# Fedomn/sqlrs

Hardware: AMD Instinct MI355X
Metric: Mrows/sec for filter->hash-join->group-by pipeline; achieved HBM GB/s vs peak (higher is better)
Workload: dtype int64 keys / f64 sum; 1 GPU; C5 filter(val>0.5) -> hash-join(fact x dim on int64 key) -> group-by(key) COUNT,SUM(f64); fact_rows=1000000000, dim_rows=10000000, groups=10000000, parallelism=single GPU

## Files before the change

sqlrs_amd/csrc/agg_partition.hip:

```cpp
#include <algorithm>
#include <cstdlib>
#include <cstring>

#include "agg_partition.hpp"
#include "device_utils.hpp"
#include "radix_part.hpp"

namespace sq {

#ifndef PART_WG_N
#define PART_WG_N 512
#endif
constexpr int PART_WG = PART_WG_N;
#ifndef DENSE_WG_N
#define DENSE_WG_N 1024
#endif
constexpr int DENSE_WG = DENSE_WG_N;
#ifndef HOT_MIN_PEERS_N
#define HOT_MIN_PEERS_N 8
#endif
constexpr int HOT_MIN_PEERS = HOT_MIN_PEERS_N;
constexpr uint64_t LDS_EMPTY = ~0ull;

__device__ __forceinline__ uint32_t bucket_of(uint64_t h, uint32_t P) {
  return (uint32_t)__umul64hi(h, (uint64_t)P);
}

__global__ __launch_bounds__(PART_WG) void key_stats_kernel(const uint64_t *__restrict__ keys,
                                                            const uint64_t *__restrict__ validity,
                                                            int64_t n, int sample_shift, int block_stride, int hll_bits,
                                                            unsigned int *__restrict__ hll) {
  __shared__ unsigned int reg[2 * 4096];
  const int nreg = 1 << hll_bits;
  for (int i = threadIdx.x; i < 2 * 4096; i += PART_WG) reg[i] = 0;
  __syncthreads();
  uint64_t kmin = ~0ull, kmax = 0;
  const int64_t smask = (1ll << sample_shift) - 1, shalf = sample_shift ? 1ll << (sample_shift - 1) : -1;
  const unsigned blk_set = block_stride > 1 && (blockIdx.x & 1) ? 4096u : 0u;
  constexpr int KU = 12;
  const int64_t nchunks = (n + PART_WG * KU - 1) / (PART_WG * KU);
  const int64_t nsel = block_stride > 1 ? (nchunks + block_stride - 1) / block_stride + 1 : nchunks;
  for (int64_t ci = blockIdx.x; ci < nsel; ci += gridDim.x) {
    const int64_t chunk = block_stride > 1 ? min(ci * block_stride, nchunks - 1) : ci;
    const int64_t base = chunk * (int64_t)(PART_WG * KU) + threadIdx.x;
    uint64_t k[KU];
#pragma unroll
    for (int u = 0; u < KU; u++) k[u] = __builtin_nontemporal_load(keys + min(base + u * PART_WG, n - 1));
#pragma unroll
    for (int u = 0; u < KU; u++) {
      const int64_t r = base + u * PART_WG;
      if (r >= n) continue;
      if (validity && !((validity[r >> 6] >> (r & 63)) & 1)) continue;
      const uint64_t o = k[u] ^ (1ull << 63);
      kmin = min(kmin, o);
      kmax = max(kmax, o);
      const int64_t grp = (r >> 6) & smask;
      if (grp != 0 && grp != shalf) continue;
      uint64_t h = mix64(k[u] ^ 0x2545f4914f6cdd1dULL);
      unsigned idx = (unsigned)(h >> (64 - hll_bits)) + (grp == shalf ? 4096u : blk_set);
      unsigned rank = (unsigned)__builtin_clzll((h << hll_bits) | (1ull << (hll_bits - 1))) + 1;
      if (reg[idx] < rank) atomicMax(&reg[idx], rank);
    }
  }
  __syncthreads();
  for (int i = threadIdx.x; i < nreg; i += PART_WG) {
    if (reg[i]) atomicMax(&hll[i], reg[i]);
    if (reg[4096 + i]) atomicMax(&hll[4096 + i], reg[4096 + i]);
  }
  __shared__ unsigned long long s_mm[2][PART_WG / 64];
  kmin = wave_min_u64(kmin);
  kmax = wave_max_u64(kmax);
  if (lane_id() == 0) {
    s_mm[0][wave_id()] = kmin;
    s_mm[1][wave_id()] = kmax;
  }
  __syncthreads();
  if (threadIdx.x == 0) {
    for (int w = 1; w < PART_WG / 64; w++) {
      kmin = min(kmin, (uint64_t)s_mm[0][w]);
      kmax = max(kmax, (uint64_t)s_mm[1][w]);
    }
    unsigned long long *mm = (unsigned long long *)(hll + 8192);
    atomicMin(mm, (unsigned long long)kmin);
    atomicMax(mm + 1, (unsigned long long)kmax);
  }
}

static double hll_pass(Ctx *ctx, const uint64_t *keys, const uint64_t *validity, int64_t n, int sample_shift,
                       uint64_t *omin, uint64_t *omax, int block_stride = 1, double *half = nullptr) {
  const int hll_bits = block_stride > 1 ? 10 : 12;
  BufP hll = ctx->alloc_zero(8192 * 4 + 16);
  SQ_HIP(hipMemsetAsync(hll->as<uint8_t>() + 8192 * 4, 0xff, 8, ctx->stream));
  {
    ProfScope ps(ctx, "key_stats");
    unsigned blocks = (unsigned)std::min<int64_t>(ceil_div(n, (int64_t)PART_WG * 16 * block_stride), 2 * (int64_t)ctx->num_cus);
    key_stats_kernel<<<dim3(std::max(blocks, 1u)), dim3(PART_WG), 0, ctx->stream>>>(keys, validity, n, sample_shift,
                                                                                  block_stride, hll_bits, hll->as<unsigned int>());
    SQ_HIP(hipGetLastError());
  }
  const unsigned int *hreg = (const unsigned int *)ctx->fetch(hll->p, 8192 * 4 + 16);
  if (omin) std::memcpy(omin, hreg + 8192, 8);
  if (omax) std::memcpy(omax, hreg + 8194, 8);
  const int nreg = 1 << hll_bits;
  const double m = (double)nreg;
  auto estimate = [&](bool both) {
    double sum = 0;
    int zeros = 0;
    for (int i = 0; i < nreg; i++) {
      const unsigned r = both ? std::max(hreg[i], hreg[4096 + i]) : hreg[i];
      sum += std::ldexp(1.0, -(int)r);
      zeros += (r == 0);
    }
    double e = (0.7213 / (1.0 + 1.079 / m)) * m * m / sum;
    if (e <= 2.5 * m && zeros) e = m * std::log(m / zeros);
    return e;
  };
  const double e_half = estimate(false), e = estimate(true);
  if (half) *half = e_half;
  return e;
}

double estimate_distinct(Ctx *ctx, const uint64_t *keys, const uint64_t *validity, int64_t n,
                         uint64_t *omin, uint64_t *omax, bool *sampled) {
  if (sampled) *sampled = false;
  constexpr double SATURATED = 0.8;
  constexpr double DISJOINT = 0.6;
  double half = 0;
  if (sampled && !validity && n >= (1ll << 24)) {
    const int stride = 8;
    const double e = hll_pass(ctx, keys, validity, n, 0, omin, omax, stride, &half);
    if (e <= 0.2 * (double)(n / stride) && half >= DISJOINT * e) {
      *sampled = true;
      return half >= SATURATED * e ? e * 1.25 : e * (1.25 + 2.5 * (SATURATED - half / e));
    }
    if (half < DISJOINT * e) return hll_pass(ctx, keys, validity, n, 0, omin, omax);
  }
  const int shift = n >= (1ll << 22) ? 3 : 0;
  double e = hll_pass(ctx, keys, validity, n, shift, omin, omax, 1, &half);
  if (shift && (e > 0.2 * (double)(n >> shift) || half < SATURATED * e)) e = hll_pass(ctx, keys, validity, n, 0, omin, omax);
  return e;
}

enum AccKind { AK_COUNT = 0, AK_SUM_I64 = 1, AK_SUM_F64 = 2, AK_MIN_I64 = 3, AK_MIN_F64 = 4, AK_MAX_I64 = 5, AK_MAX_F64 = 6 };

struct LdsAggParams {
  int n_acc;
  int code[PART_MAX_ACC];
  uint32_t cap;
  const unsigned long long *partner_bits;
  const unsigned int *partner_mult;
  int seg_off;
};

__device__ __forceinline__ unsigned long long acc_times(int kind, unsigned long long cell, unsigned int m) {
  switch (kind) {
  case 0 :
  case 1 : return cell * (unsigned long long)m;
  case 2 : return (unsigned long long)__double_as_longlong(__longlong_as_double((long long)cell) * (double)m);
  default: return cell;
  }
}

__device__ __forceinline__ uint64_t acc_identity_cell(int kind) {
  return (kind == AK_MIN_I64 || kind == AK_MIN_F64) ? ~0ull : 0ull;
}

__device__ __forceinline__ uint32_t slot_hash(uint64_t key) {
  uint32_t x = (uint32_t)key ^ ((uint32_t)(key >> 32) * 0x85ebca6bu);
  x *= 0x9e3779b1u;
  return x ^ (x >> 15);
}

__device__ __forceinline__ void acc_apply(int kind, unsigned long long *c, uint64_t v) {
  switch (kind) {
  case AK_COUNT: atomicAdd(c, 1ull); break;
  case AK_SUM_I64: atomicAdd(c, (unsigned long long)v); break;
  case AK_SUM_F64: unsafeAtomicAdd((double *)c, __longlong_as_double((long long)v)); break;
  case AK_MIN_I64: atomicMin(c, (unsigned long long)i64_to_ordered((int64_t)v)); break;
  case AK_MIN_F64: atomicMin(c, (unsigned long long)f64_to_ordered(__longlong_as_double((long long)v))); break;
  case AK_MAX_I64: atomicMax(c, (unsigned long long)i64_to_ordered((int64_t)v)); break;
  default: atomicMax(c, (unsigned long long)f64_to_ordered(__longlong_as_double((long long)v)));
  }
}

#ifndef LDS_U_ROWS
#define LDS_U_ROWS 4
#endif
constexpr int LDS_U = LDS_U_ROWS;
template <int NV> struct AggRows {
  uint64_t k[LDS_U], v0[NV >= 1 ? LDS_U : 1], v1[NV >= 2 ? LDS_U : 1];
  uint32_t id[LDS_U];
  uint8_t f[LDS_U];
};

template <int NV, bool FLAGS, bool PACK, int WG = PART_WG>
__device__ __forceinline__ void lds_agg_load(const uint64_t *__restrict__ pk, const uint32_t *__restrict__ pi,
                                             const uint64_t *__restrict__ pv0, const uint64_t *__restrict__ pv1,
                                             const uint8_t *__restrict__ pf, int64_t i0, int64_t hi,
                                             AggRows<NV> &r) {
#pragma unroll
  for (int u = 0; u < LDS_U; u++) {
    int64_t i = min(i0 + (int64_t)u * WG, hi - 1);
    r.k[u] = __builtin_nontemporal_load(pk + i);
    if (!PACK) r.id[u] = pi ? __builtin_nontemporal_load(pi + i) : (uint32_t)i;
    if (NV >= 1) r.v0[u] = __builtin_nontemporal_load(pv0 + i);
    if (NV >= 2) r.v1[u] = __builtin_nontemporal_load(pv1 + i);
    r.f[u] = FLAGS ? pf[i] : 7;
  }
}

template <int NV, int WG = PART_WG>
__device__ __forceinline__ void lds_agg_load_rec(const uint64_t *__restrict__ prec, int64_t i0, int64_t hi, AggRows<NV> &r) {
#pragma unroll
  for (int u = 0; u < LDS_U; u++) {
    int64_t i = min(i0 + (int64_t)u * WG, hi - 1);
    const u64x2 t = __builtin_nontemporal_load((const u64x2 *)prec + i);
    r.k[u] = t.x;
    r.v0[0 + (NV >= 1 ? u : 0)] = t.y;
    r.f[u] = 7;
  }
}

struct SplitTables {
  unsigned long long *key = nullptr;
  unsigned int *first = nullptr;
  unsigned long long *acc = nullptr;
  uint32_t nsplit = 0;
};

__global__ void split_init_kernel(SplitTables stb, int64_t total, int n_acc, LdsAggParams prm) {
  int64_t i = blockIdx.x * (int64_t)blockDim.x + threadIdx.x;
  if (i >= total) return;
  stb.key[i] = LDS_EMPTY;
  stb.first[i] = 0xffffffffu;
  for (int a = 0; a < n_acc; a++) stb.acc[(size_t)a * total + i] = acc_identity_cell(prm.code[a] & 7);
}

__global__ void split_emit_kernel(SplitTables stb, uint32_t nslots, uint32_t cap, int n_acc,
                                  unsigned long long *out_count, uint64_t *__restrict__ gkey,
                                  uint32_t *__restrict__ gfirst, uint8_t *__restrict__ gvalid,
                                  uint64_t *__restrict__ gacc, int64_t gcap) {
  const int64_t total = (int64_t)stb.nsplit * nslots;
  int64_t i = blockIdx.x * (int64_t)blockDim.x + threadIdx.x;
  if (i >= total) return;
  unsigned int first = stb.first[i];
  if (first == 0xffffffffu) return;
  const uint32_t s = (uint32_t)(i % nslots);
  unsigned long long base = atomicAdd(out_count, 1ull);
  if ((int64_t)base >= gcap) return;
  gkey[base] = s == cap + 1 ? LDS_EMPTY : stb.key[i];
  gfirst[base] = first;
  if (gvalid) gvalid[base] = s == cap ? 0 : 1;
  for (int a = 0; a < n_acc; a++) gacc[(size_t)a * gcap + base] = stb.acc[(size_t)a * total + i];
}

template <int NV, bool FLAGS, bool JOIN, int NACC, int C0, int C1, bool PACK, bool REC = false>
__global__ __launch_bounds__(PART_WG) void lds_agg_kernel(
    LdsAggParams prm, const uint64_t *__restrict__ pk, const uint32_t *__restrict__ pi,
    const uint64_t *__restrict__ pv0, const uint64_t *__restrict__ pv1,
    const uint8_t *__restrict__ pf, const uint32_t *__restrict__ work , uint32_t P,
    int64_t n, unsigned long long *out_count, uint64_t *__restrict__ gkey,
    uint32_t *__restrict__ gfirst, uint8_t *__restrict__ gvalid, uint64_t *__restrict__ gacc,
    int64_t gcap, unsigned long long *ov_count, uint32_t *__restrict__ ov_rows,
    const uint64_t *__restrict__ bk, const uint8_t *__restrict__ bf, const uint32_t *__restrict__ bbstart,
    KeyPack kp, SplitTables stb) {
  extern __shared__ __attribute__((aligned(16))) unsigned long long tab[];
  __shared__ unsigned int s_cnt, s_join_fail;
  __shared__ unsigned long long s_base;
  const uint32_t b = work[4 * blockIdx.x];
  const int64_t lo = work[4 * blockIdx.x + 1];
  const int64_t hi = work[4 * blockIdx.x + 2];
  const uint32_t split = work[4 * blockIdx.x + 3];
  const uint32_t cap = prm.cap, mask = cap - 1, nslots = cap + 2;
  const int n_acc = NACC >= 0 ? NACC : prm.n_acc;
  auto code_of = [&](int a) { return NACC >= 0 ? (a == 0 ? C0 : C1) : prm.code[a]; };
  unsigned long long *tkey = tab;
  unsigned long long *tacc = tab + nslots;
  unsigned int *tfirst = (unsigned int *)(tacc + (size_t)n_acc * nslots);
  AggRows<NV> cur, nxt;
  if (lo < hi) {
    if (REC) lds_agg_load_rec<NV>(pk, lo + threadIdx.x, hi, cur);
    else lds_agg_load<NV, FLAGS, PACK>(pk, pi, pv0, pv1, pf, lo + threadIdx.x, hi, cur);
  }
  for (uint32_t s = threadIdx.x; s < nslots; s += PART_WG) {
    tkey[s] = LDS_EMPTY;
    tfirst[s] = 0xffffffffu;
#pragma unroll
    for (int a = 0; a < PART_MAX_ACC; a++) {
      if (a >= n_acc) break;
      tacc[(size_t)a * nslots + s] = acc_identity_cell(code_of(a) & 7);
    }
  }
  if (threadIdx.x == 0) {
    s_cnt = 0;
    s_join_fail = 0;
  }
  __syncthreads();
  if (JOIN) {
    if (*(volatile unsigned long long *)(ov_count + 1) != 0) return;
    const int64_t blo = bbstart[b], bhi = bbstart[b + 1];
    for (int64_t i = blo + threadIdx.x; i < bhi; i += PART_WG) {
      uint64_t key = bk[i];
      bool valid = bf ? (bf[i] & 1) : true;
      if (!valid) {
        if (atomicExch(&tkey[cap], 1ull) != LDS_EMPTY) s_join_fail = 1;
      } else if (key == LDS_EMPTY) {
        if (atomicExch(&tkey[cap + 1], 1ull) != LDS_EMPTY) s_join_fail = 1;
      } else {
        uint32_t s = slot_hash(key) & mask;
        uint32_t probes = 0;
        while (true) {
          unsigned long long prev = atomicCAS(&tkey[s], LDS_EMPTY, (unsigned long long)key);
          if (prev == key) s_join_fail = 1;
          if (prev == LDS_EMPTY || prev == key) break;
          s = (s + 1) & mask;
          if (++probes >= cap) {
            s_join_fail = 1;
            break;
          }
        }
      }
    }
    __syncthreads();
    if (s_join_fail) {
      if (threadIdx.x == 0) atomicExch(ov_count + 1, 1ull);
      return;
    }
  }
  __builtin_amdgcn_s_waitcnt(0x0F70);
  for (int64_t base = lo; base < hi; base += (int64_t)LDS_U * PART_WG) {
    const int64_t i0 = base + threadIdx.x;
    if (REC) lds_agg_load_rec<NV>(pk, i0 + (int64_t)LDS_U * PART_WG, hi, nxt);
    else lds_agg_load<NV, FLAGS, PACK>(pk, pi, pv0, pv1, pf, i0 + (int64_t)LDS_U * PART_WG, hi, nxt);
    uint32_t slot[LDS_U];
    unsigned long long seen[LDS_U];
    uint32_t sentinel = 0;
    if (PACK) {
#pragma unroll
      for (int u = 0; u < LDS_U; u++) {
        if (!JOIN && packed_off(kp, cur.k[u]) == kp.kmask) sentinel |= 1u << u;
        cur.id[u] = packed_row(kp, cur.k[u]);
        cur.k[u] = packed_key(kp, cur.k[u]);
      }
    }
#pragma unroll
    for (int u = 0; u < LDS_U; u++) {
      uint32_t s = slot_hash(cur.k[u]) & mask;
      if (FLAGS && !(cur.f[u] & 1)) s = cap;
      else if (cur.k[u] == LDS_EMPTY) s = cap + 1;
      slot[u] = s;
      seen[u] = tkey[s];
    }
#pragma unroll
    for (int u = 0; u < LDS_U; u++) {
      bool act = i0 + (int64_t)u * PART_WG < hi && !((sentinel >> u) & 1u);
      const uint64_t key = cur.k[u];
      uint32_t s = slot[u];
      unsigned long long c = seen[u];
      if (act) {
        if (s >= cap) {
          if (JOIN && c == LDS_EMPTY) act = false;
        } else if (JOIN) {
          uint32_t probes = 0;
          while (c != key && c != LDS_EMPTY && ++probes < cap) {
            s = (s + 1) & mask;
            c = tkey[s];
          }
          if (c != key) act = false;
        } else {
          uint32_t probes = 0;
          while (true) {
            if (c == key) break;
            if (c == LDS_EMPTY) {
              unsigned long long prev = atomicCAS(&tkey[s], LDS_EMPTY, (unsigned long long)key);
              if (prev == LDS_EMPTY || prev == key) break;
            }
            s = (s + 1) & mask;
            if (++probes >= cap) {
              unsigned long long o = atomicAdd(ov_count, 1ull);
              ov_rows[o] = cur.id[u];
              act = false;
              break;
            }
            c = tkey[s];
          }
        }
      }
      const uint64_t actm = __ballot(act);
      if (actm) {
        const int first = __builtin_ctzll(actm);
        const uint32_t s0 = (uint32_t)__shfl((int)s, first, 64);
        const bool hot = act && s == s0;
        const uint64_t peers = __ballot(hot);
        if (__popcll(peers) >= HOT_MIN_PEERS) {
          const uint32_t idmin = wave_min_u32_dpp(hot ? cur.id[u] : 0xffffffffu);
          if (lane_id() == first) atomicMin(&tfirst[s0], idmin);
#pragma unroll
          for (int a = 0; a < PART_MAX_ACC; a++) {
            if (a >= n_acc) break;
            const int code = code_of(a), kind = code & 7, src = code >> 3;
            const bool in = hot && (!FLAGS || (cur.f[u] & (2 << src)));
            const uint64_t v = (NV >= 2 && src) ? cur.v1[u] : cur.v0[u];
            unsigned long long *cell = tacc + (size_t)a * nslots + s0;
            const uint64_t inm = __ballot(in);
            uint64_t red;
            switch (kind) {
            case AK_COUNT: red = (uint64_t)__popcll(inm); break;
            case AK_SUM_I64: red = wave_sum_u64_dpp(in ? v : 0ull); break;
            case AK_SUM_F64: red = (uint64_t)__double_as_longlong(wave_sum_f64_dpp(in ? __longlong_as_double((long long)v) : 0.0)); break;
            case AK_MIN_I64: red = wave_min_u64(in ? i64_to_ordered((int64_t)v) : ~0ull); break;
            case AK_MIN_F64: red = wave_min_u64(in ? f64_to_ordered(__longlong_as_double((long long)v)) : ~0ull); break;
            case AK_MAX_I64: red = wave_max_u64(in ? i64_to_ordered((int64_t)v) : 0ull); break;
            default: red = wave_max_u64(in ? f64_to_ordered(__longlong_as_double((long long)v)) : 0ull);
            }
            if (lane_id() == first && inm) {
              switch (kind) {
              case AK_COUNT:
              case AK_SUM_I64: atomicAdd(cell, (unsigned long long)red); break;
              case AK_SUM_F64: unsafeAtomicAdd((double *)cell, __longlong_as_double((long long)red)); break;
              case AK_MIN_I64:
              case AK_MIN_F64: atomicMin(cell, (unsigned long long)red); break;
              default: atomicMax(cell, (unsigned long long)red);
              }
            }
          }
          act = act && !hot;
        }
      }
      if (act) {
        if (cur.id[u] < tfirst[s]) atomicMin(&tfirst[s], cur.id[u]);
#pragma unroll
        for (int a = 0; a < PART_MAX_ACC; a++) {
          if (a >= n_acc) break;
          const int code = code_of(a);
          const int src = code >> 3;
          if (FLAGS && !(cur.f[u] & (2 << src))) continue;
          uint64_t v = (NV >= 2 && src) ? cur.v1[u] : cur.v0[u];
          acc_apply(code & 7, tacc + (size_t)a * nslots + s, v);
        }
      }
    }
    cur = nxt;
  }
  __syncthreads();
  if (split != 0xffffffffu) {
    unsigned long long *gk = stb.key + (size_t)split * nslots;
    unsigned int *gf = stb.first + (size_t)split * nslots;
    for (uint32_t s = threadIdx.x; s < nslots; s += PART_WG) {
      unsigned int first = tfirst[s];
      if (first == 0xffffffffu) continue;
      uint32_t g = s;
      bool placed = true;
      if (s < cap) {
        const unsigned long long key = tkey[s];
        g = slot_hash(key) & mask;
        uint32_t probes = 0;
        while (true) {
          unsigned long long prev = atomicCAS(&gk[g], LDS_EMPTY, key);
          if (prev == LDS_EMPTY || prev == key) break;
          g = (g + 1) & mask;
          if (++probes >= cap) {
            placed = false;
            break;
          }
        }
      }
      if (!placed) {
        unsigned long long o = atomicAdd(out_count, 1ull);
        if ((int64_t)o < gcap) {
          gkey[o] = tkey[s];
          gfirst[o] = first;
          if (gvalid) gvalid[o] = 1;
#pragma unroll
          for (int a = 0; a < PART_MAX_ACC; a++) {
            if (a >= n_acc) break;
            gacc[(size_t)a * gcap + o] = tacc[(size_t)a * nslots + s];
          }
        }
        atomicExch(ov_count + 2, 1ull);
        continue;
      }
      atomicMin(&gf[g], first);
#pragma unroll
      for (int a = 0; a < PART_MAX_ACC; a++) {
        if (a >= n_acc) break;
        unsigned long long *cell = stb.acc + ((size_t)a * stb.nsplit + split) * nslots + g;
        const unsigned long long v = tacc[(size_t)a * nslots + s];
        switch (code_of(a) & 7) {
        case AK_COUNT:
        case AK_SUM_I64: atomicAdd(cell, v); break;
        case AK_SUM_F64: unsafeAtomicAdd((double *)cell, __longlong_as_double((long long)v)); break;
        case AK_MIN_I64:
        case AK_MIN_F64: atomicMin(cell, v); break;
        default: atomicMax(cell, v);
        }
      }
    }
    return;
  }
  unsigned int mine = 0;
  for (uint32_t s = threadIdx.x; s < nslots; s += PART_WG) mine += tfirst[s] != 0xffffffffu;
  unsigned int my_off = atomicAdd(&s_cnt, mine);
  __syncthreads();
  if (threadIdx.x == 0) s_base = atomicAdd(out_count, (unsigned long long)s_cnt);
  __syncthreads();
  unsigned long long base = s_base + my_off;
  for (uint32_t s = threadIdx.x; s < nslots; s += PART_WG) {
    unsigned int first = tfirst[s];
    if (first == 0xffffffffu) continue;
    if ((int64_t)base < gcap) {
      gkey[base] = s == cap + 1 ? LDS_EMPTY : tkey[s];
      gfirst[base] = first;
      if (gvalid) gvalid[base] = s == cap ? 0 : 1;
#pragma unroll
      for (int a = 0; a < PART_MAX_ACC; a++) {
        if (a >= n_acc) break;
        gacc[(size_t)a * gcap + base] = tacc[(size_t)a * nslots + s];
      }
    }
    base++;
  }
}

constexpr int SED_SLOTS = 16, SED_GROUPS = 16;
__global__ __launch_bounds__(SED_SLOTS * SED_GROUPS) void split_emit_dense_kernel(
    SplitTables stb, const uint32_t *__restrict__ split_bucket, const uint32_t *__restrict__ chunk_lo, uint32_t nbuckets_split,
    uint32_t R, KeyPack kp, LdsAggParams prm, int n_acc, unsigned long long *out_count, uint64_t *__restrict__ gkey,
    uint32_t *__restrict__ gfirst, uint64_t *__restrict__ gacc, int64_t gcap) {
  __shared__ unsigned int s_first[SED_GROUPS][SED_SLOTS];
  __shared__ unsigned long long s_acc[PART_MAX_ACC][SED_GROUPS][SED_SLOTS];
  const uint32_t tiles_per_bucket = (R + SED_SLOTS - 1) / SED_SLOTS;
  const uint32_t t = blockIdx.x / tiles_per_bucket, sl = threadIdx.x % SED_SLOTS, cg = threadIdx.x / SED_SLOTS;
  const uint32_t s = (blockIdx.x % tiles_per_bucket) * SED_SLOTS + sl;
  if (t >= nbuckets_split) return;
  const int64_t total = (int64_t)stb.nsplit * R;
  unsigned int first = 0xffffffffu;
  unsigned long long acc[PART_MAX_ACC];
  for (int a = 0; a < n_acc; a++) acc[a] = acc_identity_cell(prm.code[a] & 7);
  if (s < R) {
    const uint32_t c1 = chunk_lo[t + 1];
    for (uint32_t c = chunk_lo[t] + cg; c < c1; c += SED_GROUPS) {
      const unsigned int f = stb.first[(size_t)c * R + s];
      if (f == 0xffffffffu) continue;
      first = min(first, f);
      for (int a = 0; a < n_acc; a++) {
        const unsigned long long v = stb.acc[(size_t)a * total + (size_t)c * R + s];
        switch (prm.code[a] & 7) {
        case AK_COUNT:
        case AK_SUM_I64: acc[a] += v; break;
        case AK_SUM_F64: acc[a] = (unsigned long long)__double_as_longlong(__longlong_as_double((long long)acc[a]) + __longlong_as_double((long long)v)); break;
        case AK_MIN_I64:
        case AK_MIN_F64: acc[a] = min(acc[a], v); break;
        default: acc[a] = max(acc[a], v);
        }
      }
    }
  }
  s_first[cg][sl] = first;
  for (int a = 0; a < n_acc; a++) s_acc[a][cg][sl] = acc[a];
  __syncthreads();
  if (cg != 0 || s >= R) return;
  for (int g = 1; g < SED_GROUPS; g++) {
    const unsigned int f = s_first[g][sl];
    if (f == 0xffffffffu) continue;
    first = min(first, f);
    for (int a = 0; a < n_acc; a++) {
      const unsigned long long v = s_acc[a][g][sl];
      switch (prm.code[a] & 7) {
      case AK_COUNT:
      case AK_SUM_I64: acc[a] += v; break;
      case AK_SUM_F64: acc[a] = (unsigned long long)__double_as_longlong(__longlong_as_double((long long)acc[a]) + __longlong_as_double((long long)v)); break;
      case AK_MIN_I64:
      case AK_MIN_F64: acc[a] = min(acc[a], v); break;
      default: acc[a] = max(acc[a], v);
      }
    }
  }
  if (first == 0xffffffffu) return;
  unsigned int mlt = 1;
  if (prm.partner_mult) mlt = prm.partner_mult[((uint64_t)split_bucket[t] << kp.rbits) + s];
  unsigned long long base = atomicAdd(out_count, 1ull);
  if ((int64_t)base >= gcap) return;
  gkey[base] = kp.kmin + ((uint64_t)split_bucket[t] << kp.rbits) + s;
  gfirst[base] = first;
  for (int a = 0; a < n_acc; a++) gacc[(size_t)a * gcap + base] = prm.partner_mult ? acc_times(prm.code[a] & 7, acc[a], mlt) : acc[a];
}

template <int NV, bool JOIN, int NACC, int C0, int C1, bool REC = false>
__global__ __launch_bounds__(DENSE_WG) void lds_agg_dense_kernel(
    LdsAggParams prm, const uint64_t *__restrict__ pk, const uint64_t *__restrict__ pv0,
    const uint32_t *__restrict__ work, unsigned long long *out_count, uint64_t *__restrict__ gkey,
    uint32_t *__restrict__ gfirst, uint64_t *__restrict__ gacc, int64_t gcap, KeyPack kp, SplitTables stb) {
  extern __shared__ __attribute__((aligned(16))) unsigned long long tab[];
  __shared__ unsigned int s_cnt;
  __shared__ unsigned long long s_base;
  const uint32_t b = work[4 * blockIdx.x];
  const int64_t lo = work[4 * blockIdx.x + 1];
  const int64_t hi = work[4 * blockIdx.x + 2];
  const uint32_t split = work[4 * blockIdx.x + 3];
  const uint32_t R = prm.cap, mask = R - 1;
  const int n_acc = NACC >= 0 ? NACC : prm.n_acc;
  auto code_of = [&](int a) { return NACC >= 0 ? (a == 0 ? C0 : C1) : prm.code[a]; };
  unsigned long long *tacc = tab;
  unsigned int *tfirst = (unsigned int *)(tacc + (size_t)n_acc * R);
  AggRows<NV> cur, nxt;
  if (lo < hi) {
    if (REC) lds_agg_load_rec<NV, DENSE_WG>(pk, lo + threadIdx.x, hi, cur);
    else lds_agg_load<NV, false, true, DENSE_WG>(pk, nullptr, pv0, nullptr, nullptr, lo + threadIdx.x, hi, cur);
  }
  for (uint32_t s = threadIdx.x; s < R; s += DENSE_WG) {
    tfirst[s] = 0xffffffffu;
#pragma unroll
    for (int a = 0; a < PART_MAX_ACC; a++) {
      if (a >= n_acc) break;
      tacc[(size_t)a * R + s] = acc_identity_cell(code_of(a) & 7);
    }
  }
  if (threadIdx.x == 0) s_cnt = 0;
  __syncthreads();
  uint32_t hc_slot = 0xffffffffu, hc_min = 0xffffffffu;
  uint64_t hc_acc[PART_MAX_ACC];
  auto hot_flush = [&]() {
    if (hc_slot == 0xffffffffu) return;
    if (lane_id() == 0) {
      atomicMin(&tfirst[hc_slot], hc_min);
#pragma unroll
      for (int a = 0; a < PART_MAX_ACC; a++) {
        if (a >= n_acc) break;
        unsigned long long *cell = tacc + (size_t)a * R + hc_slot;
        switch (code_of(a) & 7) {
        case AK_COUNT:
        case AK_SUM_I64: atomicAdd(cell, (unsigned long long)hc_acc[a]); break;
        case AK_SUM_F64: unsafeAtomicAdd((double *)cell, __longlong_as_double((long long)hc_acc[a])); break;
        case AK_MIN_I64:
        case AK_MIN_F64: atomicMin(cell, (unsigned long long)hc_acc[a]); break;
        default: atomicMax(cell, (unsigned long long)hc_acc[a]);
        }
      }
    }
    hc_slot = 0xffffffffu;
  };
  auto hot_take = [&](uint32_t s0, uint32_t idmin) {
    if (hc_slot != s0) {
      hot_flush();
      hc_slot = s0;
      hc_min = 0xffffffffu;
#pragma unroll
      for (int a = 0; a < PART_MAX_ACC; a++) {
        if (a >= n_acc) break;
        hc_acc[a] = acc_identity_cell(code_of(a) & 7);
      }
    }
    hc_min = idmin < hc_min ? idmin : hc_min;
  };
  auto hot_add = [&](int a, int kind, uint64_t red) {
    switch (kind) {
    case AK_COUNT:
    case AK_SUM_I64: hc_acc[a] += red; break;
    case AK_SUM_F64: hc_acc[a] = (uint64_t)__double_as_longlong(__longlong_as_double((long long)hc_acc[a]) + __longlong_as_double((long long)red)); break;
    case AK_MIN_I64:
    case AK_MIN_F64: hc_acc[a] = red < hc_acc[a] ? red : hc_acc[a]; break;
    default: hc_acc[a] = red > hc_acc[a] ? red : hc_acc[a];
    }
  };
  __builtin_amdgcn_s_waitcnt(0x0F70);
  for (int64_t base = lo; base < hi; base += (int64_t)LDS_U * DENSE_WG) {
    const int64_t i0 = base + threadIdx.x;
    if (REC) lds_agg_load_rec<NV, DENSE_WG>(pk, i0 + (int64_t)LDS_U * DENSE_WG, hi, nxt);
    else lds_agg_load<NV, false, true, DENSE_WG>(pk, nullptr, pv0, nullptr, nullptr, i0 + (int64_t)LDS_U * DENSE_WG, hi, nxt);
#pragma unroll
    for (int u = 0; u < LDS_U; u++) {
      const uint64_t off = packed_off(kp, cur.k[u]);
      const uint32_t id = packed_row(kp, cur.k[u]);
      const uint32_t s = (uint32_t)off & mask;
      bool act = i0 + (int64_t)u * DENSE_WG < hi;
      act = act && off <= kp.range;
      const uint64_t actm = __ballot(act);
      if (actm) {
        const int first = __builtin_ctzll(actm);
        const uint32_t s0 = (uint32_t)__shfl((int)s, first, 64);
        const bool hot = act && s == s0;
        const uint64_t peers = __ballot(hot);
        if (__popcll(peers) >= HOT_MIN_PEERS) {
          const uint32_t idmin = wave_min_u32_dpp(hot ? id : 0xffffffffu);
          hot_take(s0, idmin);
#pragma unroll
          for (int a = 0; a < PART_MAX_ACC; a++) {
            if (a >= n_acc) break;
            const int kind = code_of(a) & 7;
            const uint64_t v = NV >= 1 ? cur.v0[u] : 0ull;
            uint64_t red;
            switch (kind) {
            case AK_COUNT: red = (uint64_t)__popcll(peers); break;
            case AK_SUM_I64: red = wave_sum_u64_dpp(hot ? v : 0ull); break;
            case AK_SUM_F64: red = (uint64_t)__double_as_longlong(wave_sum_f64_dpp(hot ? __longlong_as_double((long long)v) : 0.0)); break;
            case AK_MIN_I64: red = wave_min_u64(hot ? i64_to_ordered((int64_t)v) : ~0ull); break;
            case AK_MIN_F64: red = wave_min_u64(hot ? f64_to_ordered(__longlong_as_double((long long)v)) : ~0ull); break;
            case AK_MAX_I64: red = wave_max_u64(hot ? i64_to_ordered((int64_t)v) : 0ull); break;
            default: red = wave_max_u64(hot ? f64_to_ordered(__longlong_as_double((long long)v)) : 0ull);
            }
            hot_add(a, kind, red);
          }
          act = act && !hot;
        }
      }
      if (act) {
        if (id < tfirst[s]) atomicMin(&tfirst[s], id);
#pragma unroll
        for (int a = 0; a < PART_MAX_ACC; a++) {
          if (a >= n_acc) break;
          acc_apply(code_of(a) & 7, tacc + (size_t)a * R + s, NV >= 1 ? cur.v0[u] : 0ull);
        }
      }
    }
    cur = nxt;
  }
  hot_flush();
  __syncthreads();
  if (JOIN && (prm.partner_bits || prm.partner_mult)) {
    const uint64_t off0 = (uint64_t)b << kp.rbits;
    for (uint32_t s = threadIdx.x; s < R; s += DENSE_WG) {
      if (tfirst[s] == 0xffffffffu) continue;
      const uint64_t o = off0 + s;
      const bool partner = prm.partner_mult ? prm.partner_mult[o] != 0 : (((prm.partner_bits[o >> 6] >> (o & 63)) & 1ull) != 0);
      if (!partner) tfirst[s] = 0xffffffffu;
    }
  }
  if (split != 0xffffffffu) {
    unsigned int *gf = stb.first + (size_t)split * R;
    for (uint32_t s = threadIdx.x; s < R; s += DENSE_WG) {
      gf[s] = tfirst[s];
#pragma unroll
      for (int a = 0; a < PART_MAX_ACC; a++) {
        if (a >= n_acc) break;
        stb.acc[((size_t)a * stb.nsplit + split) * R + s] = tacc[(size_t)a * R + s];
      }
    }
    return;
  }
  unsigned int mine = 0;
  for (uint32_t s = threadIdx.x; s < R; s += DENSE_WG) mine += tfirst[s] != 0xffffffffu;
  unsigned int my_off = atomicAdd(&s_cnt, mine);
  __syncthreads();
  if (threadIdx.x == 0) s_base = atomicAdd(out_count, (unsigned long long)s_cnt);
  __syncthreads();
  unsigned long long base = s_base + my_off;
  const uint64_t key0 = kp.kmin + ((uint64_t)b << kp.rbits);
  for (uint32_t s = threadIdx.x; s < R; s += DENSE_WG) {
    unsigned int first = tfirst[s];
    if (first == 0xffffffffu) continue;
    if ((int64_t)base < gcap) {
      gkey[base] = key0 + s;
      gfirst[base] = first;
      const unsigned int mlt = (JOIN && prm.partner_mult) ? prm.partner_mult[((uint64_t)b << kp.rbits) + s] : 1u;
#pragma unroll
      for (int a = 0; a < PART_MAX_ACC; a++) {
        if (a >= n_acc) break;
        const unsigned long long cell = tacc[(size_t)a * R + s];
        gacc[(size_t)a * gcap + base] = (JOIN && prm.partner_mult) ? acc_times(code_of(a) & 7, cell, mlt) : cell;
      }
    }
    base++;
  }
}

struct SlimBucketIn {
  SlimRowsView rows;
  const uint32_t *nzstart, *nzbt, *nzcount, *bcol;
  uint32_t tile;
  uint32_t groups;
  const uint32_t *blk_bt;
  uint32_t log_b;
};
constexpr uint32_t SLIM_BT_CAP = 4096;
struct SlimAggRows {
  uint64_t v[LDS_U];
  uint32_t w[LDS_U], bt[LDS_U];
};

template <bool JOIN, int NACC, int C0, int C1, bool BLK = false>
__global__ __launch_bounds__(DENSE_WG) void lds_agg_dense_slim_kernel(
    LdsAggParams prm, SlimBucketIn in, const uint32_t *__restrict__ work, unsigned long long *out_count,
    uint64_t *__restrict__ gkey, uint32_t *__restrict__ gfirst, uint64_t *__restrict__ gacc, int64_t gcap, KeyPack kp,
    SplitTables stb) {
  extern __shared__ __attribute__((aligned(16))) unsigned long long tab[];
  __shared__ unsigned int s_cnt, s_before, s_inside;
  __shared__ unsigned long long s_base;
  __shared__ uint32_t s_wsum[DENSE_WG / 64];
  const uint32_t b = work[4 * blockIdx.x];
  const int64_t lo = work[4 * blockIdx.x + 1];
  const int64_t hi = work[4 * blockIdx.x + 2];
  const uint32_t split = work[4 * blockIdx.x + 3];
  const uint32_t R = prm.cap, mask = R - 1;
  const int n_acc = NACC >= 0 ? NACC : prm.n_acc;
  auto code_of = [&](int a) { return NACC >= 0 ? (a == 0 ? C0 : C1) : prm.code[a]; };
  unsigned long long *tacc = tab;
  unsigned int *tfirst = (unsigned int *)(tacc + (size_t)n_acc * R);
  unsigned long long *gmask = (unsigned long long *)(tfirst + R);
  uint32_t *gpre = (uint32_t *)(gmask + in.groups);
  uint32_t *gbt = gpre + in.groups;
  const uint32_t col = BLK ? 0u : in.bcol[b], nruns = BLK ? 0u : in.nzcount[b];
  const uint32_t ngroups = BLK ? 0u : (uint32_t)((hi - lo + 63) >> 6);
  const uint64_t le_mask = (2ull << lane_id()) - 1ull;
  const uint32_t rbits = kp.rbits, lmask = (1u << 13) - 1u;

  for (uint32_t s = threadIdx.x; s < R; s += DENSE_WG) {
    tfirst[s] = 0xffffffffu;
#pragma unroll
    for (int a = 0; a < PART_MAX_ACC; a++) {
      if (a >= n_acc) break;
      tacc[(size_t)a * R + s] = acc_identity_cell(code_of(a) & 7);
    }
  }
  for (uint32_t g = threadIdx.x; g < ngroups; g += DENSE_WG) gmask[g] = 0;
  if (threadIdx.x == 0) {
    s_cnt = 0;
    s_before = 0;
    s_inside = 0;
  }
  __syncthreads();
  if (!BLK) {
    uint32_t before = 0, inside = 0;
    for (uint32_t k = threadIdx.x; k < nruns; k += DENSE_WG) {
      const int64_t st = in.nzstart[col + k];
      if (st <= lo) before++;
      else if (st < hi) {
        inside++;
        atomicOr(&gmask[(st - lo) >> 6], 1ull << ((st - lo) & 63));
      }
    }
    before = wave_sum_u32(before);
    inside = wave_sum_u32(inside);
    if (lane_id() == 0 && before) atomicAdd(&s_before, before);
    if (lane_id() == 0 && inside) atomicAdd(&s_inside, inside);
  }
  __syncthreads();
  const uint32_t k_first = s_before - 1u, k_count = s_inside + 1u;
  const bool bt_lds = !BLK && k_count <= SLIM_BT_CAP;
  const bool seg_mode = NACC == 2 && ((C0 == AK_COUNT && C1 == AK_SUM_F64) || (C0 == AK_SUM_F64 && C1 == AK_COUNT)) &&
                        hi - lo >= 4096 && (int64_t)k_count * 2048 <= hi - lo && !prm.seg_off && !BLK;
  if (bt_lds)
    for (uint32_t k = threadIdx.x; k < k_count; k += DENSE_WG) gbt[k] = in.nzbt[col + min(k_first + k, nruns - 1)];
  if (!BLK) {
    constexpr uint32_t GPT = 8;
    uint32_t carry = s_before - 1u;
    for (uint32_t g0 = 0; g0 < ngroups; g0 += DENSE_WG * GPT) {
      const uint32_t gb = g0 + threadIdx.x * GPT;
      uint32_t pc[GPT], sum = 0;
#pragma unroll
      for (uint32_t i = 0; i < GPT; i++) {
        pc[i] = gb + i < ngroups ? (uint32_t)__popcll(gmask[gb + i]) : 0u;
        sum += pc[i];
      }
      const uint32_t inc = wave_iscan_u32(sum);
      if (lane_id() == 63) s_wsum[wave_id()] = inc;
      __syncthreads();
      uint32_t wbase = 0, tot = 0;
      for (int w = 0; w < DENSE_WG / 64; w++) {
        if (w < wave_id()) wbase += s_wsum[w];
        tot += s_wsum[w];
      }
      uint32_t run = carry + wbase + inc - sum;
#pragma unroll
      for (uint32_t i = 0; i < GPT; i++) {
        if (gb + i < ngroups) gpre[gb + i] = run;
        run += pc[i];
      }
      carry += tot;
      __syncthreads();
    }
  }
#ifndef SLIM_WAVE_SPAN
#define SLIM_WAVE_SPAN 1
#endif
  constexpr int64_t SLIM_USTEP = SLIM_WAVE_SPAN ? 64 : DENSE_WG;
  const int64_t slim_toff = SLIM_WAVE_SPAN ? (int64_t)wave_id() * (LDS_U * 64) + lane_id() : (int64_t)threadIdx.x;
  auto load = [&](int64_t i0, SlimAggRows &r) {
#pragma unroll
    for (int u = 0; u < LDS_U; u++) {
      const int64_t i = min(i0 + (int64_t)u * SLIM_USTEP, hi - 1);
      slim_load_nt(in.rows, i, r.w[u], r.v[u]);
      if (BLK) {
        r.bt[u] = in.blk_bt[i >> in.log_b];
        continue;
      }
      const uint32_t g = (uint32_t)((i - lo) >> 6);
      const uint32_t k = gpre[g] + (uint32_t)__popcll(gmask[g] & le_mask);
#if defined(SLIM_DBG) && (SLIM_DBG & 16)
      r.bt[u] = k;
#else
      r.bt[u] = bt_lds ? gbt[min(k - k_first, k_count - 1)] : in.nzbt[col + min(k, nruns - 1)];
#endif
    }
  };
  uint32_t hc_slot = 0xffffffffu, hc_min = 0xffffffffu;
  uint64_t hc_acc[PART_MAX_ACC];
  auto hot_flush = [&]() {
    if (hc_slot == 0xffffffffu) return;
    if (lane_id() == 0) {
      atomicMin(&tfirst[hc_slot], hc_min);
#pragma unroll
      for (int a = 0; a < PART_MAX_ACC; a++) {
        if (a >= n_acc) break;
        unsigned long long *cell = tacc + (size_t)a * R + hc_slot;
        switch (code_of(a) & 7) {
        case AK_COUNT:
        case AK_SUM_I64: atomicAdd(cell, (unsigned long long)hc_acc[a]); break;
        case AK_SUM_F64: unsafeAtomicAdd((double *)cell, __longlong_as_double((long long)hc_acc[a])); break;
        case AK_MIN_I64:
        case AK_MIN_F64: atomicMin(cell, (unsigned long long)hc_acc[a]); break;
        default: atomicMax(cell, (unsigned long long)hc_acc[a]);
        }
      }
    }
    hc_slot = 0xffffffffu;
  };
  auto hot_take = [&](uint32_t s0, uint32_t idmin) {
    if (hc_slot != s0) {
      hot_flush();
      hc_slot = s0;
      hc_min = 0xffffffffu;
#pragma unroll
      for (int a = 0; a < PART_MAX_ACC; a++) {
        if (a >= n_acc) break;
        hc_acc[a] = acc_identity_cell(code_of(a) & 7);
      }
    }
    hc_min = idmin < hc_min ? idmin : hc_min;
  };
  auto hot_add = [&](int a, int kind, uint64_t red) {
    switch (kind) {
    case AK_COUNT:
    case AK_SUM_I64: hc_acc[a] += red; break;
    case AK_SUM_F64: hc_acc[a] = (uint64_t)__double_as_longlong(__longlong_as_double((long long)hc_acc[a]) + __longlong_as_double((long long)red)); break;
    case AK_MIN_I64:
    case AK_MIN_F64: hc_acc[a] = red < hc_acc[a] ? red : hc_acc[a]; break;
    default: hc_acc[a] = red > hc_acc[a] ? red : hc_acc[a];
    }
  };
  SlimAggRows cur, nxt;
  if (lo < hi) load(lo + slim_toff, cur);
  __builtin_amdgcn_s_waitcnt(0x0F70);
  for (int64_t base = lo; base < hi; base += (int64_t)LDS_U * DENSE_WG) {
    const int64_t i0 = base + slim_toff;
    load(i0 + (int64_t)LDS_U * DENSE_WG, nxt);
    uint32_t sl[LDS_U], id[LDS_U], tf[LDS_U];
#pragma unroll
    for (int u = 0; u < LDS_U; u++) {
      const uint32_t w = cur.w[u];
      sl[u] = w & mask;
      id[u] = (cur.bt[u] + (w >> (rbits + 13))) * in.tile + ((w >> rbits) & lmask);
      tf[u] = tfirst[sl[u]];
    }
    constexpr bool SEG_CAPABLE = NACC == 2 && ((C0 == AK_COUNT && C1 == AK_SUM_F64) || (C0 == AK_SUM_F64 && C1 == AK_COUNT));
    const int lane = (int)lane_id();
    auto seg_rows = [&](bool act, uint32_t sl_u, uint64_t v_u, uint32_t id_u, uint32_t tf_u) {
      const uint32_t key = act ? sl_u : (0x80000000u | (uint32_t)lane);
      const uint32_t prevk = (uint32_t)__builtin_amdgcn_update_dpp(0, (int)key, 0x138, 0xf, 0xf, false);
      const uint64_t bm = __ballot(lane == 0 || key != prevk);
      const int headl = 63 - __builtin_clzll(bm & le_mask);
      double incl = act ? __longlong_as_double((long long)v_u) : 0.0;
      uint32_t idh = act ? id_u : 0xffffffffu;
      wave_seg_iscan_f64_min_u32(incl, idh, headl, lane);
      const bool tail = act && (lane == 63 || ((bm >> (lane + 1)) & 1ull));
      if (tail) {
        const uint32_t s = sl_u;
        if (idh < tf_u) atomicMin(&tfirst[s], idh);
        atomicAdd(tacc + (size_t)(C0 == AK_COUNT ? 0 : 1) * R + s, (unsigned long long)(lane - headl + 1));
        unsafeAtomicAdd((double *)(tacc + (size_t)(C0 == AK_COUNT ? 1 : 0) * R + s), incl);
      }
    };
    if (seg_mode) {
#pragma unroll
      for (int u = 0; u < LDS_U; u++) {
        const bool act = i0 + (int64_t)u * SLIM_USTEP < hi;
        {
          const uint32_t s0 = (uint32_t)__builtin_amdgcn_readfirstlane((int)sl[u]);
          if (__ballot(act && sl[u] == s0) == ~0ull) {
            hot_take(s0, wave_min_u32_dpp(id[u]));
            hot_add(C0 == AK_COUNT ? 0 : 1, AK_COUNT, 64ull);
            hot_add(C0 == AK_COUNT ? 1 : 0, AK_SUM_F64, (uint64_t)__double_as_longlong(wave_sum_f64_dpp(__longlong_as_double((long long)cur.v[u]))));
            continue;
          }
        }
        seg_rows(act, sl[u], cur.v[u], id[u], tf[u]);
      }
      cur = nxt;
      continue;
    }
#pragma unroll
    for (int u = 0; u < LDS_U; u++) {
      const uint32_t s = sl[u];
      bool act = i0 + (int64_t)u * SLIM_USTEP < hi;
      if (BLK) act = act && cur.w[u] != 0xffffffffu;
#ifdef SLIM_DBG
      uint64_t actm = (SLIM_DBG & 1) ? 0ull : __ballot(act);
#else
      uint64_t actm = __ballot(act);
#endif
      for (int it = 0; it < 3 && actm; it++) {
        const int first = __builtin_ctzll(actm);
        const uint32_t s0 = (uint32_t)__builtin_amdgcn_readlane((int)s, first);
        const bool hot = act && s == s0;
        const uint64_t peers = __ballot(hot);
        if (__popcll(peers) < HOT_MIN_PEERS) break;
        if (SEG_CAPABLE && it == 0 && peers != actm && (((peers >> first) + 1) & (peers >> first)) == 0 && !prm.seg_off) {
          seg_rows(act, s, cur.v[u], id[u], tf[u]);
          act = false;
          break;
        }
        const uint32_t idmin = wave_min_u32_dpp(hot ? id[u] : 0xffffffffu);
        hot_take(s0, idmin);
#pragma unroll
        for (int a = 0; a < PART_MAX_ACC; a++) {
          if (a >= n_acc) break;
          const int kind = code_of(a) & 7;
          const uint64_t v = cur.v[u];
          uint64_t red;
          switch (kind) {
          case AK_COUNT: red = (uint64_t)__popcll(peers); break;
          case AK_SUM_I64: red = wave_sum_u64_dpp(hot ? v : 0ull); break;
          case AK_SUM_F64: red = (uint64_t)__double_as_longlong(wave_sum_f64_dpp(hot ? __longlong_as_double((long long)v) : 0.0)); break;
          case AK_MIN_I64: red = wave_min_u64(hot ? i64_to_ordered((int64_t)v) : ~0ull); break;
          case AK_MIN_F64: red = wave_min_u64(hot ? f64_to_ordered(__longlong_as_double((long long)v)) : ~0ull); break;
          case AK_MAX_I64: red = wave_max_u64(hot ? i64_to_ordered((int64_t)v) : 0ull); break;
          default: red = wave_max_u64(hot ? f64_to_ordered(__longlong_as_double((long long)v)) : 0ull);
          }
          hot_add(a, kind, red);
        }
        act = act && !hot;
        actm &= ~peers;
      }
      if (act) {
#ifdef SLIM_DBG
        if (!(SLIM_DBG & 8) && id[u] < tf[u]) atomicMin(&tfirst[s], id[u]);
#pragma unroll
        for (int a = 0; a < PART_MAX_ACC; a++) {
          if (a >= n_acc) break;
          if ((SLIM_DBG >> (1 + a)) & 1) continue;
          acc_apply(code_of(a) & 7, tacc + (size_t)a * R + s, cur.v[u]);
        }
#else
        if (id[u] < tf[u]) atomicMin(&tfirst[s], id[u]);
#pragma unroll
        for (int a = 0; a < PART_MAX_ACC; a++) {
          if (a >= n_acc) break;
          acc_apply(code_of(a) & 7, tacc + (size_t)a * R + s, cur.v[u]);
        }
#endif
      }
    }
    cur = nxt;
  }
  hot_flush();
  __syncthreads();
  if (JOIN && (prm.partner_bits || prm.partner_mult)) {
    const uint64_t off0 = (uint64_t)b << kp.rbits;
    for (uint32_t s = threadIdx.x; s < R; s += DENSE_WG) {
      if (tfirst[s] == 0xffffffffu) continue;
      const uint64_t o = off0 + s;
      const bool partner = prm.partner_mult ? prm.partner_mult[o] != 0 : (((prm.partner_bits[o >> 6] >> (o & 63)) & 1ull) != 0);
      if (!partner) tfirst[s] = 0xffffffffu;
    }
  }
  if (split != 0xffffffffu) {
    unsigned int *gf = stb.first + (size_t)split * R;
    for (uint32_t s = threadIdx.x; s < R; s += DENSE_WG) {
      gf[s] = tfirst[s];
#pragma unroll
      for (int a = 0; a < PART_MAX_ACC; a++) {
        if (a >= n_acc) break;
        stb.acc[((size_t)a * stb.nsplit + split) * R + s] = tacc[(size_t)a * R + s];
      }
    }
    return;
  }
  unsigned int mine = 0;
  for (uint32_t s = threadIdx.x; s < R; s += DENSE_WG) mine += tfirst[s] != 0xffffffffu;
  unsigned int my_off = atomicAdd(&s_cnt, mine);
  __syncthreads();
  if (threadIdx.x == 0) s_base = atomicAdd(out_count, (unsigned long long)s_cnt);
  __syncthreads();
  unsigned long long obase = s_base + my_off;
  const uint64_t key0 = kp.kmin + ((uint64_t)b << kp.rbits);
  for (uint32_t s = threadIdx.x; s < R; s += DENSE_WG) {
    unsigned int first = tfirst[s];
    if (first == 0xffffffffu) continue;
    if ((int64_t)obase < gcap) {
      gkey[obase] = key0 + s;
      gfirst[obase] = first;
      const unsigned int mlt = (JOIN && prm.partner_mult) ? prm.partner_mult[((uint64_t)b << kp.rbits) + s] : 1u;
#pragma unroll
      for (int a = 0; a < PART_MAX_ACC; a++) {
        if (a >= n_acc) break;
        const unsigned long long cell = tacc[(size_t)a * R + s];
        gacc[(size_t)a * gcap + obase] = (JOIN && prm.partner_mult) ? acc_times(code_of(a) & 7, cell, mlt) : cell;
      }
    }
    obase++;
  }
}

__global__ void first_to_rowid_kernel(const uint32_t *__restrict__ gfirst, int64_t n, uint64_t offset,
                                      uint64_t *__restrict__ out) {
  int64_t i = blockIdx.x * (int64_t)blockDim.x + threadIdx.x;
  if (i < n) out[i] = offset + gfirst[i];
}
__global__ void bytes_pack_kernel(const uint8_t *__restrict__ bytes, int64_t n, uint64_t *__restrict__ out) {
  int64_t i = blockIdx.x * (int64_t)blockDim.x + threadIdx.x;
  bool b = (i < n) && bytes[i];
  uint64_t m = __ballot(b);
  if (lane_id() == 0 && i < n) out[i >> 6] = m;
}

__global__ __launch_bounds__(256) void key_range_kernel(const uint64_t *__restrict__ keys, int64_t n, unsigned long long *mm) {
  uint64_t kmin = ~0ull, kmax = 0;
  for (int64_t r = blockIdx.x * (int64_t)blockDim.x + threadIdx.x; r < n; r += (int64_t)gridDim.x * blockDim.x) {
    const uint64_t o = keys[r] ^ (1ull << 63);
    kmin = min(kmin, o);
    kmax = max(kmax, o);
  }
  kmin = wave_min_u64(kmin);
  kmax = wave_max_u64(kmax);
  __shared__ unsigned long long s_lo[4], s_hi[4];
  if (lane_id() == 0) {
    s_lo[wave_id()] = kmin;
    s_hi[wave_id()] = kmax;
  }
  __syncthreads();
  if (threadIdx.x == 0) {
    for (int w = 1; w < 4; w++) {
      kmin = min(kmin, (uint64_t)s_lo[w]);
      kmax = max(kmax, (uint64_t)s_hi[w]);
    }
    atomicMin(mm, (unsigned long long)kmin);
    atomicMax(mm + 1, (unsigned long long)kmax);
  }
}

const uint64_t *part_row_ids(Ctx *ctx, PartAggOutput &po) {
  if (!po.row_ids) {
    const int64_t g1 = std::max<int64_t>(po.groups, 1);
    po.row_ids = ctx->alloc(8 * (size_t)g1);
    if (po.groups) {
      first_to_rowid_kernel<<<dim3((unsigned)ceil_div(g1, 256)), dim3(256), 0, ctx->stream>>>(
          po.gfirst->as<uint32_t>(), po.groups, po.row_offset, po.row_ids->as<uint64_t>());
      SQ_HIP(hipGetLastError());
    }
  }
  return po.row_ids->as<uint64_t>();
}

bool partitioned_preaggregate(Ctx *ctx, const PartAggSpec &spec, const PartAggInput &in,
                              uint64_t row_offset, PartAggOutput *out) {
  int64_t n = in.n;
  if (n > 0xffffffffll || spec.n_acc > PART_MAX_ACC || spec.nv > 2) return false;
  const bool join_mode = in.join_keys != nullptr;
  uint64_t omin = ~0ull, omax = 0;
  bool sampled = false;
  const char *kse = hook("SQLRS_KEY_STATS_EXACT");
  const bool stats_exact_env = kse && kse[0] == '1';
  double est = join_mode ? (double)in.join_n
                         : estimate_distinct(ctx, in.keys, in.key_validity, n, &omin, &omax, (in.exact_stats || stats_exact_env) ? nullptr : &sampled);
  BufP ctr = ctx->alloc_zero(48);
  if (sampled && omin <= omax) {
    const uint64_t w = omax - omin, pad = std::max<uint64_t>(w / 8, 65536);
    omin = omin >= pad ? omin - pad : 0;
    omax = omax <= ~0ull - pad ? omax + pad : ~0ull;
  }
  static const double est_scale = [] {
    const char *e = hook("SQLRS_EST_SCALE");
    return e ? std::atof(e) : 1.0;
  }();
  if (!join_mode) est = std::max(1.0, est * est_scale);
  KeyPack kp;
  const bool nullable = in.key_validity || in.val_validity[0] || in.val_validity[1];
  if (!nullable && spec.nv <= 1 && !(join_mode && in.join_validity)) {
    if (join_mode && in.join_range_known) {
      omin = in.join_omin;
      omax = in.join_omax;
    } else if (join_mode) {
      BufP mm = ctx->alloc(16);
      SQ_HIP(hipMemsetAsync(mm->p, 0xff, 8, ctx->stream));
      SQ_HIP(hipMemsetAsync(mm->as<uint8_t>() + 8, 0, 8, ctx->stream));
      unsigned blocks = (unsigned)std::min<int64_t>(ceil_div(in.join_n, 1024), 1024);
      key_range_kernel<<<dim3(std::max(blocks, 1u)), dim3(256), 0, ctx->stream>>>(
          in.join_keys, in.join_n, mm->as<unsigned long long>());
      SQ_HIP(hipGetLastError());
      const uint64_t *h = (const uint64_t *)ctx->fetch(mm->p, 16);
      omin = h[0];
      omax = h[1];
    }
    if (omin <= omax) {
      uint64_t range = omax - omin;
      uint32_t kbits = 1;
      while (kbits < 64 && ((1ull << kbits) - 1) <= range) kbits++;
      int rowbits = 1;
      while (rowbits < 32 && (1ll << rowbits) < n) rowbits++;
      if (kbits + rowbits <= 64) {
        kp.kbits = kbits;
        kp.kmask = (1ull << kbits) - 1;
        kp.kmin = omin ^ (1ull << 63);
        if (sampled) {
          kp.oob = (unsigned int *)(ctr->as<uint64_t>() + 4);
          out->ov_rows = ctx->alloc(4 * (size_t)std::max<int64_t>(n, 1));
          kp.ov_rows = out->ov_rows->as<uint32_t>();
          kp.ov_count = ctr->as<unsigned long long>() + 1;
          kp.ov_cap = (uint32_t)std::min<int64_t>(n, std::max<int64_t>(65536, n / 1024));
        }
      }
    }
  }
  constexpr size_t lds_budget = 72 * 1024;
  const size_t slot_bytes = 8 + 8 * (size_t)spec.n_acc + 4;
  uint32_t cap = 1;
  while ((size_t)(cap * 2 + 2) * slot_bytes <= lds_budget) cap *= 2;
  constexpr double load_factor = 0.275;
  const double groups_per_table = cap * load_factor;
  double want = est * 1.15 / groups_per_table;
  if (!join_mode) est = std::min(est, (double)n);
  const char *dense_e = hook("SQLRS_DENSE_AGG");
  const bool dense_on = !(dense_e && dense_e[0] == '0');
  const uint64_t *partner_bits = nullptr;
  const double want_hashed = want;
  bool dense = false;
  if (dense_on && kp.kbits) {
    const uint64_t range = omax - omin;
    constexpr size_t dense_budget = 150 * 1024;
    const size_t dslot = 8 * (size_t)spec.n_acc + 4;
    uint32_t rbits = 8;
    while (rbits < 14 && ((size_t)2 << rbits) * dslot <= dense_budget) rbits++;
    while (rbits > 8 && (range >> (rbits - 1)) == 0) rbits--;
    const uint64_t pd = (range >> rbits) + 1;
    const bool fills = join_mode ? (in.join_unique_known && (range + 1 == (uint64_t)in.join_n ||
                                                             ((in.join_bits || in.join_mult) && in.join_range_known && range / 16 <= (uint64_t)in.join_n)))
                                 : ((double)range + 1.0 <= 4.0 * est);
    partner_bits = (join_mode && fills && !in.join_mult && range + 1 != (uint64_t)in.join_n) ? in.join_bits : nullptr;
    if (fills && pd <= 65536 && (double)pd <= 1.5 * std::max(1.0, std::ceil(want))) {
      dense = true;
      kp.dense = 1;
      kp.rbits = rbits;
      kp.range = range;
      cap = 1u << rbits;
      want = (double)pd;
    }
  }
  if (join_mode && in.join_mult && !dense) return false;
  if (want > 65536.0) return false;
  uint32_t P = (uint32_t)std::max(1.0, std::ceil(want));
  out->est_groups = est;
  PartitionInput pin;
  pin.pack = kp;
  pin.filter = in.filter;
  pin.keys = in.keys;
  pin.key_validity = in.key_validity;
  pin.n = n;
  pin.nv = spec.nv;
  for (int k = 0; k < 2; k++) {
    pin.vals[k] = in.vals[k];
    pin.val_validity[k] = in.val_validity[k];
  }
  PartitionedRows pr;
  const bool in_place = P == 1 && !join_mode && !nullable && want_hashed <= 1.0 && !in.filter.col;
  if (in_place) {
    dense = false;
    kp = KeyPack();
    cap = 1;
    while ((size_t)(cap * 2 + 2) * slot_bytes <= lds_budget) cap *= 2;
    pr.n = n;
    pr.P = 1;
    auto borrowed = [&](const void *p) {
      BufP b = std::make_shared<Buf>(ctx, const_cast<void *>(p), 0);
      b->owned = false;
      return b;
    };
    pr.key = borrowed(in.keys);
    pr.v0 = spec.nv >= 1 ? borrowed(in.vals[0]) : nullptr;
    pr.v1 = spec.nv >= 2 ? borrowed(in.vals[1]) : nullptr;
    pr.bstart_host = {0u, (uint32_t)n};
    pr.bstart = nullptr;
  } else if (!partition_rows(ctx, pin, P, &pr)) {
    return false;
  }
  P = pr.P;
  n = pr.n;
  if (dense != (pr.pack.dense != 0)) return false;
  if (n == 0) {
    out->groups = out->n_overflow = 0;
    out->gcap = 1;
    out->buckets = (int)P;
    out->gkey = ctx->alloc(8);
    out->gfirst = ctx->alloc(4);
    out->gacc = ctx->alloc(8 * (size_t)std::max(spec.n_acc, 1));
    out->ov_rows = ctx->alloc(4);
    out->row_ids = nullptr;
    out->row_offset = row_offset;
    return true;
  }
  out->buckets = (int)P;
  BufP pk = pr.key, pi = pr.idx, pv0 = pr.v0, pv1 = pr.v1, pf = pr.flags;
  PartitionedRows local_build;
  const PartitionedRows *bp = nullptr;
  if (join_mode && !dense) {
    if (in.join_cache && in.join_cache->P == P && in.join_cache->n == in.join_n) {
      bp = in.join_cache;
    } else {
      PartitionInput bin;
      bin.keys = in.join_keys;
      bin.key_validity = in.join_validity;
      bin.n = in.join_n;
      bin.nv = 0;
      bin.build_side = true;
      PartitionedRows *dst = in.join_cache ? in.join_cache : &local_build;
      if (!partition_rows(ctx, bin, P, dst) || dst->P != P) return false;
      bp = dst;
    }
  }
  LdsAggParams prm;
  prm.n_acc = spec.n_acc;
  for (int a = 0; a < PART_MAX_ACC; a++) {
    int kind = AK_COUNT;
    if (a < spec.n_acc) {
      switch (spec.op[a]) {
      case PART_COUNT: kind = AK_COUNT; break;
      case PART_SUM_I64: kind = AK_SUM_I64; break;
      case PART_SUM_F64: kind = AK_SUM_F64; break;
      case PART_MIN: kind = spec.kind[a] ? AK_MIN_F64 : AK_MIN_I64; break;
      default: kind = spec.kind[a] ? AK_MAX_F64 : AK_MAX_I64;
      }
    }
    prm.code[a] = a < spec.n_acc ? (kind | (spec.src[a] << 3)) : 0;
  }
  prm.cap = cap;
  prm.partner_bits = dense ? (const unsigned long long *)partner_bits : nullptr;
  prm.partner_mult = (dense && join_mode) ? in.join_mult : nullptr;
  {
    const char *seg_e = hook("SQLRS_AGG_SEG");
    prm.seg_off = (seg_e && seg_e[0] == '0') ? 1 : 0;
  }
  int64_t gcap = (int64_t)std::min<double>((double)n, est * 1.5 + 65536.0 + 2.0 * P);
  if (dense) gcap = (int64_t)std::min<uint64_t>((uint64_t)n, join_mode ? (uint64_t)in.join_n : kp.range + 1);
  size_t lds = dense ? round_up((size_t)cap * (slot_bytes - 8), 16) : round_up((size_t)(cap + 2) * slot_bytes, 16);
  const std::vector<uint32_t> &hb = pr.bstart_host;
  if (hb.size() != (size_t)P + 1) return false;
  uint32_t chunk = (uint32_t)std::max<int64_t>(32768, 2 * (n / std::max<uint32_t>(P, 1)));
  uint32_t split_above = chunk;
  if (dense) {
    int64_t nonempty_d = 0;
    for (uint32_t bkt = 0; bkt < P; bkt++) nonempty_d += pr.bucket_end(bkt) > hb[bkt];
    const int64_t avg = n / std::max<int64_t>(nonempty_d, 1);
    const char *cd_e = hook("SQLRS_DENSE_CHUNK_DIV");
    const int cdiv = cd_e ? std::max(1, std::atoi(cd_e)) : 2;
    constexpr int sa_pct = 125;
    chunk = (uint32_t)std::max<int64_t>(32768, avg / cdiv);
    split_above = (uint32_t)std::max<int64_t>(65536, avg * sa_pct / 100);
  }
  {
    const uint32_t slots = (lds > 80 * 1024 - 64 ? 1u : 2u) * (uint32_t)ctx->num_cus;
    uint32_t nonempty = 0;
    for (uint32_t bkt = 0; bkt < P; bkt++) nonempty += pr.bucket_end(bkt) > hb[bkt];
    if (nonempty < slots / 2) {
      chunk = (uint32_t)std::max<int64_t>(32768, n / (2 * (int64_t)slots));
      split_above = chunk;
    }
  }
  if (pr.slim.on && !pr.slim.blk_bt) {
    const size_t table = round_up((size_t)cap * (slot_bytes - 8), 16);
    const size_t room = 159 * 1024 > table + 4 * SLIM_BT_CAP ? 159 * 1024 - table - 4 * SLIM_BT_CAP : 0;
    const uint32_t item_rows = (uint32_t)std::min<size_t>(1u << 18, (room / 12 > 2 ? room / 12 - 2 : 0) * 64);
    if (item_rows < 16384) return false;
    chunk = std::min(chunk, item_rows);
    split_above = std::min(split_above, item_rows);
  }
  std::vector<uint32_t> work, split_bucket, chunk_lo;
  work.reserve(4 * ((size_t)P + 64));
  out->may_dup = false;
  uint32_t nsplit = 0, nchunk_tables = 0;
  for (uint32_t bkt = 0; bkt < P; bkt++) {
    uint32_t lo = hb[bkt], hi = pr.bucket_end(bkt);
    if (dense && lo == hi) continue;
    if (hi - lo <= split_above) {
      work.insert(work.end(), {bkt, lo, hi, 0xffffffffu});
    } else if (dense) {
      chunk_lo.push_back(nchunk_tables);
      const uint32_t pieces = (uint32_t)ceil_div((int64_t)(hi - lo), (int64_t)chunk);
      for (uint32_t q = 0; q < pieces; q++) {
        const uint32_t c0 = lo + (uint32_t)((uint64_t)(hi - lo) * q / pieces), c1 = lo + (uint32_t)((uint64_t)(hi - lo) * (q + 1) / pieces);
        work.insert(work.end(), {bkt, c0, c1, nchunk_tables++});
      }
      split_bucket.push_back(bkt);
      nsplit++;
    } else {
      for (uint32_t c0 = lo; c0 < hi; c0 += chunk) work.insert(work.end(), {bkt, c0, std::min(hi, c0 + chunk), nsplit});
      split_bucket.push_back(bkt);
      nsplit++;
    }
  }
  chunk_lo.push_back(nchunk_tables);
  if (nsplit) {
    std::vector<uint32_t> ord(work.size() / 4), sorted(work.size());
    for (uint32_t i = 0; i < ord.size(); i++) ord[i] = i;
    std::stable_sort(ord.begin(), ord.end(), [&](uint32_t a, uint32_t b) {
      return work[4 * a + 2] - work[4 * a + 1] > work[4 * b + 2] - work[4 * b + 1];
    });
    for (size_t i = 0; i < ord.size(); i++) std::memcpy(&sorted[4 * i], &work[4 * ord[i]], 16);
    work.swap(sorted);
  }
  const uint32_t nwork = (uint32_t)(work.size() / 4);
  BufP dwork = ctx->alloc(4 * work.size() + 16);
  SQ_HIP(hipMemcpyAsync(dwork->p, work.data(), 4 * work.size(), hipMemcpyHostToDevice, ctx->stream));
  const uint32_t nslots_h = dense ? cap : cap + 2;
  SplitTables stb;
  BufP stb_key, stb_first, stb_acc, dsplit;
  BufP dchunk_lo;
  if (nsplit && dense) {
    const int64_t total = (int64_t)nchunk_tables * nslots_h;
    stb_first = ctx->alloc(4 * (size_t)total);
    stb_acc = ctx->alloc(8 * (size_t)total * (size_t)std::max(spec.n_acc, 1));
    stb.first = stb_first->as<unsigned int>();
    stb.acc = stb_acc->as<unsigned long long>();
    stb.nsplit = nchunk_tables;
    dsplit = ctx->alloc(4 * (size_t)nsplit);
    dchunk_lo = ctx->alloc(4 * ((size_t)nsplit + 1));
    SQ_HIP(hipMemcpyAsync(dsplit->p, split_bucket.data(), 4 * (size_t)nsplit, hipMemcpyHostToDevice, ctx->stream));
    SQ_HIP(hipMemcpyAsync(dchunk_lo->p, chunk_lo.data(), 4 * ((size_t)nsplit + 1), hipMemcpyHostToDevice, ctx->stream));
  } else if (nsplit) {
    const int64_t total = (int64_t)nsplit * nslots_h;
    stb_key = ctx->alloc(8 * (size_t)total);
    stb_first = ctx->alloc(4 * (size_t)total);
    stb_acc = ctx->alloc(8 * (size_t)total * (size_t)std::max(spec.n_acc, 1));
    stb.key = stb_key->as<unsigned long long>();
    stb.first = stb_first->as<unsigned int>();
    stb.acc = stb_acc->as<unsigned long long>();
    stb.nsplit = nsplit;
    split_init_kernel<<<dim3((unsigned)ceil_div(total, 256)), dim3(256), 0, ctx->stream>>>(stb, total, spec.n_acc, prm);
    SQ_HIP(hipGetLastError());
  }
  out->gkey = ctx->alloc(8 * (size_t)gcap);
  out->gfirst = ctx->alloc(4 * (size_t)gcap);
  out->gvalid = in.key_validity ? ctx->alloc((size_t)gcap) : nullptr;
  out->gacc = ctx->alloc(8 * (size_t)gcap * (size_t)std::max(spec.n_acc, 1));
  out->gcap = gcap;
  if (!out->ov_rows) out->ov_rows = ctx->alloc(4 * (size_t)std::max<int64_t>(n, 1));
  ctx->agg_route[pr.pack.kbits ? Ctx::AR_PACKED : Ctx::AR_UNPACKED]++;
  ctx->agg_route[Ctx::AR_FLAGS] += pf != nullptr;
  ctx->agg_route[Ctx::AR_REC] += pr.rec != nullptr;
  ctx->agg_route[Ctx::AR_IN_PLACE] += in_place;
  ctx->agg_route[Ctx::AR_JOIN] += join_mode;
  ctx->agg_route[Ctx::AR_JOIN_MULT] += prm.partner_mult != nullptr;
  ctx->agg_route[Ctx::AR_SPLIT] += nsplit > 0;
  {
    ProfScope ps(ctx, "lds_agg");
#define SQ_LA(NV, FL, JN, NA, C0, C1, PK)                                                                        \
  do {                                                                                                         \
    auto kfn = lds_agg_kernel<NV, FL, JN, NA, C0, C1, PK>;                                                      \
    constexpr bool can_rec = NV == 1 && PK && !FL;                                                             \
    if (can_rec && pr.rec) kfn = lds_agg_kernel<NV, FL, JN, NA, C0, C1, PK, can_rec>;                          \
    else if (pr.rec) fail(SQLRS_ERR_INTERNAL, "record-form partition in a column-form bucket pass");           \
    allow_big_lds(ctx, kfn);                                                                                   \
    kfn<<<dim3(nwork), dim3(PART_WG), lds, ctx->stream>>>(                                                     \
        prm, pr.rec ? pr.rec->as<uint64_t>() : pk->as<uint64_t>(), pi ? pi->as<uint32_t>() : nullptr, pv0 ? pv0->as<uint64_t>() : nullptr,       \
        pv1 ? pv1->as<uint64_t>() : nullptr, pf ? pf->as<uint8_t>() : nullptr, dwork->as<uint32_t>(), P, n,    \
        ctr->as<unsigned long long>(), out->gkey->as<uint64_t>(), out->gfirst->as<uint32_t>(),                 \
        out->gvalid ? out->gvalid->as<uint8_t>() : nullptr, out->gacc->as<uint64_t>(), gcap,                   \
        ctr->as<unsigned long long>() + 1, out->ov_rows->as<uint32_t>(),                                       \
        bp ? bp->key->as<uint64_t>() : nullptr, (bp && bp->flags) ? bp->flags->as<uint8_t>() : nullptr,        \
        bp ? bp->bstart->as<uint32_t>() : nullptr, pr.pack, stb);                                              \
    ctx->agg_route[NA < 0 ? Ctx::AR_PROBE_GENERIC : Ctx::AR_PROBE_SPEC]++;                                     \
    launched = true;                                                                                           \
  } while (0)
#define SQ_LA_J(NV, FL, NA, C0, C1)                                                                            \
  do {                                                                                                         \
    if (pr.pack.kbits) {                                                                                       \
      if (join_mode) SQ_LA(NV, FL, true, NA, C0, C1, true);                                                    \
      else SQ_LA(NV, FL, false, NA, C0, C1, true);                                                             \
    } else {                                                                                                   \
      if (join_mode) SQ_LA(NV, FL, true, NA, C0, C1, false);                                                   \
      else SQ_LA(NV, FL, false, NA, C0, C1, false);                                                            \
    }                                                                                                          \
  } while (0)
    const int nvu = pv1 ? 2 : ((pv0 || pr.rec) ? 1 : 0);
    bool launched = false;
    if (dense && pr.slim.on) {
      uint32_t max_item = 64;
      for (uint32_t i = 0; i < nwork; i++) max_item = std::max(max_item, work[4 * i + 2] - work[4 * i + 1]);
      const bool blk = pr.slim.blk_bt != nullptr;
      SlimBucketIn sb;
      sb.rows = pr.slim.rows;
      sb.nzstart = blk ? nullptr : pr.slim.nzstart->as<uint32_t>();
      sb.nzbt = blk ? nullptr : pr.slim.nzbt->as<uint32_t>();
      sb.nzcount = blk ? nullptr : pr.slim.nzcount->as<uint32_t>();
      sb.bcol = blk ? nullptr : pr.slim.bcol->as<uint32_t>();
      sb.tile = pr.slim.tile;
      sb.groups = blk ? 0u : (uint32_t)ceil_div((int64_t)max_item, 64) + 1;
      sb.blk_bt = blk ? pr.slim.blk_bt->as<uint32_t>() : nullptr;
      sb.log_b = pr.slim.log_b;
      const size_t slds = round_up((size_t)cap * (slot_bytes - 8), 16) + (blk ? 16 : 12 * (size_t)sb.groups + 4 * SLIM_BT_CAP);
#define SQ_LS(JN, NA, C0, C1)                                                                                  \
  do {                                                                                                         \
    auto kfn = lds_agg_dense_slim_kernel<JN, NA, C0, C1>;                                                       \
    if (blk) kfn = lds_agg_dense_slim_kernel<JN, NA, C0, C1, true>;                                             \
    allow_big_lds(ctx, kfn, 159 * 1024);                                                                                 \
    kfn<<<dim3(nwork), dim3(DENSE_WG), slds, ctx->stream>>>(prm, sb, dwork->as<uint32_t>(), ctr->as<unsigned long long>(), \
                                                           out->gkey->as<uint64_t>(), out->gfirst->as<uint32_t>(), \
                                                           out->gacc->as<uint64_t>(), gcap, pr.pack, stb);        \
    ctx->agg_route[blk ? Ctx::AR_SLIM_BLK : Ctx::AR_SLIM_RUNS]++;                                              \
    ctx->agg_route[Ctx::AR_INTERPRETED] += NA < 0;                                                             \
    launched = true;                                                                                           \
  } while (0)
#define SQ_LS_J(NA, C0, C1) do { if (join_mode) SQ_LS(true, NA, C0, C1); else SQ_LS(false, NA, C0, C1); } while (0)
      const int c0 = prm.code[0], c1 = spec.n_acc == 2 ? prm.code[1] : -1;
      if (spec.n_acc == 2 && c0 == AK_COUNT && c1 == AK_SUM_F64) SQ_LS_J(2, AK_COUNT, AK_SUM_F64);
      else if (spec.n_acc == 2 && c0 == AK_SUM_F64 && c1 == AK_COUNT) SQ_LS_J(2, AK_SUM_F64, AK_COUNT);
      else if (spec.n_acc == 1 && c0 == AK_SUM_F64) SQ_LS_J(1, AK_SUM_F64, 0);
      else if (spec.n_acc == 1 && c0 == AK_COUNT) SQ_LS_J(1, AK_COUNT, 0);
      else SQ_LS_J(-1, 0, 0);
#undef SQ_LS_J
#undef SQ_LS
      if (nsplit) {
        split_emit_dense_kernel<<<dim3((unsigned)(nsplit * ceil_div((int64_t)nslots_h, SED_SLOTS))), dim3(SED_SLOTS * SED_GROUPS), 0, ctx->stream>>>(
            stb, dsplit->as<uint32_t>(), dchunk_lo->as<uint32_t>(), nsplit, cap, pr.pack, prm, spec.n_acc,
            ctr->as<unsigned long long>(), out->gkey->as<uint64_t>(), out->gfirst->as<uint32_t>(), out->gacc->as<uint64_t>(), gcap);
      }
    } else if (dense) {
#define SQ_LD(NV, JN, NA, C0, C1)                                                                              \
  do {                                                                                                         \
    auto kfn = lds_agg_dense_kernel<NV, JN, NA, C0, C1>;                                                        \
    if (NV == 1 && pr.rec) kfn = lds_agg_dense_kernel<NV, JN, NA, C0, C1, NV == 1>;                            \
    allow_big_lds(ctx, kfn);                                                                                   \
    kfn<<<dim3(nwork), dim3(DENSE_WG), lds, ctx->stream>>>(                                                    \
        prm, pr.rec ? pr.rec->as<uint64_t>() : pk->as<uint64_t>(), pv0 ? pv0->as<uint64_t>() : nullptr, dwork->as<uint32_t>(), \
        ctr->as<unsigned long long>(), out->gkey->as<uint64_t>(), out->gfirst->as<uint32_t>(),                 \
        out->gacc->as<uint64_t>(), gcap, pr.pack, stb);                                                        \
    ctx->agg_route[Ctx::AR_DENSE]++;                                                                           \
    ctx->agg_route[Ctx::AR_INTERPRETED] += NA < 0;                                                             \
    launched = true;                                                                                           \
  } while (0)
#define SQ_LD_J(NV, NA, C0, C1) do { if (join_mode) SQ_LD(NV, true, NA, C0, C1); else SQ_LD(NV, false, NA, C0, C1); } while (0)
      if (nvu == 1 && spec.n_acc <= 2) {
        const int c0 = prm.code[0], c1 = spec.n_acc == 2 ? prm.code[1] : -1;
#define SQ_SIG1(K) if (!launched && spec.n_acc == 1 && c0 == K) SQ_LD_J(1, 1, K, 0)
#define SQ_SIG2(K0, K1) if (!launched && spec.n_acc == 2 && c0 == K0 && c1 == K1) SQ_LD_J(1, 2, K0, K1)
        SQ_SIG1(AK_COUNT); SQ_SIG1(AK_SUM_I64); SQ_SIG1(AK_SUM_F64); SQ_SIG1(AK_MIN_I64); SQ_SIG1(AK_MIN_F64);
        SQ_SIG1(AK_MAX_I64); SQ_SIG1(AK_MAX_F64);
        SQ_SIG2(AK_COUNT, AK_SUM_F64); SQ_SIG2(AK_SUM_F64, AK_COUNT);
        SQ_SIG2(AK_COUNT, AK_SUM_I64); SQ_SIG2(AK_SUM_I64, AK_COUNT);
        SQ_SIG2(AK_MIN_F64, AK_MAX_F64); SQ_SIG2(AK_MIN_I64, AK_MAX_I64);
#undef SQ_SIG1
#undef SQ_SIG2
      }
      if (!launched) { if (nvu == 0) SQ_LD_J(0, -1, 0, 0); else SQ_LD_J(1, -1, 0, 0); }
#undef SQ_LD_J
#undef SQ_LD
      if (nsplit) {
        split_emit_dense_kernel<<<dim3((unsigned)(nsplit * ceil_div((int64_t)nslots_h, SED_SLOTS))), dim3(SED_SLOTS * SED_GROUPS), 0, ctx->stream>>>(
            stb, dsplit->as<uint32_t>(), dchunk_lo->as<uint32_t>(), nsplit, cap, pr.pack, prm, spec.n_acc,
            ctr->as<unsigned long long>(), out->gkey->as<uint64_t>(), out->gfirst->as<uint32_t>(), out->gacc->as<uint64_t>(), gcap);
      }
    }
    if (!launched && !pf && nvu == 1 && spec.n_acc <= 2) {
      const int c0 = prm.code[0], c1 = spec.n_acc == 2 ? prm.code[1] : -1;
#define SQ_SIG1(K) if (!launched && spec.n_acc == 1 && c0 == K) SQ_LA_J(1, false, 1, K, 0)
#define SQ_SIG2(K0, K1) if (!launched && spec.n_acc == 2 && c0 == K0 && c1 == K1) SQ_LA_J(1, false, 2, K0, K1)
      SQ_SIG1(AK_COUNT); SQ_SIG1(AK_SUM_I64); SQ_SIG1(AK_SUM_F64); SQ_SIG1(AK_MIN_I64); SQ_SIG1(AK_MIN_F64);
      SQ_SIG1(AK_MAX_I64); SQ_SIG1(AK_MAX_F64);
      SQ_SIG2(AK_COUNT, AK_SUM_F64); SQ_SIG2(AK_SUM_F64, AK_COUNT);
      SQ_SIG2(AK_COUNT, AK_SUM_I64); SQ_SIG2(AK_SUM_I64, AK_COUNT);
      SQ_SIG2(AK_MIN_F64, AK_MAX_F64); SQ_SIG2(AK_MIN_I64, AK_MAX_I64);
#undef SQ_SIG1
#undef SQ_SIG2
    }
    if (!launched) {
      if (pf) { if (nvu == 0) SQ_LA_J(0, true, -1, 0, 0); else if (nvu == 1) SQ_LA_J(1, true, -1, 0, 0); else SQ_LA_J(2, true, -1, 0, 0); }
      else { if (nvu == 0) SQ_LA_J(0, false, -1, 0, 0); else if (nvu == 1) SQ_LA_J(1, false, -1, 0, 0); else SQ_LA_J(2, false, -1, 0, 0); }
    }
#undef SQ_LA_J
#undef SQ_LA
    if (nsplit && !dense) {
      const int64_t total = (int64_t)nsplit * nslots_h;
      split_emit_kernel<<<dim3((unsigned)ceil_div(total, 256)), dim3(256), 0, ctx->stream>>>(
          stb, nslots_h, cap, spec.n_acc, ctr->as<unsigned long long>(), out->gkey->as<uint64_t>(),
          out->gfirst->as<uint32_t>(), out->gvalid ? out->gvalid->as<uint8_t>() : nullptr,
          out->gacc->as<uint64_t>(), gcap);
    }
    SQ_HIP(hipGetLastError());
  }
  const uint64_t *h = (const uint64_t *)ctx->fetch(ctr->p, 40);
  if (h[4]) {
    out->retry_exact = true;
    return false;
  }
  out->groups = (int64_t)h[0];
  out->n_overflow = (int64_t)h[1];
  ctx->agg_route[Ctx::AR_OVERFLOW_ROWS] += out->n_overflow;
  out->may_dup = h[3] != 0;
  if (join_mode && h[2]) return false;
  if (out->groups > gcap) return false;
  int64_t g1 = std::max<int64_t>(out->groups, 1);
  out->row_offset = row_offset;
  out->row_ids = nullptr;
  if (out->groups) {
    if (out->gvalid) {
      out->gvalid_bits = ctx->alloc(bitmap_bytes(g1));
      int64_t g64 = (int64_t)round_up((size_t)g1, 64);
      bytes_pack_kernel<<<dim3((unsigned)ceil_div(g64, 256)), dim3(256), 0, ctx->stream>>>(
          out->gvalid->as<uint8_t>(), out->groups, out->gvalid_bits->as<uint64_t>());
    }
    SQ_HIP(hipGetLastError());
  }
  return true;
}

}
```

sqlrs_amd/csrc/agg_partition.hpp:

```cpp
#pragma once

#include <cmath>

#include "common.hpp"
#include "prims.hpp"
#include "radix_part.hpp"

namespace sq {

constexpr int PART_MAX_ACC = 6;
enum PartOp { PART_COUNT = 0, PART_SUM_I64 = 1, PART_SUM_F64 = 2, PART_MIN = 3, PART_MAX = 4 };

struct PartAggSpec {
  int n_acc = 0;
  int op[PART_MAX_ACC] = {0};
  int src[PART_MAX_ACC] = {0};
  int kind[PART_MAX_ACC] = {0};
  int nv = 0;
};

struct PartAggInput {
  const uint64_t *keys = nullptr;
  const uint64_t *key_validity = nullptr;
  int64_t n = 0;
  const void *vals[2] = {nullptr, nullptr};
  const uint64_t *val_validity[2] = {nullptr, nullptr};
  const uint64_t *join_keys = nullptr;
  const uint64_t *join_validity = nullptr;
  int64_t join_n = 0;
  struct PartitionedRows *join_cache = nullptr;
  bool join_range_known = false;
  uint64_t join_omin = 0, join_omax = 0;
  bool join_unique_known = true;
  const uint64_t *join_bits = nullptr;
  const uint32_t *join_mult = nullptr;
  RowFilter filter;
  bool exact_stats = false;
};

struct PartAggOutput {
  int64_t groups = 0, gcap = 0;
  BufP gkey, gfirst, gvalid, gvalid_bits, gacc;
  BufP row_ids;
  uint64_t row_offset = 0;
  int64_t n_overflow = 0;
  BufP ov_rows;
  bool may_dup = false;
  double est_groups = 0;
  int buckets = 0;
  bool retry_exact = false;
};

const uint64_t *part_row_ids(Ctx *ctx, PartAggOutput &po);
double estimate_distinct(Ctx *ctx, const uint64_t *keys, const uint64_t *validity, int64_t n,
                         uint64_t *omin = nullptr, uint64_t *omax = nullptr, bool *sampled = nullptr);
bool partitioned_preaggregate(Ctx *ctx, const PartAggSpec &spec, const PartAggInput &in,
                              uint64_t row_offset, PartAggOutput *out);

}
```

sqlrs_amd/csrc/common.hpp:

```cpp
#pragma once

#include <hip/hip_runtime.h>

#include <cstdint>
#include <cstdlib>
#include <cstring>
#include <map>
#include <set>
#include <memory>
#include <string>
#include <vector>

#include "sqlrs_hip.h"

namespace sq {

inline bool hooks_enabled() {
  static const bool on = [] {
    const char *e = std::getenv("SQLRS_HOOKS");
    return e && e[0] == '1';
  }();
  return on;
}
inline const char *hook(const char *name) { return hooks_enabled() ? std::getenv(name) : nullptr; }

struct Error {
  int status;
  std::string msg;
};
[[noreturn]] inline void fail(int status, const std::string &m) { throw Error{status, m}; }

#define SQ_HIP(expr)                                                                              \
  do {                                                                                            \
    hipError_t _e = (expr);                                                                       \
    if (_e != hipSuccess)                                                                         \
      ::sq::fail(SQLRS_ERR_DEVICE, std::string(#expr) + ": " + hipGetErrorString(_e));            \
  } while (0)

inline int64_t ceil_div(int64_t a, int64_t b) { return (a + b - 1) / b; }
inline size_t round_up(size_t a, size_t b) { return (a + b - 1) / b * b; }
inline size_t bitmap_bytes(int64_t rows) { return (size_t)ceil_div(rows, 64) * 8; }

inline size_t width_of(int32_t dtype) {
  switch (dtype) {
  case SQLRS_INT32:
  case SQLRS_UINT32:
    return 4;
  case SQLRS_INT64:
  case SQLRS_UINT64:
  case SQLRS_FLOAT64:
    return 8;
  default:
    return 0;
  }
}

struct Pool {
  std::multimap<size_t, void *> free_blocks;
  size_t live_bytes = 0, cached_bytes = 0;
  bool closed = false;
  int device = 0;
  uint8_t *arena = nullptr;
  size_t arena_bytes = 0, arena_used = 0;
  bool in_arena(const void *p) const { return arena && (const uint8_t *)p >= arena && (const uint8_t *)p < arena + arena_bytes; }
  struct VmmBlock {
    std::vector<hipMemGenericAllocationHandle_t> handles;
    size_t size = 0;
  };
  std::map<void *, VmmBlock> vmm_blocks;
  int vmm = -1;
  void *vmm_alloc(size_t want);
  bool vmm_free(void *p);
  void *alloc(size_t bytes, size_t *cap);
  void release(void *p, size_t cap);
  void trim();
};

struct Ctx;
struct Buf {
  Ctx *ctx;
  std::shared_ptr<Pool> pool;
  void *p;
  size_t cap;
  bool owned = true;
  std::shared_ptr<Buf> parent;
  Buf(Ctx *c, void *ptr, size_t n);
  ~Buf();
  Buf(const Buf &) = delete;
  Buf &operator=(const Buf &) = delete;
  template <class T> T *as() const { return (T *)p; }
};
using BufP = std::shared_ptr<Buf>;
inline BufP buf_view(const BufP &parent, const void *p, size_t bytes) {
  BufP v = std::make_shared<Buf>(parent->ctx, const_cast<void *>(p), bytes);
  v->owned = false;
  v->parent = parent;
  return v;
}

struct ProfEntry {
  const char *name;
  double total_ms = 0;
  int64_t launches = 0;
};
struct ProfPending {
  int entry;
  hipEvent_t a, b;
};

struct Ctx {
  int device = 0;
  hipStream_t stream = nullptr;
  std::string last_error;
  std::shared_ptr<Pool> pool_ref = std::make_shared<Pool>();
  Pool &pool = *pool_ref;
  int num_cus = 256;
  bool prof_on = false;
  std::vector<ProfEntry> prof;
  std::vector<ProfPending> prof_pending;
  std::vector<hipEvent_t> event_pool;
  hipEvent_t order_event = nullptr;
  void *pinned = nullptr;
  size_t pinned_bytes = 0;

  BufP alloc(size_t bytes);
  BufP alloc_zero(size_t bytes);
  BufP zero_block;
  size_t zero_used = 0;
  std::set<const void *> big_lds_set;
  std::map<const void *, int> occ_cache;
  int64_t lb_timeouts = 0;
  int64_t order_lb_fallbacks = 0;
  int lb_backoff = 0;
  int64_t async_conj_batches = 0;
  int64_t async_fast_batches = 0;
  enum AggRoute {
    AR_DENSE, AR_SLIM_RUNS, AR_SLIM_BLK, AR_PROBE_SPEC, AR_PROBE_GENERIC,
    AR_INTERPRETED,
    AR_PACKED, AR_UNPACKED,
    AR_FLAGS,
    AR_REC,
    AR_IN_PLACE,
    AR_JOIN,
    AR_JOIN_MULT,
    AR_SPLIT,
    AR_OVERFLOW_ROWS,
    AR_MERGE_GROUPS,
    AR_PENDING,
    AR_WIDE_PARTS,
    AR_COUNT_
  };
  int64_t agg_route[AR_COUNT_] = {};
  enum JoinRoute {
    JR_DENSE_ADOPTED,
    JR_DENSE_REFUSED,
    JR_DENSE_ONE_FETCH, JR_DENSE_TWO_FETCH,
    JR_DENSE_PACKED, JR_DENSE_PLAIN,
    JR_PROBE_PENDING,
    JR_ALLHIT_KEPT, JR_ALLHIT_REDONE,
    JR_COMPACT_DENSE, JR_COMPACT_SLOTS,
    JR_UNIQUE_OUTER,
    JR_DD_STREAM, JR_DD_ROWS,
    JR_COUNTS_GROUPED, JR_COUNTS_PER_ROW,
    JR_LDS_UNIQUE, JR_LDS_DISTINCT,
    JR_TABLE_LATE,
    JR_COUNT_
  };
  int64_t join_route[JR_COUNT_] = {};
  enum OrderRoute {
    OR_GENERAL,
    OR_UTF8,
    OR_NARROW,
    OR_NARROW_HBM_ONLY,
    OR_LOOKBACK, OR_COUNTING,
    OR_REC12, OR_REC16,
    OR_WIDE,
    OR_WIDE_DECLINED,
    OR_WIDE_PURE,
    OR_WIDE_FIN2, OR_WIDE_FIN3,
    OR_HEAVY_TO_WIDE,
    OR_SAMPLED, OR_SAMPLE_MISSED,
    OR_IN_ORDER,
    OR_COMPOSITE, OR_COMPOSITE_NULLABLE,
    OR_COMPOSITE_TOO_WIDE,
    OR_NULL_SPLIT,
    OR_TOPK, OR_TOPK_IGNORED,
    OR_ALLOC_DECLINED,
    OR_TOPK_KEYS, OR_TOPK_KEYS_IGNORED,
    OR_COUNT_
  };
  int64_t order_route[OR_COUNT_] = {};
  int64_t stage_all_types_batches = 0;
  int64_t stage_stitch_flushes = 0;
  int64_t simple_reduce_batches = 0;
  int64_t fused_eval_filter_batches = 0;
  int64_t fused_eval_project_columns = 0;
  std::shared_ptr<void> small_ring;
  void sync() { SQ_HIP(hipStreamSynchronize(stream)); }
  const void *fetch(const void *dptr, size_t bytes);
  template <class T> T fetch_value(const T *dptr) { return *(const T *)fetch(dptr, sizeof(T)); }
  void *pinned_early = nullptr;
  hipEvent_t early_event = nullptr;
  bool fetch_early(const void *dptr, size_t bytes);
  const void *fetch_early_wait();
  int prof_entry(const char *name);
  void prof_resolve();
};

template <class K> inline void allow_big_lds(Ctx *ctx, K kfn, int bytes = 150 * 1024) {
  const void *f = (const void *)kfn;
  if (ctx->big_lds_set.count(f)) return;
  SQ_HIP(hipFuncSetAttribute(f, hipFuncAttributeMaxDynamicSharedMemorySize, bytes));
  ctx->big_lds_set.insert(f);
}

struct ProfScope {
  Ctx *ctx;
  int entry = -1;
  hipEvent_t a = nullptr, b = nullptr;
  ProfScope(Ctx *c, const char *name);
  ~ProfScope();
};

struct DCol {
  int32_t dtype = SQLRS_NULLTYPE;
  int64_t length = 0;
  int64_t null_count = 0;
  int stride = 1;
  const void *values = nullptr;
  const uint64_t *validity = nullptr;
  const int32_t *offsets = nullptr;
  int64_t data_bytes = 0;
  uint64_t scalar_bits = 0;
  bool scalar_null = false;
  BufP own_values, own_validity, own_offsets;
  bool has_nulls() const { return validity != nullptr && null_count != 0; }
  template <class T> const T *v() const { return (const T *)values; }
};

struct DBatch {
  int64_t rows = 0;
  std::vector<DCol> cols;
};

struct InBatch {
  Ctx *ctx;
  const sqlrs_batch_t *abi;
  std::vector<DCol> cache;
  std::vector<uint8_t> loaded;
  bool host_upload = false;
  const DBatch *shared = nullptr;
  InBatch(Ctx *c, const sqlrs_batch_t *b);
  ~InBatch();
  InBatch(const InBatch &) = delete;
  InBatch &operator=(const InBatch &) = delete;
  int64_t rows() const { return abi->num_rows; }
  int num_columns() const { return abi->num_columns; }
  int32_t dtype(int i) const { return abi->columns[i].dtype; }
  const DCol &col(int i);
  DBatch materialize(bool owned);
};

DCol upload_column(Ctx *ctx, const sqlrs_column_t &c, bool force_copy);
sqlrs_batch_t *emit_batch(Ctx *ctx, DBatch &&b, int out_mem);
sqlrs_batch_t *emit_host_copy(Ctx *ctx, int ncols, const int32_t *dtypes, int64_t rows, const void *const *values,
                              const uint8_t *const *validity, const int64_t *null_counts, const int32_t *const *offsets = nullptr);
sqlrs_batch_t *emit_host_columns(Ctx *ctx, std::vector<sqlrs_column_t> &&cols, int64_t rows);
bool all_fixed_width(const DBatch &b);
void split_rows_to_host(Ctx *ctx, const DBatch &o, const std::vector<int64_t> &cut, void **pin, size_t *pin_cap, int n,
                        sqlrs_batch_t **out);
DCol make_null_column(Ctx *ctx, int32_t dtype, int64_t n);
int64_t count_nulls(Ctx *ctx, const DCol &c);

template <class F> int guard(Ctx *ctx, F &&f) {
  try {
    f();
    return SQLRS_OK;
  } catch (const Error &e) {
    if (ctx) ctx->last_error = e.msg;
    return e.status;
  } catch (const std::exception &e) {
    if (ctx) ctx->last_error = e.what();
    return SQLRS_ERR_INTERNAL;
  }
}

inline int first_lookback_mode() {
  static const int forced = [] {
    const char *e = hook("SQLRS_FORCE_TICKET");
    return (e && e[0] == '1') ? 1 : 0;
  }();
  return forced;
}

constexpr int LB_BACKOFF_CALLS = 64;
inline int lookback_start_mode(Ctx *ctx) {
  if (first_lookback_mode()) return 1;
  if (ctx->lb_backoff > 0) {
    ctx->lb_backoff--;
    return 1;
  }
  return 0;
}
inline void lookback_timed_out(Ctx *ctx) {
  ctx->lb_timeouts++;
  ctx->lb_backoff = LB_BACKOFF_CALLS;
}

struct Expr {
  std::vector<sqlrs_expr_node_t> nodes;
  std::vector<std::string> strings;
  bool empty() const { return nodes.empty(); }
};
Expr expr_from_abi(const sqlrs_expr_t *e);

}

struct sqlrs_ctx : sq::Ctx {};
```

sqlrs_amd/csrc/ctx.hip:

```cpp
#include <cstdlib>

#include <array>
#include <atomic>
#include <mutex>
#include <unordered_set>

#include "common.hpp"
#include "host_stage.hpp"
#include "prims.hpp"
#include "small_async.hpp"

extern "C" void sqlrs_batch_release(sqlrs_batch_t *batch);
namespace sq {

static size_t pool_size_class(size_t bytes) {
  if (bytes < 512) return 512;
  if (bytes <= (1u << 20)) {
    size_t s = 512;
    while (s < bytes) s <<= 1;
    return s;
  }
  return round_up(bytes, (size_t)2 << 20);
}

// ... 1099 lines not shown

struct ExportHolder {
  std::atomic<int> refs{0};
  sqlrs_batch_t *batch = nullptr;
  std::vector<ArrowArray> children;
  std::vector<ArrowArray *> child_ptrs;
  std::vector<std::array<const void *, 3>> bufs;
  const void *top_buf[1] = {nullptr};
  void unref() {
    if (refs.fetch_sub(1) == 1) {
      sqlrs_batch_release(batch);
      delete this;
    }
  }
};
void export_child_release(ArrowArray *a) {
  if (!a || !a->release) return;
  ExportHolder *h = (ExportHolder *)a->private_data;
  a->release = nullptr;
  h->unref();
}
void export_parent_release(ArrowArray *a) {
  if (!a || !a->release) return;
  ExportHolder *h = (ExportHolder *)a->private_data;
  for (int64_t i = 0; i < a->n_children; i++)
    if (a->children[i] && a->children[i]->release) a->children[i]->release(a->children[i]);
  a->release = nullptr;
  h->unref();
}
struct SchemaHolder {
  std::vector<ArrowSchema> children;
  std::vector<ArrowSchema *> child_ptrs;
  std::vector<std::string> names;
};
void export_schema_child_release(ArrowSchema *s) {
  if (s) s->release = nullptr;
}
void export_schema_release(ArrowSchema *s) {
  if (!s || !s->release) return;
  SchemaHolder *h = (SchemaHolder *)s->private_data;
  for (int64_t i = 0; i < s->n_children; i++)
    if (s->children[i] && s->children[i]->release) s->children[i]->release(s->children[i]);
  s->release = nullptr;
  delete h;
}
}

int sqlrs_batch_import_arrow(sqlrs_ctx_t *ctx, struct ArrowArray *array, struct ArrowSchema *schema, sqlrs_batch_t **out) {
  if (out) *out = nullptr;
  return guard(ctx, [&] {
    if (!array || !schema || !out || !array->release || !schema->release) fail(SQLRS_ERR_ARROW, "import_arrow: null or released structure");
    if (!schema->format || std::strcmp(schema->format, "+s") != 0) fail(SQLRS_ERR_ARROW, "import_arrow: a struct array (\"+s\", an exported RecordBatch) is expected");
    if (array->n_children != schema->n_children || array->dictionary || array->length < 0 || array->offset < 0)
      fail(SQLRS_ERR_ARROW, "import_arrow: array and schema do not match");
    if (array->null_count > 0 || (array->null_count < 0 && array->n_buffers > 0 && array->buffers && array->buffers[0]))
      fail(SQLRS_ERR_ARROW, "import_arrow: NULL rows at the struct level");
    if (array->length >= (1ll << 31)) fail(SQLRS_ERR_ARROW, "batch num_rows outside [0, 2^31)");
    const int64_t n = array->length;
    const int nc = (int)array->n_children;
    auto o = std::unique_ptr<OwnedBatch>(new OwnedBatch());
    o->ctx = ctx;
    o->out_mem = SQLRS_MEM_HOST;
    o->descs.resize((size_t)nc);
    for (int c = 0; c < nc; c++) {
      const ArrowArray *a = array->children[c];
      const ArrowSchema *sc = schema->children[c];
      const int32_t dt = (a && sc && !a->dictionary) ? arrow_dtype(sc->format) : -1;
      if (dt < 0) fail(SQLRS_ERR_ARROW, std::string("import_arrow: unsupported column type \"") + ((sc && sc->format) ? sc->format : "?") + "\"");
      const int64_t off = array->offset + a->offset;
      if (a->offset < 0 || a->length < array->offset + n) fail(SQLRS_ERR_ARROW, "import_arrow: child shorter than the struct");
      const int64_t need = dt == SQLRS_UTF8 ? 3 : 2;
      if (a->n_buffers < need || !a->buffers) fail(SQLRS_ERR_ARROW, "import_arrow: missing buffers");
      sqlrs_column_t &d = o->descs[(size_t)c];
      d.dtype = dt;
      d.mem = SQLRS_MEM_HOST;
      d.length = n;
      d.values = nullptr;
      d.validity = nullptr;
      d.offsets = nullptr;
      d.null_count = 0;
      if (a->null_count != 0 && a->buffers[0] && n > 0) {
        d.validity = bits_at(a->buffers[0], off, n, o->host_blocks);
        d.null_count = a->null_count > 0 && a->offset == 0 && a->length == n && array->offset == 0 ? a->null_count : clear_bits(d.validity, n);
        if (d.null_count == 0) d.validity = nullptr;
      }
      if (n > 0 && !a->buffers[1] && dt != SQLRS_UTF8) fail(SQLRS_ERR_ARROW, "import_arrow: missing values buffer");
      switch (dt) {
      case SQLRS_BOOLEAN: d.values = bits_at(a->buffers[1], off, n, o->host_blocks); break;
      case SQLRS_UTF8: {
        static const int32_t zero_off[1] = {0};
        const int32_t *po = a->buffers[1] ? (const int32_t *)a->buffers[1] + off : zero_off;
        if (po[0] != 0) {
          int32_t *no = (int32_t *)std::malloc(4 * (size_t)(n + 1) + 8);
          if (!no) fail(SQLRS_ERR_INTERNAL, "host allocation failed");
          o->host_blocks.push_back(no);
          for (int64_t i = 0; i <= n; i++) no[i] = po[i] - po[0];
          d.values = (const uint8_t *)a->buffers[2] + po[0];
          d.offsets = no;
        } else {
          d.offsets = po;
          d.values = a->buffers[2] ? a->buffers[2] : (const void *)zero_off;
        }
        break;
      }
      default: d.values = (const uint8_t *)a->buffers[1] + (size_t)off * width_of(dt);
      }
    }
    o->abi.num_rows = n;
    o->abi.num_columns = nc;
    o->abi.reserved = 0;
    o->abi.columns = o->descs.data();
    o->abi.owner = o.get();
    o->imported = *array;
    array->release = nullptr;
    schema->release(schema);
    *out = &o.release()->abi;
  });
}

int sqlrs_batch_export_arrow(sqlrs_ctx_t *ctx, sqlrs_batch_t *batch, const char *const *names, struct ArrowArray *out_array,
                             struct ArrowSchema *out_schema) {
  return guard(ctx, [&] {
    if (!batch || !out_array || !out_schema) fail(SQLRS_ERR_ARROW, "export_arrow: null argument");
    SQ_HIP(hipSetDevice(ctx->device));
    bool ours = false;
    if (batch->owner) {
      std::lock_guard<std::mutex> lk(g_owned_mu);
      ours = g_owned.count(batch->owner) != 0;
    }
    bool host = true;
    for (int c = 0; c < batch->num_columns; c++) host = host && batch->columns[c].mem == SQLRS_MEM_HOST;
    sqlrs_batch_t *hb = batch;
    if (!ours || !host) {
      InBatch ib(ctx, batch);
      hb = emit_batch(ctx, ib.materialize(true), SQLRS_MEM_HOST);
    }
    const int nc = hb->num_columns;
    for (int c = 0; c < nc; c++)
      if (!arrow_format(hb->columns[c].dtype)) {
        if (hb != batch) sqlrs_batch_release(hb);
        fail(SQLRS_ERR_ARROW, "export_arrow: column type without an Arrow format");
      }
    auto h = std::unique_ptr<ExportHolder>(new ExportHolder());
    auto sh = std::unique_ptr<SchemaHolder>(new SchemaHolder());
    h->children.resize((size_t)nc);
    h->child_ptrs.resize((size_t)nc);
    h->bufs.resize((size_t)nc);
    sh->children.resize((size_t)nc);
    sh->child_ptrs.resize((size_t)nc);
    sh->names.resize((size_t)nc);
    static const int32_t zero_off[1] = {0};
    for (int c = 0; c < nc; c++) {
      const sqlrs_column_t &col = hb->columns[c];
      ArrowArray &a = h->children[(size_t)c];
      a = ArrowArray{};
      a.length = col.length;
      a.null_count = col.validity ? col.null_count : 0;
      a.offset = 0;
      h->bufs[(size_t)c] = {col.validity && col.null_count != 0 ? col.validity : nullptr, nullptr, nullptr};
      if (col.dtype == SQLRS_UTF8) {
        a.n_buffers = 3;
        h->bufs[(size_t)c][1] = col.offsets ? (const void *)col.offsets : (const void *)zero_off;
        h->bufs[(size_t)c][2] = col.values;
      } else {
        a.n_buffers = 2;
        h->bufs[(size_t)c][1] = col.values;
      }
      a.buffers = h->bufs[(size_t)c].data();
      a.release = export_child_release;
      a.private_data = h.get();
      h->child_ptrs[(size_t)c] = &a;
      ArrowSchema &s = sh->children[(size_t)c];
      s = ArrowSchema{};
      sh->names[(size_t)c] = (names && names[c]) ? names[c] : ("c" + std::to_string(c));
      s.format = arrow_format(col.dtype);
      s.name = sh->names[(size_t)c].c_str();
      s.flags = ARROW_FLAG_NULLABLE;
      s.release = export_schema_child_release;
      sh->child_ptrs[(size_t)c] = &s;
    }
    *out_array = ArrowArray{};
    out_array->length = hb->num_rows;
    out_array->n_buffers = 1;
    out_array->buffers = h->top_buf;
    out_array->n_children = nc;
    out_array->children = h->child_ptrs.data();
    out_array->release = export_parent_release;
    out_array->private_data = h.get();
    *out_schema = ArrowSchema{};
    out_schema->format = "+s";
    out_schema->name = "";
    out_schema->n_children = nc;
    out_schema->children = sh->child_ptrs.data();
    out_schema->release = export_schema_release;
    out_schema->private_data = sh.release();
    h->batch = hb;
    h->refs.store(nc + 1);
    h.release();
    if (hb != batch) sqlrs_batch_release(batch);
  });
}

struct sqlrs_timer {
  Ctx *ctx;
  hipEvent_t a, b;
};
int sqlrs_timer_create(sqlrs_ctx_t *ctx, sqlrs_timer_t **out) {
  return guard(ctx, [&] {
    auto *t = new sqlrs_timer();
    t->ctx = ctx;
    SQ_HIP(hipEventCreate(&t->a));
    SQ_HIP(hipEventCreate(&t->b));
    *out = t;
  });
}
int sqlrs_timer_start(sqlrs_timer_t *t) {
  return guard(t->ctx, [&] { SQ_HIP(hipEventRecord(t->a, t->ctx->stream)); });
}
int sqlrs_timer_stop(sqlrs_timer_t *t) {
  return guard(t->ctx, [&] { SQ_HIP(hipEventRecord(t->b, t->ctx->stream)); });
}
int sqlrs_timer_elapsed_ms(sqlrs_timer_t *t, double *ms) {
  return guard(t->ctx, [&] {
    SQ_HIP(hipEventSynchronize(t->b));
    float f = 0;
    SQ_HIP(hipEventElapsedTime(&f, t->a, t->b));
    *ms = f;
  });
}
void sqlrs_timer_destroy(sqlrs_timer_t *t) {
  if (!t) return;
  (void)hipEventDestroy(t->a);
  (void)hipEventDestroy(t->b);
  delete t;
}

int sqlrs_ctx_profile_enable(sqlrs_ctx_t *ctx, int on) {
  return guard(ctx, [&] {
    ctx->prof_resolve();
    ctx->prof_on = on != 0;
  });
}
int sqlrs_ctx_profile_reset(sqlrs_ctx_t *ctx) {
  return guard(ctx, [&] {
    ctx->prof_resolve();
    for (auto &e : ctx->prof) {
      e.total_ms = 0;
      e.launches = 0;
    }
  });
}
int sqlrs_ctx_profile_read(sqlrs_ctx_t *ctx, int cap, const char **names, double *total_ms,
                           int64_t *launches) {
  try {
    ctx->prof_resolve();
  } catch (...) {
    return 0;
  }
  int n = 0;
  for (auto &e : ctx->prof) {
    if (n < cap) {
      names[n] = e.name;
      total_ms[n] = e.total_ms;
      launches[n] = e.launches;
    }
    n++;
  }
  if (ctx->lb_timeouts) {
    if (n < cap) {
      names[n] = "lookback_ticket_reruns";
      total_ms[n] = 0;
      launches[n] = ctx->lb_timeouts;
    }
    n++;
  }
  if (ctx->async_fast_batches) {
    if (n < cap) {
      names[n] = "async_fast_batches";
      total_ms[n] = 0;
      launches[n] = ctx->async_fast_batches;
    }
    n++;
  }
  if (ctx->async_conj_batches) {
    if (n < cap) {
      names[n] = "async_conj_batches";
      total_ms[n] = 0;
      launches[n] = ctx->async_conj_batches;
    }
    n++;
  }
  if (ctx->order_lb_fallbacks) {
    if (n < cap) {
      names[n] = "order_lookback_fallbacks";
      total_ms[n] = 0;
      launches[n] = ctx->order_lb_fallbacks;
    }
    n++;
  }
  static const char *const AGG_ROUTE_NAMES[Ctx::AR_COUNT_] = {
      "agg_part_dense", "agg_part_slim_runs", "agg_part_slim_blk", "agg_part_probe_spec", "agg_part_probe_generic",
      "agg_part_interpreted", "agg_part_packed", "agg_part_unpacked", "agg_part_flags", "agg_part_rec",
      "agg_part_in_place", "agg_part_join", "agg_part_join_mult", "agg_part_split", "agg_part_overflow_rows",
      "agg_merge_groups", "agg_pending_deferred", "agg_wide_parts"};
  for (int r = 0; r < Ctx::AR_COUNT_; r++) {
    if (!ctx->agg_route[r]) continue;
    if (n < cap) {
      names[n] = AGG_ROUTE_NAMES[r];
      total_ms[n] = 0;
      launches[n] = ctx->agg_route[r];
    }
    n++;
  }
  static const char *const JOIN_ROUTE_NAMES[Ctx::JR_COUNT_] = {
      "join_dense_adopted", "join_dense_refused", "join_dense_one_fetch", "join_dense_two_fetch", "join_dense_packed",
      "join_dense_plain", "join_probe_pending", "join_allhit_kept", "join_allhit_redone", "join_compact_dense",
      "join_compact_slots", "join_unique_outer", "join_dd_stream", "join_dd_rows", "join_counts_grouped",
      "join_counts_per_row", "join_lds_unique", "join_lds_distinct", "join_table_late"};
  for (int r = 0; r < Ctx::JR_COUNT_; r++) {
    if (!ctx->join_route[r]) continue;
    if (n < cap) {
      names[n] = JOIN_ROUTE_NAMES[r];
      total_ms[n] = 0;
      launches[n] = ctx->join_route[r];
    }
    n++;
  }
  static const char *const ORDER_ROUTE_NAMES[Ctx::OR_COUNT_] = {
      "order_general", "order_utf8_key", "order_narrow", "order_narrow_hbm_only", "order_form_lookback", "order_form_counting",
      "order_rec12", "order_rec16", "order_wide", "order_wide_declined", "order_wide_pure_copy", "order_wide_finish2",
      "order_wide_finish3", "order_heavy_to_wide", "order_range_sampled", "order_range_missed", "order_in_order",
      "order_composite", "order_composite_nullable", "order_composite_too_wide", "order_null_split", "order_topk",
      "order_topk_ignored", "order_alloc_declined", "order_topk_keys", "order_topk_keys_ignored"};
  for (int r = 0; r < Ctx::OR_COUNT_; r++) {
    if (!ctx->order_route[r]) continue;
    if (n < cap) {
      names[n] = ORDER_ROUTE_NAMES[r];
      total_ms[n] = 0;
      launches[n] = ctx->order_route[r];
    }
    n++;
  }
  const int64_t stage_counts[2] = {ctx->stage_all_types_batches, ctx->stage_stitch_flushes};
  static const char *const STAGE_COUNT_NAMES[2] = {"stage_all_types_batches", "stage_stitch_flushes"};
  for (int r = 0; r < 2; r++) {
    if (!stage_counts[r]) continue;
    if (n < cap) {
      names[n] = STAGE_COUNT_NAMES[r];
      total_ms[n] = 0;
      launches[n] = stage_counts[r];
    }
    n++;
  }
  if (ctx->simple_reduce_batches) {
    if (n < cap) {
      names[n] = "simple_reduce_batches";
      total_ms[n] = 0;
      launches[n] = ctx->simple_reduce_batches;
    }
    n++;
  }
  const int64_t fused_counts[2] = {ctx->fused_eval_filter_batches, ctx->fused_eval_project_columns};
  static const char *const FUSED_COUNT_NAMES[2] = {"fused_eval_filter_batches", "fused_eval_project_columns"};
  for (int r = 0; r < 2; r++) {
    if (!fused_counts[r]) continue;
    if (n < cap) {
      names[n] = FUSED_COUNT_NAMES[r];
      total_ms[n] = 0;
      launches[n] = fused_counts[r];
    }
    n++;
  }
  return n;
}

const char *sqlrs_version(void) { return "sqlrs-hip 0.1.0 gfx950"; }

}
```

sqlrs_amd/csrc/hashagg_op.hip:

```cpp
#include <cstdlib>

#include "agg_partition.hpp"
#include "agg_state.hpp"
#include "common.hpp"
#include "device_utils.hpp"
#include "host_stage.hpp"
#include "prims.hpp"

using namespace sq;

namespace {

struct AggSpec {
  int func = 0, distinct = 0;
  int32_t return_dtype = 0;
  Expr arg;
  GrowBuf acc, nn;
  bool track_nn = false;
  int32_t acc_dtype = 0;
  int argcol = -1;
  struct StrBatch {
    DCol col;
    BufP gid;
    int64_t n;
  };
  std::vector<StrBatch> strs;
};

uint64_t acc_identity(const AggSpec &a) { return a.func == SQLRS_AGG_MIN ? ~0ull : 0ull; }

bool same_expr(const Expr &x, const Expr &y) {
  if (x.nodes.size() != y.nodes.size()) return false;
  for (size_t i = 0; i < x.nodes.size(); i++) {
    const sqlrs_expr_node_t &p = x.nodes[i], &q = y.nodes[i];
    if (p.op != q.op || p.dtype != q.dtype || p.index != q.index || p.is_null != q.is_null || p.i != q.i ||
        std::memcmp(&p.f, &q.f, 8) != 0 || x.strings[i] != y.strings[i])
      return false;
  }
  return true;
}

}

struct PendingGroups {
  bool active = false;
  PartAggOutput po;
  std::vector<DCol> keyvals;
  std::vector<int> cnt_of_col, acc_of_agg, col_of_agg;
  std::vector<uint8_t> col_nullable;
  std::vector<int32_t> col_dtype;
  bool exact = true;
  int32_t key_dtype = SQLRS_INT64;
};

struct sqlrs_hash_agg {
  Ctx *ctx = nullptr;
  HostStage hstage;
  PendingGroups pending;
  std::vector<Expr> group_by;
  std::vector<AggSpec> aggs;
  AggState st;
  bool saw_batch = false, in_order = true;
  struct Staged {
    std::vector<DCol> kcols, acols;
    int64_t n = 0;
  };
  std::vector<Staged> staged;
  int64_t staged_rows = 0;
  bool any_order = false;
  bool strong_keys = false;
  int64_t rows_seen = 0;
  std::vector<int32_t> key_dtypes;
  std::vector<std::vector<DCol>> key_parts;
  std::vector<Expr> arg_exprs;
  std::vector<int32_t> arg_cast;
  struct DistinctAgg {
    int func = 0;
    int32_t return_dtype = 0;
    sqlrs_hash_agg *dedup = nullptr;
  };
  std::vector<DistinctAgg> distinct_aggs;
  std::vector<std::pair<int, int>> out_order;
  bool has_filter = false;
  Expr filter;
  int64_t filter_fused_batches = 0;
  std::vector<sqlrs_hash_agg *> parts;
  std::vector<std::pair<int, int>> part_col;
  ~sqlrs_hash_agg() {
    for (auto &d : distinct_aggs) delete d.dedup;
    for (auto *p : parts) delete p;
  }
};

extern "C" int sqlrs_hash_agg_push(sqlrs_hash_agg_t *a, const sqlrs_batch_t *in);
extern "C" int sqlrs_hash_agg_finish(sqlrs_hash_agg_t *a, int out_mem, sqlrs_batch_t **out);
extern "C" int sqlrs_hash_agg_create(sqlrs_ctx_t *ctx, int num_group_by, const sqlrs_expr_t *group_by, int num_aggs,
                                     const sqlrs_agg_func_t *aggs, sqlrs_hash_agg_t **out);
extern "C" void sqlrs_hash_agg_destroy(sqlrs_hash_agg_t *a);
extern "C" void sqlrs_batch_release(sqlrs_batch_t *batch);
extern "C" int sqlrs_filter_create(sqlrs_ctx_t *, const sqlrs_expr_t *, sqlrs_filter_t **);
extern "C" int sqlrs_filter_push(sqlrs_filter_t *, const sqlrs_batch_t *, int, sqlrs_batch_t **);
extern "C" void sqlrs_filter_destroy(sqlrs_filter_t *);

namespace sq {
bool fusable_row_filter(const Expr &e, InBatch &ib, RowFilter *rf);

__global__ void gather_u32_kernel(const uint32_t *__restrict__ src, const uint32_t *__restrict__ idx,
                                  int64_t n, uint32_t *__restrict__ out) {
  int64_t i = blockIdx.x * (int64_t)blockDim.x + threadIdx.x;
  if (i < n) out[i] = src[idx[i]];
}
__global__ void rowid_from_u32_kernel(const uint32_t *__restrict__ rows, int64_t n, uint64_t offset,
                                      uint64_t *__restrict__ out) {
  int64_t i = blockIdx.x * (int64_t)blockDim.x + threadIdx.x;
  if (i < n) out[i] = offset + rows[i];
}

struct ArgView {
  const void *values = nullptr;
  const uint64_t *validity = nullptr;
  int32_t dtype = 0;
  const DCol *col = nullptr;
};

static BufP resolve_groups(sqlrs_hash_agg *a, const NKeys &nk, const uint64_t *row_ids,
                           const uint32_t *local_map, const std::vector<DCol> &kcols, int64_t *nnew_out) {
  Ctx *ctx = a->ctx;
  BufP new_rows;
  int64_t nnew = 0;
  BufP row_gid = agg_resolve_rows(ctx, a->st, nk, row_ids, (uint64_t)a->rows_seen, &new_rows, &nnew);
  if (nnew) {
    const void *idx = new_rows->p;
    BufP mapped;
    if (local_map) {
      mapped = ctx->alloc(4 * (size_t)nnew);
      gather_u32_kernel<<<dim3((unsigned)ceil_div(nnew, 256)), dim3(256), 0, ctx->stream>>>(
          local_map, new_rows->as<uint32_t>(), nnew, mapped->as<uint32_t>());
      SQ_HIP(hipGetLastError());
      idx = mapped->p;
    }
    for (size_t c = 0; c < kcols.size(); c++)
      a->key_parts[c].push_back(gather_column(ctx, kcols[c], idx, false, nullptr, nnew));
  }
  if (row_ids) a->in_order = false;
  *nnew_out = nnew;
  return row_gid;
}

static void start_tracking(Ctx *ctx, AggSpec &s, int64_t G, int64_t nnew) {
  if (s.track_nn) return;
  s.track_nn = true;
  s.nn.ensure(ctx, std::max<int64_t>(G, 1), 0);
  if (G - nnew > 0) fill_u64(ctx, s.nn.buf->as<uint64_t>(), G - nnew, 1);
}

__global__ void rank_of_perm_kernel(const uint32_t *__restrict__ perm, int64_t n, uint32_t *__restrict__ rank) {
  int64_t i = blockIdx.x * (int64_t)blockDim.x + threadIdx.x;
  if (i < n) rank[perm[i]] = (uint32_t)i;
}
__global__ void best_rank_kernel(const uint32_t *__restrict__ gid, const uint32_t *__restrict__ rank,
                                 const uint64_t *__restrict__ validity, int64_t n, int is_min,
                                 uint32_t *__restrict__ best) {
  int64_t i = blockIdx.x * (int64_t)blockDim.x + threadIdx.x;
  if (i >= n) return;
  if (validity && !((validity[i >> 6] >> (i & 63)) & 1)) return;
  if (is_min) atomicMin(&best[gid[i]], rank[i] + 1);
  else atomicMax(&best[gid[i]], rank[i] + 1);
}
__global__ void winner_row_kernel(const uint32_t *__restrict__ best, const uint32_t *__restrict__ perm, int64_t G,
                                  int is_min, uint32_t *__restrict__ row, uint64_t *__restrict__ has) {
  int64_t g = blockIdx.x * (int64_t)blockDim.x + threadIdx.x;
  uint32_t b = g < G ? best[g] : 0;
  bool ok = g < G && b != (is_min ? 0xffffffffu : 0u);
  if (g < G) row[g] = ok ? perm[b - 1] : 0;
  uint64_t m = __ballot(ok);
  if (lane_id() == 0 && g < G) has[g >> 6] = m;
}

static DCol finalize_utf8_minmax(Ctx *ctx, AggSpec &s, int64_t G) {
  const int is_min = s.func == SQLRS_AGG_MIN;
  int64_t G1 = std::max<int64_t>(G, 1);
  std::vector<const DCol *> parts;
  int64_t N = 0;
  for (auto &sb : s.strs) {
    parts.push_back(&sb.col);
    N += sb.n;
  }
  if (parts.empty() || N == 0) return make_null_column(ctx, SQLRS_UTF8, G);
  if (N > 0xfffffffell) fail(SQLRS_ERR_INTERNAL, "utf8 min/max: more than 2^32 rows");
  DCol all = concat_columns(ctx, parts);
  BufP gid = ctx->alloc(4 * (size_t)N);
  size_t off = 0;
  for (auto &sb : s.strs) {
    if (sb.n) SQ_HIP(hipMemcpyAsync(gid->as<uint8_t>() + off, sb.gid->p, 4 * (size_t)sb.n, hipMemcpyDeviceToDevice, ctx->stream));
    off += 4 * (size_t)sb.n;
  }
  const uint64_t *valid = (all.validity && all.null_count != 0) ? all.validity : nullptr;
  BufP perm = ctx->alloc(4 * (size_t)N), keys = ctx->alloc(8 * (size_t)N), rank = ctx->alloc(4 * (size_t)N);
  iota_u32(ctx, perm->as<uint32_t>(), N);
  sort_perm_by_utf8(ctx, all, valid, 0, perm->as<uint32_t>(), keys->as<uint64_t>(), N);
  dim3 b(256), gn((unsigned)ceil_div(N, 256));
  rank_of_perm_kernel<<<gn, b, 0, ctx->stream>>>(perm->as<uint32_t>(), N, rank->as<uint32_t>());
  BufP best = ctx->alloc(4 * (size_t)G1);
  SQ_HIP(hipMemsetAsync(best->p, is_min ? 0xff : 0, 4 * (size_t)G1, ctx->stream));
  best_rank_kernel<<<gn, b, 0, ctx->stream>>>(gid->as<uint32_t>(), rank->as<uint32_t>(), valid, N, is_min,
                                               best->as<uint32_t>());
  BufP row = ctx->alloc(4 * (size_t)G1), has = ctx->alloc_zero(bitmap_bytes(G1));
  int64_t G64 = (int64_t)round_up((size_t)G1, 64);
  winner_row_kernel<<<dim3((unsigned)ceil_div(G64, 256)), b, 0, ctx->stream>>>(
      best->as<uint32_t>(), perm->as<uint32_t>(), G, is_min, row->as<uint32_t>(), has->as<uint64_t>());
  SQ_HIP(hipGetLastError());
  DCol out = gather_column(ctx, all, row->p, false, has->as<uint64_t>(), G);
  out.dtype = SQLRS_UTF8;
  return out;
}

static void update_from_rows(sqlrs_hash_agg *a, const BufP &rgbuf, const std::vector<ArgView> &args,
                             int64_t n, int64_t nnew) {
  Ctx *ctx = a->ctx;
  int64_t G = a->st.ngroups;
  const uint32_t *rg = rgbuf->as<uint32_t>();
  for (AggSpec &s : a->aggs) {
    const ArgView &v = args[(size_t)s.argcol];
    if (v.dtype == SQLRS_UTF8 && (s.func == SQLRS_AGG_MIN || s.func == SQLRS_AGG_MAX)) {
      if (s.return_dtype != SQLRS_UTF8 || !v.col) fail(SQLRS_ERR_INTERNAL, "unsupported min_max scalar type");
      AggSpec::StrBatch sb;
      bool borrowed = (v.col->values && !v.col->own_values) || (v.col->validity && !v.col->own_validity) ||
                      (v.col->offsets && !v.col->own_offsets);
      sb.col = borrowed ? copy_column(ctx, *v.col) : *v.col;
      sb.gid = rgbuf;
      sb.n = n;
      s.strs.push_back(std::move(sb));
      continue;
    }
    if (s.func == SQLRS_AGG_COUNT) {
      s.nn.ensure(ctx, G, 0);
      agg_update_count(ctx, s.nn, rg, v.validity, nullptr, n);
      continue;
    }
    if (v.validity) start_tracking(ctx, s, G, nnew);
    if (s.track_nn) {
      s.nn.ensure(ctx, G, 0);
      agg_update_count(ctx, s.nn, rg, v.validity, nullptr, n);
    }
    if (s.func == SQLRS_AGG_SUM) {
      s.acc_dtype = s.return_dtype;
      s.acc.ensure(ctx, G, 0);
      agg_update_sum(ctx, s.acc, s.acc_dtype, rg, v.values, v.validity, n);
    } else {
      if (v.dtype != s.return_dtype) fail(SQLRS_ERR_INTERNAL, "unsupported min_max scalar type");
      s.acc_dtype = v.dtype;
      s.acc.ensure(ctx, G, acc_identity(s));
      agg_update_minmax(ctx, s.acc, s.acc_dtype, s.func == SQLRS_AGG_MIN, rg, v.values, v.validity, n);
    }
  }
}

static void merge_groups(sqlrs_hash_agg *a, PendingGroups &pg) {
  Ctx *ctx = a->ctx;
  ctx->agg_route[Ctx::AR_MERGE_GROUPS]++;
  PartAggOutput &po = pg.po;
  NKeys gk;
  gk.rows = po.groups;
  gk.keys = po.gkey;
  gk.exact = pg.exact;
  gk.dtype = pg.key_dtype;
  if (po.gvalid_bits) {
    gk.validity = po.gvalid_bits->as<uint64_t>();
    gk.own_validity = po.gvalid_bits;
  }
  int64_t nnew = 0;
  BufP rgid = resolve_groups(a, gk, part_row_ids(ctx, po), nullptr, pg.keyvals, &nnew);
  const uint32_t *rg = rgid->as<uint32_t>();
  int64_t G = a->st.ngroups, g = po.groups;
  auto cell = [&](int acc) { return po.gacc->as<uint64_t>() + (size_t)acc * (size_t)po.gcap; };
  for (size_t i = 0; i < a->aggs.size(); i++) {
    AggSpec &s = a->aggs[i];
    int col = pg.col_of_agg[i];
    int cc = pg.cnt_of_col[(size_t)col];
    if (s.func == SQLRS_AGG_COUNT) {
      s.nn.ensure(ctx, G, 0);
      agg_update_count(ctx, s.nn, rg, nullptr, (const int64_t *)cell(cc), g);
      continue;
    }
    if (pg.col_nullable[(size_t)col]) start_tracking(ctx, s, G, nnew);
    if (s.track_nn) {
      s.nn.ensure(ctx, G, 0);
      agg_update_count(ctx, s.nn, rg, nullptr, (const int64_t *)cell(cc), g);
    }
    int ac = pg.acc_of_agg[i];
    if (s.func == SQLRS_AGG_SUM) {
      s.acc_dtype = s.return_dtype;
      s.acc.ensure(ctx, G, 0);
      agg_update_sum(ctx, s.acc, s.acc_dtype, rg, cell(ac), nullptr, g);
    } else {
      s.acc_dtype = pg.col_dtype[(size_t)col];
      s.acc.ensure(ctx, G, acc_identity(s));
      agg_update_minmax(ctx, s.acc, SQLRS_UINT64 , s.func == SQLRS_AGG_MIN, rg,
                        cell(ac), nullptr, g);
    }
  }
}

static void flush_pending(sqlrs_hash_agg *a) {
  if (!a->pending.active) return;
  PendingGroups pg = std::move(a->pending);
  a->pending = PendingGroups();
  merge_groups(a, pg);
}

static DBatch emit_pending(sqlrs_hash_agg *a) {
  Ctx *ctx = a->ctx;
  PendingGroups &pg = a->pending;
  PartAggOutput &po = pg.po;
  int64_t G = po.groups;
  DBatch o;
  o.rows = G;
  for (const DCol &k : pg.keyvals) o.cols.push_back(k);
  auto cell = [&](int acc) { return po.gacc->as<uint64_t>() + (size_t)acc * (size_t)po.gcap; };
  for (size_t i = 0; i < a->aggs.size(); i++) {
    AggSpec &s = a->aggs[i];
    int col = pg.col_of_agg[i];
    int cc = pg.cnt_of_col[(size_t)col];
    if (s.func == SQLRS_AGG_COUNT) {
      o.cols.push_back(agg_finalize_raw(ctx, s.func, SQLRS_INT64, cell(cc), nullptr, G, po.gacc));
      continue;
    }
    const uint64_t *nn = pg.col_nullable[(size_t)col] ? cell(cc) : nullptr;
    int32_t dt = s.func == SQLRS_AGG_SUM ? s.return_dtype : pg.col_dtype[(size_t)col];
    DCol c = agg_finalize_raw(ctx, s.func, dt, cell(pg.acc_of_agg[i]), nn, G, po.gacc);
    c.dtype = s.return_dtype;
    o.cols.push_back(c);
  }
  if (G > 1 && !a->any_order) {
    ProfScope ps(ctx, "agg_order_groups");
    BufP perm = ctx->alloc(4 * (size_t)G);
    int bits = 1;
    while (bits < 32 && (1ull << bits) <= (uint64_t)std::max<int64_t>(a->rows_seen, 1)) bits++;
    radix_sort_index_u32(ctx, po.gfirst->as<uint32_t>(), G, bits, perm->as<uint32_t>());
    if (!gather_columns_packed(ctx, o.cols, G, perm->as<uint32_t>(), G))
      for (DCol &c : o.cols) c = gather_column(ctx, c, perm->p, false, nullptr, G);
  }
  return o;
}

static DCol distinct_column(sqlrs_hash_agg *a, sqlrs_hash_agg::DistinctAgg &d, int64_t G) {
  Ctx *ctx = a->ctx;
  sqlrs_batch_t *dd = nullptr, *res = nullptr;
  int st = sqlrs_hash_agg_finish(d.dedup, SQLRS_MEM_DEVICE, &dd);
  if (st != SQLRS_OK) fail(st, ctx->last_error);
  const int nk = (int)a->group_by.size();
  std::vector<sqlrs_expr_node_t> nodes((size_t)nk + 1);
  std::vector<sqlrs_expr_t> gb((size_t)nk);
  std::memset(nodes.data(), 0, sizeof(sqlrs_expr_node_t) * nodes.size());
  for (int i = 0; i < nk; i++) {
    nodes[(size_t)i].op = SQLRS_EXPR_INPUT_REF;
    nodes[(size_t)i].index = i;
    gb[(size_t)i].nodes = &nodes[(size_t)i];
    gb[(size_t)i].num_nodes = 1;
    gb[(size_t)i].reserved = 0;
  }
  sqlrs_agg_func_t af;
  std::memset(&af, 0, sizeof(af));
  if (d.func == SQLRS_AGG_COUNT) {
    nodes[(size_t)nk].op = SQLRS_EXPR_CONSTANT;
    nodes[(size_t)nk].dtype = SQLRS_INT64;
    nodes[(size_t)nk].i = 1;
    af.func = SQLRS_AGG_COUNT;
    af.return_dtype = SQLRS_INT64;
  } else {
    nodes[(size_t)nk].op = SQLRS_EXPR_INPUT_REF;
    nodes[(size_t)nk].index = nk;
    af.func = SQLRS_AGG_SUM;
    af.return_dtype = d.return_dtype;
  }
  af.arg.nodes = &nodes[(size_t)nk];
  af.arg.num_nodes = 1;
  sqlrs_hash_agg_t *b = nullptr;
  st = sqlrs_hash_agg_create((sqlrs_ctx_t *)ctx, nk, gb.data(), 1, &af, &b);
  if (st == SQLRS_OK) st = sqlrs_hash_agg_push(b, dd);
  if (st == SQLRS_OK) st = sqlrs_hash_agg_finish(b, SQLRS_MEM_DEVICE, &res);
  std::string err = ctx->last_error;
  if (b) sqlrs_hash_agg_destroy(b);
  DCol out;
  if (st == SQLRS_OK) {
    if (res->num_rows != G) {
      st = SQLRS_ERR_INTERNAL;
      err = "distinct aggregate produced a different number of groups";
    } else {
      const sqlrs_column_t &c = res->columns[nk];
      out.dtype = c.dtype;
      out.length = G;
      size_t w = width_of(c.dtype);
      out.own_values = ctx->alloc(w * (size_t)std::max<int64_t>(G, 1));
      out.values = out.own_values->p;
      if (G) SQ_HIP(hipMemcpyAsync(out.own_values->p, c.values, w * (size_t)G, hipMemcpyDeviceToDevice, ctx->stream));
      if (c.validity && c.null_count != 0) {
        out.own_validity = ctx->alloc(bitmap_bytes(std::max<int64_t>(G, 1)));
        SQ_HIP(hipMemcpyAsync(out.own_validity->p, c.validity, bitmap_bytes(G), hipMemcpyDeviceToDevice, ctx->stream));
        out.validity = out.own_validity->as<uint64_t>();
        out.null_count = c.null_count;
      }
      ctx->sync();
    }
  }
  if (dd) sqlrs_batch_release(dd);
  if (res) sqlrs_batch_release(res);
  if (st != SQLRS_OK) fail(st, err);
  return out;
}

static void place_aggregate_columns(sqlrs_hash_agg *a, DBatch &o) {
  if (a->distinct_aggs.empty()) return;
  const size_t nk = a->group_by.size();
  std::vector<DCol> cols(o.cols.begin(), o.cols.begin() + (long)nk);
  for (auto &e : a->out_order) {
    if (e.first == 0)
      cols.push_back(o.cols[nk + (size_t)e.second]);
    else
      cols.push_back(distinct_column(a, a->distinct_aggs[(size_t)e.second], o.rows));
  }
  o.cols = std::move(cols);
}

static std::vector<DCol> eval_arg_columns(sqlrs_hash_agg *a, const std::function<const DCol &(int)> &colfn,
                                          int64_t n, int shift) {
  Ctx *ctx = a->ctx;
  std::vector<DCol> acols;
  for (size_t k = 0; k < a->arg_exprs.size(); k++) {
    Expr e = a->arg_exprs[k];
    if (shift)
      for (auto &nd : e.nodes)
        if (nd.op == SQLRS_EXPR_INPUT_REF) nd.index -= shift;
    DCol c = eval_expr(ctx, e, colfn, n, true);
    if (a->arg_cast[k] && c.dtype != a->arg_cast[k]) {
      sqlrs_expr_node_t cn[2];
      std::memset(cn, 0, sizeof(cn));
      cn[0].op = SQLRS_EXPR_INPUT_REF;
      cn[1].op = SQLRS_EXPR_TYPE_CAST;
      cn[1].dtype = a->arg_cast[k];
      Expr ce;
      ce.nodes.assign(cn, cn + 2);
      ce.strings.resize(2);
      auto one = [&](int) -> const DCol & { return c; };
      DCol casted = eval_expr(ctx, ce, one, n, true);
      c = casted;
    }
    acols.push_back(c);
  }
  return acols;
}

struct JoinSide {
  const uint64_t *keys;
  const uint64_t *validity;
  int64_t n;
  PartitionedRows *cache;
  bool unique_known = true;
  bool range_known = false;
  uint64_t omin = 0, omax = 0;
  const uint64_t *bits = nullptr;
  const uint32_t *mult = nullptr;
};

static bool agg_consume(sqlrs_hash_agg *a, int64_t n, const std::vector<DCol> &kcols, const NKeys &nk,
                        const std::vector<DCol> &acols, const JoinSide *js, const RowFilter *rf = nullptr) {
  Ctx *ctx = a->ctx;
    auto views_of = [&](const std::vector<DCol> &cols) {
      std::vector<ArgView> v;
      for (const DCol &c : cols) {
        ArgView x;
        x.values = c.values;
        x.validity = (c.validity && c.null_count != 0) ? c.validity : nullptr;
        x.dtype = c.dtype;
        x.col = &c;
        v.push_back(x);
      }
      return v;
    };

    std::vector<DCol> pcols;
    std::vector<int> pidx(acols.size(), -1);
    for (size_t k = 0; k < acols.size(); k++) {
      for (size_t j = 0; j < k && pidx[k] < 0; j++)
        if (same_expr(a->arg_exprs[j], a->arg_exprs[k]) && acols[j].dtype == acols[k].dtype) pidx[k] = pidx[j];
      if (pidx[k] < 0) {
        pidx[k] = (int)pcols.size();
        pcols.push_back(acols[k]);
      }
    }
    bool done = false;
    const int64_t PART_MIN_ROWS = 1ll << 21;
    if ((n >= PART_MIN_ROWS || js) && pcols.size() <= 2) {
      PartAggSpec spec;
      bool ok = true;
      std::vector<int> acc_of_agg(a->aggs.size(), -1), cnt_of_col(pcols.size(), -1);
      for (const DCol &c : pcols)
        ok &= (c.dtype == SQLRS_INT64 || c.dtype == SQLRS_FLOAT64);
      for (size_t k = 0; ok && k < pcols.size(); k++) {
        bool need = pcols[k].validity && pcols[k].null_count != 0;
        for (const AggSpec &s : a->aggs)
          if (pidx[(size_t)s.argcol] == (int)k && (s.func == SQLRS_AGG_COUNT || s.track_nn)) need = true;
        if (need) {
          if (spec.n_acc >= PART_MAX_ACC) { ok = false; break; }
          cnt_of_col[k] = spec.n_acc;
          spec.op[spec.n_acc] = PART_COUNT;
          spec.src[spec.n_acc++] = (int)k;
        }
      }
      for (size_t i = 0; ok && i < a->aggs.size(); i++) {
        const AggSpec &s = a->aggs[i];
        if (s.func == SQLRS_AGG_COUNT) {
          acc_of_agg[i] = cnt_of_col[(size_t)pidx[(size_t)s.argcol]];
          continue;
        }
        if (spec.n_acc >= PART_MAX_ACC) { ok = false; break; }
        const DCol &c = pcols[(size_t)pidx[(size_t)s.argcol]];
        if (s.func != SQLRS_AGG_SUM && c.dtype != s.return_dtype) { ok = false; break; }
        acc_of_agg[i] = spec.n_acc;
        spec.op[spec.n_acc] = s.func == SQLRS_AGG_SUM ? (c.dtype == SQLRS_FLOAT64 ? PART_SUM_F64 : PART_SUM_I64)
                              : s.func == SQLRS_AGG_MIN ? PART_MIN : PART_MAX;
        spec.kind[spec.n_acc] = c.dtype == SQLRS_FLOAT64 ? 1 : 0;
        spec.src[spec.n_acc++] = pidx[(size_t)s.argcol];
      }
      spec.nv = (int)pcols.size();
      if (ok) {
        PartAggInput pin;
        pin.keys = nk.keys->as<uint64_t>();
        pin.key_validity = nk.validity;
        pin.n = n;
        for (size_t k = 0; k < pcols.size(); k++) {
          pin.vals[k] = pcols[k].values;
          pin.val_validity[k] = (pcols[k].validity && pcols[k].null_count != 0) ? pcols[k].validity : nullptr;
        }
        if (js) {
          pin.join_keys = js->keys;
          pin.join_validity = js->validity;
          pin.join_n = js->n;
          pin.join_cache = js->cache;
          pin.join_range_known = js->range_known;
          pin.join_unique_known = js->unique_known;
          pin.join_omin = js->omin;
          pin.join_omax = js->omax;
          pin.join_bits = js->bits;
          pin.join_mult = js->mult;
        }
        if (rf) pin.filter = *rf;
        PartAggOutput po;
        flush_pending(a);
        bool part_ok = partitioned_preaggregate(ctx, spec, pin, (uint64_t)a->rows_seen, &po);
        if (!part_ok && po.retry_exact) {
          pin.exact_stats = true;
          po = PartAggOutput();
          part_ok = partitioned_preaggregate(ctx, spec, pin, (uint64_t)a->rows_seen, &po);
        }
        if (part_ok) {
          PendingGroups pg;
          pg.active = true;
          pg.exact = nk.exact;
          pg.key_dtype = nk.dtype;
          pg.cnt_of_col = cnt_of_col;
          pg.acc_of_agg = acc_of_agg;
          for (const AggSpec &s : a->aggs) pg.col_of_agg.push_back(pidx[(size_t)s.argcol]);
          for (size_t k = 0; k < pcols.size(); k++) {
            pg.col_nullable.push_back(pin.val_validity[k] != nullptr);
            pg.col_dtype.push_back(pcols[k].dtype);
          }
          if (nk.exact && kcols.size() == 1 && (kcols[0].dtype == SQLRS_INT64 || kcols[0].dtype == SQLRS_FLOAT64) &&
              kcols[0].dtype == nk.dtype) {
            DCol kv;
            kv.dtype = kcols[0].dtype;
            kv.length = po.groups;
            kv.values = po.gkey->p;
            kv.own_values = po.gkey;
            if (po.gvalid_bits) {
              kv.validity = po.gvalid_bits->as<uint64_t>();
              kv.own_validity = po.gvalid_bits;
              kv.null_count = -1;
            }
            pg.keyvals.push_back(kv);
          } else {
            for (const DCol &kc : kcols)
              pg.keyvals.push_back(gather_column(ctx, kc, po.gfirst->p, false, nullptr, po.groups));
          }
          pg.po = po;
          if (a->st.ngroups == 0 && po.n_overflow == 0 && !po.may_dup) {
            a->pending = std::move(pg);
            ctx->agg_route[Ctx::AR_PENDING]++;
          } else
            merge_groups(a, pg);
          if (po.n_overflow) {
            int64_t m = po.n_overflow;
            DCol kc;
            kc.dtype = SQLRS_UINT64;
            kc.length = n;
            kc.values = nk.keys->p;
            kc.validity = nk.validity;
            kc.null_count = nk.validity ? -1 : 0;
            DCol sub = gather_column(ctx, kc, po.ov_rows->p, false, nullptr, m);
            NKeys ok_;
            ok_.rows = m;
            ok_.keys = sub.own_values;
            ok_.exact = nk.exact;
            ok_.dtype = nk.dtype;
            if (sub.validity) {
              ok_.validity = sub.validity;
              ok_.own_validity = sub.own_validity;
            }
            BufP rid = ctx->alloc(8 * (size_t)m);
            rowid_from_u32_kernel<<<dim3((unsigned)ceil_div(m, 256)), dim3(256), 0, ctx->stream>>>(
                po.ov_rows->as<uint32_t>(), m, (uint64_t)a->rows_seen, rid->as<uint64_t>());
            SQ_HIP(hipGetLastError());
            std::vector<DCol> sub_args;
            for (const DCol &c : acols) sub_args.push_back(gather_column(ctx, c, po.ov_rows->p, false, nullptr, m));
            int64_t nn2 = 0;
            BufP rg2 = resolve_groups(a, ok_, rid->as<uint64_t>(), po.ov_rows->as<uint32_t>(), kcols, &nn2);
            for (DCol &c : sub_args)
              if (c.validity && c.null_count < 0) c.null_count = count_nulls(ctx, c);
            update_from_rows(a, rg2, views_of(sub_args), m, nn2);
          }
          done = true;
        }
      }
    }
    if (!done && (js || rf)) return false;
    if (!done) {
      flush_pending(a);
      int64_t nnew = 0;
      BufP row_gid = resolve_groups(a, nk, nullptr, nullptr, kcols, &nnew);
      update_from_rows(a, row_gid, views_of(acols), n, nnew);
    }
    return true;
}

static const int64_t STAGE_DIRECT_ROWS = [] {
  const char *e = hook("SQLRS_STAGE_DIRECT_ROWS");
  return e ? std::atoll(e) : (1ll << 26);
}();
static const int64_t STAGE_FLUSH_ROWS = [] {
  const char *e = hook("SQLRS_STAGE_FLUSH_ROWS");
  return e ? std::atoll(e) : (1ll << 28);
}();

static DCol own_column(Ctx *ctx, const DCol &c, int64_t n) {
  DCol m = c.stride == 0 ? materialize_scalar(ctx, c, n) : c;
  bool borrowed = (m.values && !m.own_values) || (m.validity && !m.own_validity) || (m.offsets && !m.own_offsets);
  return borrowed ? copy_column(ctx, m) : m;
}

static void flush_staged(sqlrs_hash_agg *a) {
  if (a->staged.empty()) return;
  Ctx *ctx = a->ctx;
  std::vector<sqlrs_hash_agg::Staged> st = std::move(a->staged);
  a->staged.clear();
  int64_t n = a->staged_rows;
  a->staged_rows = 0;
  std::vector<DCol> kcols, acols;
  if (st.size() == 1) {
    kcols = std::move(st[0].kcols);
    acols = std::move(st[0].acols);
  } else {
    for (size_t c = 0; c < st[0].kcols.size(); c++) {
      std::vector<const DCol *> parts;
      for (auto &b : st) parts.push_back(&b.kcols[c]);
      kcols.push_back(concat_columns(ctx, parts));
    }
    for (size_t c = 0; c < st[0].acols.size(); c++) {
      std::vector<const DCol *> parts;
      for (auto &b : st) parts.push_back(&b.acols[c]);
      acols.push_back(concat_columns(ctx, parts));
    }
  }
  NKeys nk = a->strong_keys ? normalize_keys_strong(ctx, kcols, n) : normalize_keys(ctx, kcols, n);
  agg_consume(a, n, kcols, nk, acols, nullptr);
  a->rows_seen += n;
}

}

extern "C" {

static int hash_agg_create_impl(sqlrs_ctx_t *ctx, int num_group_by, const sqlrs_expr_t *group_by, int num_aggs,
                                const sqlrs_agg_func_t *aggs, bool allow_split, sqlrs_hash_agg_t **out);
int sqlrs_hash_agg_create(sqlrs_ctx_t *ctx, int num_group_by, const sqlrs_expr_t *group_by,
                          int num_aggs, const sqlrs_agg_func_t *aggs, sqlrs_hash_agg_t **out) {
  int st = hash_agg_create_impl(ctx, num_group_by, group_by, num_aggs, aggs, true, out);
  if (st == SQLRS_OK) (*out)->hstage.all_types = stage_all_types_flag(num_group_by, group_by);
  return st;
}

static void hash_agg_plan_parts(sqlrs_hash_agg *a, sqlrs_ctx_t *ctx, int num_group_by, const sqlrs_expr_t *group_by,
                                const sqlrs_agg_func_t *aggs) {
  const char *env = hook("SQLRS_AGG_SPLIT");
  if (env && std::atoi(env) == 0) return;
  if (!a->distinct_aggs.empty() || a->aggs.size() < 3) return;
  std::vector<int> col_of((size_t)a->aggs.size(), -1);
  int ncols = 0;
  for (size_t i = 0; i < a->aggs.size(); i++) {
    if (a->aggs[i].return_dtype == SQLRS_UTF8) return;
    for (size_t k = 0; k < i && col_of[i] < 0; k++)
      if (same_expr(a->aggs[k].arg, a->aggs[i].arg)) col_of[i] = col_of[k];
    if (col_of[i] < 0) col_of[i] = ncols++;
  }
  struct Part {
    std::vector<int> cols, aggs;
    int cells = 0;
  };
  std::vector<Part> plan;
  for (size_t i = 0; i < a->aggs.size(); i++) {
    const int c = col_of[i], own = a->aggs[i].func != SQLRS_AGG_COUNT ? 1 : 0;
    size_t at = plan.size();
    for (size_t q = 0; q < plan.size() && at == plan.size(); q++) {
      const bool has = std::find(plan[q].cols.begin(), plan[q].cols.end(), c) != plan[q].cols.end();
      if (has && plan[q].cells + own <= PART_MAX_ACC) at = q;
    }
    if (at == plan.size()) plan.emplace_back();
    Part &pt = plan[at];
    if (std::find(pt.cols.begin(), pt.cols.end(), c) == pt.cols.end()) {
      pt.cols.push_back(c);
      pt.cells++;
    }
    pt.cells += own;
    pt.aggs.push_back((int)i);
  }
  if (plan.size() < 2) return;
  if (ncols <= 2) {
    int cells = ncols;
    for (const AggSpec &sp : a->aggs) cells += sp.func != SQLRS_AGG_COUNT ? 1 : 0;
    if (cells <= PART_MAX_ACC) return;
  }
  a->part_col.assign(a->aggs.size(), {0, 0});
  for (size_t q = 0; q < plan.size(); q++) {
    std::vector<sqlrs_agg_func_t> sub;
    for (size_t k = 0; k < plan[q].aggs.size(); k++) {
      sub.push_back(aggs[plan[q].aggs[k]]);
      a->part_col[(size_t)plan[q].aggs[k]] = {(int)q, (int)k};
    }
    sqlrs_hash_agg_t *p = nullptr;
    int st = hash_agg_create_impl(ctx, num_group_by, group_by, (int)sub.size(), sub.data(), false, &p);
    if (st != SQLRS_OK) fail(st, ctx->last_error);
    a->parts.push_back(p);
  }
}

static int hash_agg_create_impl(sqlrs_ctx_t *ctx, int num_group_by, const sqlrs_expr_t *group_by, int num_aggs,
                                const sqlrs_agg_func_t *aggs, bool allow_split, sqlrs_hash_agg_t **out) {
  return guard(ctx, [&] {
    if (num_group_by < 1)
      fail(SQLRS_ERR_INTERNAL, "HashAgg needs at least one group-by expression");
    auto a = std::unique_ptr<sqlrs_hash_agg>(new sqlrs_hash_agg());
    a->ctx = ctx;
    for (int i = 0; i < num_group_by; i++) a->group_by.push_back(expr_from_abi(&group_by[i]));
    for (int i = 0; i < num_aggs; i++) {
      AggSpec s;
      s.func = aggs[i].func;
      s.distinct = aggs[i].distinct;
      s.return_dtype = aggs[i].return_dtype;
      s.arg = expr_from_abi(&aggs[i].arg);
      if (s.func < SQLRS_AGG_COUNT || s.func > SQLRS_AGG_MAX)
        fail(SQLRS_ERR_INTERNAL, "unknown aggregate function");
      if (s.distinct && (s.func == SQLRS_AGG_COUNT || s.func == SQLRS_AGG_SUM)) {
        if (s.func == SQLRS_AGG_SUM && s.return_dtype != SQLRS_INT64 && s.return_dtype != SQLRS_FLOAT64)
          fail(SQLRS_ERR_INTERNAL, "not expected types for sum");
        sqlrs_hash_agg::DistinctAgg d;
        d.func = s.func;
        d.return_dtype = s.return_dtype;
        d.dedup = new sqlrs_hash_agg();
        d.dedup->ctx = ctx;
        d.dedup->strong_keys = true;
        d.dedup->group_by = a->group_by;
        d.dedup->group_by.push_back(s.arg);
        d.dedup->key_parts.resize(d.dedup->group_by.size());
        a->out_order.emplace_back(1, (int)a->distinct_aggs.size());
        a->distinct_aggs.push_back(d);
        continue;
      }
      a->out_order.emplace_back(0, (int)a->aggs.size());
      if (s.func == SQLRS_AGG_SUM && s.return_dtype != SQLRS_INT64 && s.return_dtype != SQLRS_FLOAT64)
        fail(SQLRS_ERR_INTERNAL, "not expected types for sum");
      int32_t cast = s.func == SQLRS_AGG_SUM ? s.return_dtype : 0;
      int found = -1;
      for (size_t k = 0; k < a->arg_exprs.size(); k++)
        if (a->arg_cast[k] == cast && same_expr(a->arg_exprs[k], s.arg)) found = (int)k;
      if (found < 0) {
        a->arg_exprs.push_back(s.arg);
        a->arg_cast.push_back(cast);
        found = (int)a->arg_exprs.size() - 1;
      }
      s.argcol = found;
      a->aggs.push_back(std::move(s));
    }
    a->key_parts.resize((size_t)num_group_by);
    if (allow_split) hash_agg_plan_parts(a.get(), ctx, num_group_by, group_by, aggs);
    *out = a.release();
  });
}

static int hash_agg_push_device(sqlrs_hash_agg_t *a, const sqlrs_batch_t *in, bool filtered = false);
static int hash_agg_flush_host(sqlrs_hash_agg_t *a) {
  if (!a->hstage.has_schema) return SQLRS_OK;
  sqlrs_batch_t *dev = nullptr;
  int st = guard(a->ctx, [&] {
    SQ_HIP(hipSetDevice(a->ctx->device));
    dev = a->hstage.take();
  });
  if (st != SQLRS_OK) return st;
  st = hash_agg_push_device(a, dev);
  sqlrs_batch_release(dev);
  return st;
}

int sqlrs_hash_agg_push(sqlrs_hash_agg_t *a, const sqlrs_batch_t *in) {
  if (!a->parts.empty()) a->saw_batch = true;
  a->hstage.ctx = a->ctx;
  if (a->hstage.accepts(in)) {
    int st = a->hstage.flush_before(in) ? hash_agg_flush_host(a) : SQLRS_OK;
    if (st == SQLRS_OK) st = guard(a->ctx, [&] { a->hstage.append(in); });
    if (st != SQLRS_OK || a->hstage.rows < HOST_STAGE_FLUSH_ROWS) return st;
    return hash_agg_flush_host(a);
  }
  int st = hash_agg_flush_host(a);
  return st != SQLRS_OK ? st : hash_agg_push_device(a, in);
}

static bool hash_agg_try_fused_filter(sqlrs_hash_agg_t *a, const sqlrs_batch_t *in) {
  Ctx *ctx = a->ctx;
  const int64_t n = in->num_rows;
  if (!a->staged.empty() || n < STAGE_DIRECT_ROWS || !a->distinct_aggs.empty()) return false;
  for (const Expr &e : a->group_by)
    for (const sqlrs_expr_node_t &nd : e.nodes)
      if (nd.op == SQLRS_EXPR_DIVIDE) return false;
  for (const Expr &e : a->arg_exprs)
    for (const sqlrs_expr_node_t &nd : e.nodes)
      if (nd.op == SQLRS_EXPR_DIVIDE) return false;
  InBatch ib(ctx, in);
  RowFilter rf;
  if (!fusable_row_filter(a->filter, ib, &rf)) return false;
  auto colfn = [&](int i) -> const DCol & { return ib.col(i); };
  std::vector<DCol> kcols;
  for (const Expr &e : a->group_by) kcols.push_back(eval_expr(ctx, e, colfn, n, true));
  std::vector<DCol> acols = eval_arg_columns(a, colfn, n, 0);
  NKeys nk = a->strong_keys ? normalize_keys_strong(ctx, kcols, n) : normalize_keys(ctx, kcols, n);
  if (!agg_consume(a, n, kcols, nk, acols, nullptr, &rf)) return false;
  if (!a->saw_batch) {
    a->saw_batch = true;
    for (const DCol &k : kcols) a->key_dtypes.push_back(k.dtype);
  }
  a->rows_seen += n;
  a->filter_fused_batches++;
  return true;
}

static bool any_host_column(const sqlrs_batch_t *b) {
  for (int c = 0; c < b->num_columns; c++)
    if (b->columns[c].mem == SQLRS_MEM_HOST && b->columns[c].length > 0) return true;
  return false;
}
static int hash_agg_push_parts(sqlrs_hash_agg_t *a, const sqlrs_batch_t *in0) {
  const sqlrs_batch_t *in = in0;
  sqlrs_batch_t *dev = nullptr, *kept = nullptr;
  bool filtered = false;
  int st = SQLRS_OK;
  if (a->has_filter) {
    bool fusable = false;
    st = guard(a->ctx, [&] {
      SQ_HIP(hipSetDevice(a->ctx->device));
      if (any_host_column(in0) || in0->num_rows < STAGE_DIRECT_ROWS) return;
      InBatch ib(a->ctx, in0);
      RowFilter rf;
      fusable = fusable_row_filter(a->filter, ib, &rf);
    });
    if (st != SQLRS_OK) return st;
    if (!fusable) {
      std::vector<sqlrs_expr_node_t> nodes = a->filter.nodes;
      for (size_t i = 0; i < nodes.size(); i++) nodes[i].s = a->filter.strings[i].empty() ? nullptr : a->filter.strings[i].c_str();
      sqlrs_expr_t fe{nodes.data(), (int32_t)nodes.size(), 0};
      sqlrs_filter_t *f = nullptr;
      st = sqlrs_filter_create((sqlrs_ctx_t *)a->ctx, &fe, &f);
      if (st != SQLRS_OK) return st;
      st = sqlrs_filter_push(f, in0, SQLRS_MEM_DEVICE, &kept);
      sqlrs_filter_destroy(f);
      if (st != SQLRS_OK) return st;
      in = kept;
      filtered = true;
    }
  }
  if (any_host_column(in)) {
    st = guard(a->ctx, [&] {
      SQ_HIP(hipSetDevice(a->ctx->device));
// ... 611 lines not shown
```

sqlrs_amd/csrc/prims.hpp:

```cpp
#pragma once

#include <functional>

#include "common.hpp"

namespace sq {

void exclusive_scan_u32(Ctx *ctx, const uint32_t *in, int64_t n, uint64_t *out64, uint32_t *out32,
                        uint64_t *total);

struct Selection {
  int64_t rows = 0;
  int64_t count = 0;
  const uint64_t *bits = nullptr;
  BufP own_bits;
  BufP tile_off;
};
Selection selection_from_mask(Ctx *ctx, const DCol &mask);
Selection selection_from_clear_bits(Ctx *ctx, const uint64_t *bits, int64_t rows);
Selection selection_from_set_bits(Ctx *ctx, const uint64_t *bits, int64_t rows);
void selection_finish(Ctx *ctx, Selection &s);
DCol compact_column(Ctx *ctx, const DCol &c, const Selection &s);
BufP selection_indices_u32(Ctx *ctx, const Selection &s);
BufP selection_indices_u64(Ctx *ctx, const Selection &s);
void selection_rows_u32(Ctx *ctx, const uint64_t *bits, const uint64_t *tile_off, int64_t rows, uint32_t *out);

bool filter_fast_path(Ctx *ctx, const Expr &e, const std::function<const DCol &(int)> &col,
                      int64_t rows, int *col_index, Selection *sel, DCol *out_col);

DCol gather_column(Ctx *ctx, const DCol &src, const void *idx, bool idx_is_u64,
                   const uint64_t *idx_validity, int64_t n);
bool gather_columns_packed(Ctx *ctx, std::vector<DCol> &cols, int64_t src_rows, const uint32_t *idx, int64_t n);
DCol concat_columns(Ctx *ctx, const std::vector<const DCol *> &parts);
DCol copy_column(Ctx *ctx, const DCol &c);
void sort_perm_by_utf8(Ctx *ctx, const DCol &c, const uint64_t *valid, int desc, uint32_t *perm, uint64_t *keys,
                       int64_t n);
bool order_topk_keys_select(Ctx *ctx, const DCol &key, int desc, int64_t n, int64_t limit, BufP *idx, int64_t *count);
DCol materialize_scalar(Ctx *ctx, const DCol &c, int64_t rows);
int64_t count_clear_bits(Ctx *ctx, const uint64_t *bits, int64_t rows);

DCol eval_expr(Ctx *ctx, const Expr &e, const std::function<const DCol &(int)> &col, int64_t rows,
               bool materialize);

bool fused_filter_selection(Ctx *ctx, const Expr &e, InBatch &ib, Selection *sel);
bool fused_project_columns(Ctx *ctx, const std::vector<Expr> &exprs, InBatch &ib, std::vector<DCol> *out, std::vector<uint8_t> *computed);

struct NKeys {
  int64_t rows = 0;
  BufP keys;
  const uint64_t *validity = nullptr;
  BufP own_validity;
  bool exact = true;
  int32_t dtype = SQLRS_INT64;
};
NKeys normalize_keys(Ctx *ctx, const std::vector<DCol> &cols, int64_t rows);
NKeys normalize_keys_strong(Ctx *ctx, const std::vector<DCol> &cols, int64_t rows);

void radix_sort_pairs(Ctx *ctx, uint64_t *keys, uint32_t *vals, int64_t n, int begin_bit,
                      int end_bit, bool keys_below_end_bit = false);
void radix_sort_index_u32(Ctx *ctx, const uint32_t *keys, int64_t n, int bits, uint32_t *perm);
void iota_u32(Ctx *ctx, uint32_t *out, int64_t n);
bool order_fast(Ctx *ctx, const DCol &key, int desc, const DCol *carry, int64_t n, DCol *key_out, DCol *carry_out,
                BufP *perm, bool want_perm, bool *in_order = nullptr);
bool order_composite(Ctx *ctx, const std::vector<const DCol *> &keys, const std::vector<int> &desc, const DCol *carry, int64_t n,
                     std::vector<DCol> *keys_out, DCol *carry_out, BufP *perm, bool want_perm, bool *in_order);

}
```

sqlrs_amd/csrc/sort.hip:

```cpp
#include "common.hpp"
#include "device_utils.hpp"
#include "prims.hpp"

namespace sq {

constexpr int RS_WG = 512;
constexpr int RS_WAVES = RS_WG / 64;
constexpr int RS_ITEMS = 8;
constexpr int RS_TILE = RS_WG * RS_ITEMS;

template <bool KEY32 = false>
__global__ __launch_bounds__(RS_WG) void rs_hist_kernel(const uint64_t *__restrict__ keys, int64_t n,
                                                        int shift, int64_t nblocks,
                                                        uint32_t *__restrict__ hist) {
  __shared__ uint32_t h[256];
  if (threadIdx.x < 256) h[threadIdx.x] = 0;
  const int64_t base = (int64_t)blockIdx.x * RS_TILE + threadIdx.x;
  uint64_t k[RS_ITEMS];
#pragma unroll
  for (int r = 0; r < RS_ITEMS; r++)
    k[r] = KEY32 ? (uint64_t)__builtin_nontemporal_load((const uint32_t *)keys + min(base + r * RS_WG, n - 1))
                 : __builtin_nontemporal_load(keys + min(base + r * RS_WG, n - 1));
  __syncthreads();
#pragma unroll
  for (int r = 0; r < RS_ITEMS; r++)
    if (base + r * RS_WG < n) atomicAdd(&h[(k[r] >> shift) & 255], 1u);
  __syncthreads();
  if (threadIdx.x < 256) hist[(int64_t)threadIdx.x * nblocks + blockIdx.x] = h[threadIdx.x];
}

enum { RS_PAIR = 0, RS_PACKED = 1 };
template <int IN, int OUT, bool KEY32 = false>
__global__ __launch_bounds__(RS_WG) void rs_scatter_kernel(
    const uint64_t *__restrict__ keys, const uint32_t *__restrict__ vals, int64_t n, int shift,
    int64_t nblocks, const uint32_t *__restrict__ offsets, uint64_t *__restrict__ keys_out,
    uint32_t *__restrict__ vals_out, int key_lo, uint64_t key_const) {
  __shared__ uint64_t skey[RS_TILE];
  __shared__ uint32_t sval[(IN == RS_PAIR && OUT == RS_PAIR) ? RS_TILE : 1];
  __shared__ uint32_t wcnt[RS_WAVES][256];
  __shared__ uint32_t dstart[256];
  __shared__ int64_t gbase[256];
  __shared__ uint32_t s_wsum[4];
  const int w = wave_id(), lane = lane_id();
  const int64_t tbase = (int64_t)blockIdx.x * RS_TILE;
  const int64_t wrow = tbase + (int64_t)w * (RS_ITEMS * 64) + lane;
  uint64_t k[RS_ITEMS];
  uint32_t v[RS_ITEMS];
#pragma unroll
  for (int j = 0; j < RS_ITEMS; j++) {
    const int64_t i = min(wrow + j * 64, n - 1);
    k[j] = KEY32 ? (uint64_t)__builtin_nontemporal_load((const uint32_t *)keys + i) : __builtin_nontemporal_load(keys + i);
    v[j] = KEY32 ? (uint32_t)i : (IN == RS_PAIR ? __builtin_nontemporal_load(vals + i) : 0u);
  }
  uint32_t goff = threadIdx.x < 256 ? offsets[(int64_t)threadIdx.x * nblocks + blockIdx.x] : 0;
#pragma unroll
  for (int q = 0; q < 4; q++) wcnt[w][lane + 64 * q] = 0;
  uint32_t rnk[RS_ITEMS];
#pragma unroll
  for (int j = 0; j < RS_ITEMS; j++) {
    const bool valid = wrow + j * 64 < n;
    const uint32_t d = (uint32_t)(k[j] >> shift) & 255u;
    uint64_t peers = __ballot(valid);
    uint32_t dlo = 0, dhi = 0;
#pragma unroll
    for (int b = 0; b < 8; b++) {
      const int32_t mask = ((int32_t)(d << (31 - b))) >> 31;
      const uint64_t bm = __ballot(mask != 0);
      dlo |= (uint32_t)bm ^ (uint32_t)mask;
      dhi |= (uint32_t)(bm >> 32) ^ (uint32_t)mask;
    }
    peers &= ~(((uint64_t)dhi << 32) | dlo);
    const uint32_t r = (uint32_t)mbcnt(peers);
    uint32_t old = 0;
    if (valid && r == 0) {
      old = wcnt[w][d];
      wcnt[w][d] = old + (uint32_t)__popcll(peers);
    }
    old = (uint32_t)__shfl((int)old, valid ? __builtin_ctzll(peers) : 0, 64);
    rnk[j] = old + r;
  }
  __syncthreads();
  if (threadIdx.x < 256) {
    uint32_t acc = 0;
#pragma unroll
    for (int q = 0; q < RS_WAVES; q++) {
      uint32_t c = wcnt[q][threadIdx.x];
      wcnt[q][threadIdx.x] = acc;
      acc += c;
    }
    uint32_t inc = wave_iscan_u32(acc);
    if (lane == 63) s_wsum[w] = inc;
    dstart[threadIdx.x] = inc - acc;
  }
  __syncthreads();
  if (threadIdx.x < 256) {
    uint32_t wb = 0;
    for (int q = 0; q < w; q++) wb += s_wsum[q];
    uint32_t ds = dstart[threadIdx.x] + wb;
    dstart[threadIdx.x] = ds;
    gbase[threadIdx.x] = (int64_t)goff - (int64_t)ds;
  }
  __syncthreads();
#pragma unroll
  for (int j = 0; j < RS_ITEMS; j++) {
    if (wrow + j * 64 >= n) continue;
    const uint32_t d = (uint32_t)(k[j] >> shift) & 255u;
    const uint32_t p = dstart[d] + wcnt[w][d] + rnk[j];
    if (IN == RS_PAIR && OUT == RS_PACKED) skey[p] = ((k[j] >> key_lo) << 32) | v[j];
    else skey[p] = k[j];
    if (IN == RS_PAIR && OUT == RS_PAIR) sval[p] = v[j];
  }
  __syncthreads();
  const uint32_t len = (uint32_t)min<int64_t>(RS_TILE, n - tbase);
#pragma unroll
  for (int j = 0; j < RS_ITEMS; j++) {
    const uint32_t p = j * RS_WG + threadIdx.x;
    if (p < len) {
      const uint64_t kk = skey[p];
      const int sh = (IN == RS_PAIR && OUT == RS_PACKED) ? shift - key_lo + 32 : shift;
      const int64_t g = gbase[(uint32_t)(kk >> sh) & 255u] + p;
      if (OUT == RS_PACKED) {
        keys_out[g] = kk;
      } else if (IN == RS_PACKED) {
        if (keys_out) keys_out[g] = ((kk >> 32) << key_lo) | key_const;
        vals_out[g] = (uint32_t)kk;
      } else {
        if (keys_out) keys_out[g] = kk;
        vals_out[g] = sval[p];
      }
    }
  }
}

__global__ __launch_bounds__(256) void rs_diff_kernel(const uint64_t *__restrict__ keys, int64_t n,
                                                      unsigned long long *diff_or) {
  const uint64_t k0 = keys[0];
  uint64_t d = 0;
  for (int64_t i = blockIdx.x * (int64_t)(256 * 8) + threadIdx.x; i < n; i += (int64_t)gridDim.x * (256 * 8)) {
    uint64_t k[8];
#pragma unroll
    for (int u = 0; u < 8; u++) k[u] = keys[min(i + u * 256, n - 1)];
#pragma unroll
    for (int u = 0; u < 8; u++) d |= k[u] ^ k0;
  }
  for (int m = 32; m >= 1; m >>= 1) d |= shfl_xor_u64(d, m);
  __shared__ unsigned long long s_d[4];
  if (lane_id() == 0) s_d[wave_id()] = d;
  __syncthreads();
  if (threadIdx.x == 0) {
    d = s_d[0] | s_d[1] | s_d[2] | s_d[3];
    if (d) atomicOr(diff_or, (unsigned long long)d);
  }
  if (blockIdx.x == 0 && threadIdx.x == 0) diff_or[1] = k0;
}

void radix_sort_pairs(Ctx *ctx, uint64_t *keys, uint32_t *vals, int64_t n, int begin_bit,
                      int end_bit, bool keys_below_end_bit) {
  if (n <= 1 || end_bit <= begin_bit) return;
  if (n > 0xffffffffll) fail(SQLRS_ERR_INTERNAL, "radix sort: more than 2^32 rows");
  ProfScope ps(ctx, "radix_sort");
  uint64_t varying = ~0ull, key0 = 0;
  if (keys_below_end_bit && begin_bit == 0 && end_bit <= 32) {
    varying = (1ull << end_bit) - 1;
    key0 = 0;
  } else if ((end_bit - begin_bit > 16 && n >= (1 << 22)) || (end_bit - begin_bit > 32 && n >= (1 << 15))) {
    BufP diff = ctx->alloc_zero(16);
    unsigned blocks = (unsigned)std::min<int64_t>(ceil_div(n, 256 * 8), 4 * (int64_t)ctx->num_cus);
    rs_diff_kernel<<<dim3(blocks), dim3(256), 0, ctx->stream>>>(keys, n, diff->as<unsigned long long>());
    SQ_HIP(hipGetLastError());
    const uint64_t *h = (const uint64_t *)ctx->fetch(diff->p, 16);
    varying = h[0];
    key0 = h[1];
  }
  int64_t nblocks = ceil_div(n, RS_TILE);
  BufP k2 = ctx->alloc(8 * (size_t)n), v2 = ctx->alloc(4 * (size_t)n);
  BufP hist = ctx->alloc(4 * (size_t)(256 * nblocks)), offs = ctx->alloc(4 * (size_t)(256 * nblocks));
  BufP total = ctx->alloc(8);
  uint64_t *ka = keys, *kb = k2->as<uint64_t>();
  uint32_t *va = vals, *vb = v2->as<uint32_t>();
  std::vector<int> shifts;
  for (int shift = begin_bit; shift < end_bit; shift += 8)
    if (((varying >> shift) & 0xff) != 0) shifts.push_back(shift);
  int key_lo = 0;
  uint64_t key_const = 0;
  bool packed = false;
  if (varying != ~0ull && varying != 0 && shifts.size() >= 2) {
    key_lo = shifts.front();
    int key_hi = 64 - __builtin_clzll(varying);
    const bool low_bits_constant = key_lo == 0 || (varying & ((1ull << key_lo) - 1)) == 0;
    if (key_hi - key_lo <= 32 && low_bits_constant) {
      packed = true;
      uint64_t k0 = key0;
      uint64_t span = (key_hi - key_lo == 64) ? ~0ull : (((1ull << (key_hi - key_lo)) - 1) << key_lo);
      key_const = k0 & ~span;
    }
  }
  for (size_t pi = 0; pi < shifts.size(); pi++) {
    const int shift = shifts[pi];
    const bool in_packed = packed && pi > 0, out_packed = packed && pi + 1 < shifts.size();
    const int eff = in_packed ? shift - key_lo + 32 : shift;
    rs_hist_kernel<false><<<dim3((unsigned)nblocks), dim3(RS_WG), 0, ctx->stream>>>(ka, n, eff, nblocks,
                                                                                   hist->as<uint32_t>());
    SQ_HIP(hipGetLastError());
    exclusive_scan_u32(ctx, hist->as<uint32_t>(), 256 * nblocks, nullptr, offs->as<uint32_t>(),
                       total->as<uint64_t>());
    dim3 g((unsigned)nblocks), b(RS_WG);
    if (!in_packed && !out_packed)
      rs_scatter_kernel<RS_PAIR, RS_PAIR><<<g, b, 0, ctx->stream>>>(ka, va, n, shift, nblocks, offs->as<uint32_t>(), kb, vb, 0, 0);
    else if (!in_packed)
      rs_scatter_kernel<RS_PAIR, RS_PACKED><<<g, b, 0, ctx->stream>>>(ka, va, n, shift, nblocks, offs->as<uint32_t>(), kb, vb, key_lo, key_const);
    else if (out_packed)
      rs_scatter_kernel<RS_PACKED, RS_PACKED><<<g, b, 0, ctx->stream>>>(ka, va, n, eff, nblocks, offs->as<uint32_t>(), kb, vb, key_lo, key_const);
    else
      rs_scatter_kernel<RS_PACKED, RS_PAIR><<<g, b, 0, ctx->stream>>>(ka, va, n, eff, nblocks, offs->as<uint32_t>(), kb, vb, key_lo, key_const);
    SQ_HIP(hipGetLastError());
    std::swap(ka, kb);
    std::swap(va, vb);
  }
  if (ka != keys) {
    SQ_HIP(hipMemcpyAsync(keys, ka, 8 * (size_t)n, hipMemcpyDeviceToDevice, ctx->stream));
    SQ_HIP(hipMemcpyAsync(vals, va, 4 * (size_t)n, hipMemcpyDeviceToDevice, ctx->stream));
  }
}

void radix_sort_index_u32(Ctx *ctx, const uint32_t *keys, int64_t n, int bits, uint32_t *perm) {
  if (n <= 0) return;
  if (n > 0xffffffffll) fail(SQLRS_ERR_INTERNAL, "radix sort: more than 2^32 rows");
  ProfScope ps(ctx, "radix_sort");
  const int passes = std::max(1, (std::min(bits, 32) + 7) / 8);
  const int64_t nblocks = ceil_div(n, RS_TILE);
  BufP w0 = ctx->alloc(8 * (size_t)n), w1 = passes > 2 ? ctx->alloc(8 * (size_t)n) : nullptr;
  BufP hist = ctx->alloc(4 * (size_t)(256 * nblocks)), offs = ctx->alloc(4 * (size_t)(256 * nblocks));
  BufP total = ctx->alloc(8);
  dim3 g((unsigned)nblocks), b(RS_WG);
  const uint64_t *in = (const uint64_t *)keys;
  uint64_t *out = w0->as<uint64_t>();
  for (int pi = 0; pi < passes; pi++) {
    const bool first = pi == 0, last = pi + 1 == passes;
    const int shift = first ? 0 : 32 + 8 * pi;
    if (first) rs_hist_kernel<true><<<g, b, 0, ctx->stream>>>(in, n, shift, nblocks, hist->as<uint32_t>());
    else rs_hist_kernel<false><<<g, b, 0, ctx->stream>>>(in, n, shift, nblocks, hist->as<uint32_t>());
    SQ_HIP(hipGetLastError());
    exclusive_scan_u32(ctx, hist->as<uint32_t>(), 256 * nblocks, nullptr, offs->as<uint32_t>(), total->as<uint64_t>());
    if (first && last)
      rs_scatter_kernel<RS_PAIR, RS_PAIR, true><<<g, b, 0, ctx->stream>>>(in, nullptr, n, shift, nblocks, offs->as<uint32_t>(), nullptr, perm, 0, 0);
    else if (first)
      rs_scatter_kernel<RS_PAIR, RS_PACKED, true><<<g, b, 0, ctx->stream>>>(in, nullptr, n, shift, nblocks, offs->as<uint32_t>(), out, nullptr, 0, 0);
    else if (last)
      rs_scatter_kernel<RS_PACKED, RS_PAIR><<<g, b, 0, ctx->stream>>>(in, nullptr, n, shift, nblocks, offs->as<uint32_t>(), nullptr, perm, 0, 0);
    else
      rs_scatter_kernel<RS_PACKED, RS_PACKED><<<g, b, 0, ctx->stream>>>(in, nullptr, n, shift, nblocks, offs->as<uint32_t>(), out, nullptr, 0, 0);
    SQ_HIP(hipGetLastError());
    in = out;
    out = (out == w0->as<uint64_t>() && w1) ? w1->as<uint64_t>() : w0->as<uint64_t>();
  }
}

}
```

Baseline: 92750 Mrows/s.

## Emit packed group rows and fuse first-seen ordering sort with gather

```diff
diff --git a/sqlrs_amd/csrc/agg_partition.hip b/sqlrs_amd/csrc/agg_partition.hip
--- a/sqlrs_amd/csrc/agg_partition.hip
+++ b/sqlrs_amd/csrc/agg_partition.hip
@@ -150,6 +150,10 @@
   const unsigned long long *partner_bits;
   const unsigned int *partner_mult;
   int seg_off;
+};
+
+struct alignas(32) GroupRow {
+  unsigned long long key, cell0, cell1, first;
 };
 
 __device__ __forceinline__ unsigned long long acc_times(int kind, unsigned long long cell, unsigned int m) {
@@ -526,7 +530,7 @@
 __global__ __launch_bounds__(SED_SLOTS * SED_GROUPS) void split_emit_dense_kernel(
     SplitTables stb, const uint32_t *__restrict__ split_bucket, const uint32_t *__restrict__ chunk_lo, uint32_t nbuckets_split,
     uint32_t R, KeyPack kp, LdsAggParams prm, int n_acc, unsigned long long *out_count, uint64_t *__restrict__ gkey,
-    uint32_t *__restrict__ gfirst, uint64_t *__restrict__ gacc, int64_t gcap) {
+    uint32_t *__restrict__ gfirst, uint64_t *__restrict__ gacc, int64_t gcap, GroupRow *__restrict__ grow) {
   __shared__ unsigned int s_first[SED_GROUPS][SED_SLOTS];
   __shared__ unsigned long long s_acc[PART_MAX_ACC][SED_GROUPS][SED_SLOTS];
   const uint32_t tiles_per_bucket = (R + SED_SLOTS - 1) / SED_SLOTS;
@@ -581,16 +585,24 @@
   if (prm.partner_mult) mlt = prm.partner_mult[((uint64_t)split_bucket[t] << kp.rbits) + s];
   unsigned long long base = atomicAdd(out_count, 1ull);
   if ((int64_t)base >= gcap) return;
-  gkey[base] = kp.kmin + ((uint64_t)split_bucket[t] << kp.rbits) + s;
   gfirst[base] = first;
-  for (int a = 0; a < n_acc; a++) gacc[(size_t)a * gcap + base] = prm.partner_mult ? acc_times(prm.code[a] & 7, acc[a], mlt) : acc[a];
+  if (prm.partner_mult)
+    for (int a = 0; a < n_acc; a++) acc[a] = acc_times(prm.code[a] & 7, acc[a], mlt);
+  const uint64_t key = kp.kmin + ((uint64_t)split_bucket[t] << kp.rbits) + s;
+  if (grow) {
+    grow[base] = GroupRow{key, acc[0], n_acc > 1 ? acc[1] : 0ull, first};
+    return;
+  }
+  gkey[base] = key;
+  for (int a = 0; a < n_acc; a++) gacc[(size_t)a * gcap + base] = acc[a];
 }
 
 template <int NV, bool JOIN, int NACC, int C0, int C1, bool REC = false>
 __global__ __launch_bounds__(DENSE_WG) void lds_agg_dense_kernel(
     LdsAggParams prm, const uint64_t *__restrict__ pk, const uint64_t *__restrict__ pv0,
     const uint32_t *__restrict__ work, unsigned long long *out_count, uint64_t *__restrict__ gkey,
-    uint32_t *__restrict__ gfirst, uint64_t *__restrict__ gacc, int64_t gcap, KeyPack kp, SplitTables stb) {
+    uint32_t *__restrict__ gfirst, uint64_t *__restrict__ gacc, int64_t gcap, KeyPack kp, SplitTables stb,
+    GroupRow *__restrict__ grow) {
   extern __shared__ __attribute__((aligned(16))) unsigned long long tab[];
   __shared__ unsigned int s_cnt;
   __shared__ unsigned long long s_base;
@@ -750,14 +762,25 @@
     unsigned int first = tfirst[s];
     if (first == 0xffffffffu) continue;
     if ((int64_t)base < gcap) {
-      gkey[base] = key0 + s;
       gfirst[base] = first;
       const unsigned int mlt = (JOIN && prm.partner_mult) ? prm.partner_mult[((uint64_t)b << kp.rbits) + s] : 1u;
-#pragma unroll
-      for (int a = 0; a < PART_MAX_ACC; a++) {
-        if (a >= n_acc) break;
-        const unsigned long long cell = tacc[(size_t)a * R + s];
-        gacc[(size_t)a * gcap + base] = (JOIN && prm.partner_mult) ? acc_times(code_of(a) & 7, cell, mlt) : cell;
+      if (grow) {
+        unsigned long long c[2] = {0, 0};
+#pragma unroll
+        for (int a = 0; a < 2; a++) {
+          if (a >= n_acc) break;
+          const unsigned long long cell = tacc[(size_t)a * R + s];
+          c[a] = (JOIN && prm.partner_mult) ? acc_times(code_of(a) & 7, cell, mlt) : cell;
+        }
+        grow[base] = GroupRow{key0 + s, c[0], c[1], first};
+      } else {
+        gkey[base] = key0 + s;
+#pragma unroll
+        for (int a = 0; a < PART_MAX_ACC; a++) {
+          if (a >= n_acc) break;
+          const unsigned long long cell = tacc[(size_t)a * R + s];
+          gacc[(size_t)a * gcap + base] = (JOIN && prm.partner_mult) ? acc_times(code_of(a) & 7, cell, mlt) : cell;
+        }
       }
     }
     base++;
@@ -782,7 +805,7 @@
 __global__ __launch_bounds__(DENSE_WG) void lds_agg_dense_slim_kernel(
     LdsAggParams prm, SlimBucketIn in, const uint32_t *__restrict__ work, unsigned long long *out_count,
     uint64_t *__restrict__ gkey, uint32_t *__restrict__ gfirst, uint64_t *__restrict__ gacc, int64_t gcap, KeyPack kp,
-    SplitTables stb) {
+    SplitTables stb, GroupRow *__restrict__ grow) {
   extern __shared__ __attribute__((aligned(16))) unsigned long long tab[];
   __shared__ unsigned int s_cnt, s_before, s_inside;
   __shared__ unsigned long long s_base;
@@ -1087,14 +1110,25 @@
     unsigned int first = tfirst[s];
     if (first == 0xffffffffu) continue;
     if ((int64_t)obase < gcap) {
-      gkey[obase] = key0 + s;
       gfirst[obase] = first;
       const unsigned int mlt = (JOIN && prm.partner_mult) ? prm.partner_mult[((uint64_t)b << kp.rbits) + s] : 1u;
-#pragma unroll
-      for (int a = 0; a < PART_MAX_ACC; a++) {
-        if (a >= n_acc) break;
-        const unsigned long long cell = tacc[(size_t)a * R + s];
-        gacc[(size_t)a * gcap + obase] = (JOIN && prm.partner_mult) ? acc_times(code_of(a) & 7, cell, mlt) : cell;
+      if (grow) {
+        unsigned long long c[2] = {0, 0};
+#pragma unroll
+        for (int a = 0; a < 2; a++) {
+          if (a >= n_acc) break;
+          const unsigned long long cell = tacc[(size_t)a * R + s];
+          c[a] = (JOIN && prm.partner_mult) ? acc_times(code_of(a) & 7, cell, mlt) : cell;
+        }
+        grow[obase] = GroupRow{key0 + s, c[0], c[1], first};
+      } else {
+        gkey[obase] = key0 + s;
+#pragma unroll
+        for (int a = 0; a < PART_MAX_ACC; a++) {
+          if (a >= n_acc) break;
+          const unsigned long long cell = tacc[(size_t)a * R + s];
+          gacc[(size_t)a * gcap + obase] = (JOIN && prm.partner_mult) ? acc_times(code_of(a) & 7, cell, mlt) : cell;
+        }
       }
     }
     obase++;
@@ -1105,6 +1139,15 @@
                                       uint64_t *__restrict__ out) {
   int64_t i = blockIdx.x * (int64_t)blockDim.x + threadIdx.x;
   if (i < n) out[i] = offset + gfirst[i];
+}
+__global__ void group_rows_to_columns_kernel(const GroupRow *__restrict__ grow, int64_t n, int n_acc, int64_t gcap,
+                                             uint64_t *__restrict__ gkey, uint64_t *__restrict__ gacc) {
+  int64_t i = blockIdx.x * (int64_t)blockDim.x + threadIdx.x;
+  if (i >= n) return;
+  const GroupRow r = grow[i];
+  gkey[i] = r.key;
+  gacc[i] = r.cell0;
+  if (n_acc > 1) gacc[gcap + i] = r.cell1;
 }
 __global__ void bytes_pack_kernel(const uint8_t *__restrict__ bytes, int64_t n, uint64_t *__restrict__ out) {
   int64_t i = blockIdx.x * (int64_t)blockDim.x + threadIdx.x;
@@ -1149,6 +1192,18 @@
     }
   }
   return po.row_ids->as<uint64_t>();
+}
+
+void part_group_columns(Ctx *ctx, PartAggOutput &po, int n_acc) {
+  if (!po.grow) return;
+  po.gkey = ctx->alloc(8 * (size_t)po.gcap);
+  po.gacc = ctx->alloc(8 * (size_t)po.gcap * (size_t)std::max(n_acc, 1));
+  if (po.groups) {
+    group_rows_to_columns_kernel<<<dim3((unsigned)ceil_div(po.groups, 256)), dim3(256), 0, ctx->stream>>>(
+        po.grow->as<GroupRow>(), po.groups, n_acc, po.gcap, po.gkey->as<uint64_t>(), po.gacc->as<uint64_t>());
+    SQ_HIP(hipGetLastError());
+  }
+  po.grow = nullptr;
 }
 
 bool partitioned_preaggregate(Ctx *ctx, const PartAggSpec &spec, const PartAggInput &in,
@@ -1436,11 +1491,15 @@
     split_init_kernel<<<dim3((unsigned)ceil_div(total, 256)), dim3(256), 0, ctx->stream>>>(stb, total, spec.n_acc, prm);
     SQ_HIP(hipGetLastError());
   }
-  out->gkey = ctx->alloc(8 * (size_t)gcap);
+  const bool group_rows = in.want_group_rows && dense && !in.key_validity && spec.n_acc >= 1 && spec.n_acc <= 2;
   out->gfirst = ctx->alloc(4 * (size_t)gcap);
   out->gvalid = in.key_validity ? ctx->alloc((size_t)gcap) : nullptr;
-  out->gacc = ctx->alloc(8 * (size_t)gcap * (size_t)std::max(spec.n_acc, 1));
+  out->grow = group_rows ? ctx->alloc(sizeof(GroupRow) * (size_t)gcap) : nullptr;
+  out->gkey = group_rows ? nullptr : ctx->alloc(8 * (size_t)gcap);
+  out->gacc = group_rows ? nullptr : ctx->alloc(8 * (size_t)gcap * (size_t)std::max(spec.n_acc, 1));
   out->gcap = gcap;
+  GroupRow *const grow = group_rows ? out->grow->as<GroupRow>() : nullptr;
+  uint64_t *const gkey = group_rows ? nullptr : out->gkey->as<uint64_t>(), *const gacc = group_rows ? nullptr : out->gacc->as<uint64_t>();
   if (!out->ov_rows) out->ov_rows = ctx->alloc(4 * (size_t)std::max<int64_t>(n, 1));
   ctx->agg_route[pr.pack.kbits ? Ctx::AR_PACKED : Ctx::AR_UNPACKED]++;
   ctx->agg_route[Ctx::AR_FLAGS] += pf != nullptr;
@@ -1502,8 +1561,7 @@
     if (blk) kfn = lds_agg_dense_slim_kernel<JN, NA, C0, C1, true>;                                             \
     allow_big_lds(ctx, kfn, 159 * 1024);                                                                                 \
     kfn<<<dim3(nwork), dim3(DENSE_WG), slds, ctx->stream>>>(prm, sb, dwork->as<uint32_t>(), ctr->as<unsigned long long>(), \
-                                                           out->gkey->as<uint64_t>(), out->gfirst->as<uint32_t>(), \
-                                                           out->gacc->as<uint64_t>(), gcap, pr.pack, stb);        \
+                                                           gkey, out->gfirst->as<uint32_t>(), gacc, gcap, pr.pack, stb, grow); \
     ctx->agg_route[blk ? Ctx::AR_SLIM_BLK : Ctx::AR_SLIM_RUNS]++;                                              \
     ctx->agg_route[Ctx::AR_INTERPRETED] += NA < 0;                                                             \
     launched = true;                                                                                           \
@@ -1520,7 +1578,7 @@
       if (nsplit) {
         split_emit_dense_kernel<<<dim3((unsigned)(nsplit * ceil_div((int64_t)nslots_h, SED_SLOTS))), dim3(SED_SLOTS * SED_GROUPS), 0, ctx->stream>>>(
             stb, dsplit->as<uint32_t>(), dchunk_lo->as<uint32_t>(), nsplit, cap, pr.pack, prm, spec.n_acc,
-            ctr->as<unsigned long long>(), out->gkey->as<uint64_t>(), out->gfirst->as<uint32_t>(), out->gacc->as<uint64_t>(), gcap);
+            ctr->as<unsigned long long>(), gkey, out->gfirst->as<uint32_t>(), gacc, gcap, grow);
       }
     } else if (dense) {
 #define SQ_LD(NV, JN, NA, C0, C1)                                                                              \
@@ -1530,8 +1588,7 @@
     allow_big_lds(ctx, kfn);                                                                                   \
     kfn<<<dim3(nwork), dim3(DENSE_WG), lds, ctx->stream>>>(                                                    \
         prm, pr.rec ? pr.rec->as<uint64_t>() : pk->as<uint64_t>(), pv0 ? pv0->as<uint64_t>() : nullptr, dwork->as<uint32_t>(), \
-        ctr->as<unsigned long long>(), out->gkey->as<uint64_t>(), out->gfirst->as<uint32_t>(),                 \
-        out->gacc->as<uint64_t>(), gcap, pr.pack, stb);                                                        \
+        ctr->as<unsigned long long>(), gkey, out->gfirst->as<uint32_t>(), gacc, gcap, pr.pack, stb, grow);     \
     ctx->agg_route[Ctx::AR_DENSE]++;                                                                           \
     ctx->agg_route[Ctx::AR_INTERPRETED] += NA < 0;                                                             \
     launched = true;                                                                                           \
@@ -1555,7 +1612,7 @@
       if (nsplit) {
         split_emit_dense_kernel<<<dim3((unsigned)(nsplit * ceil_div((int64_t)nslots_h, SED_SLOTS))), dim3(SED_SLOTS * SED_GROUPS), 0, ctx->stream>>>(
             stb, dsplit->as<uint32_t>(), dchunk_lo->as<uint32_t>(), nsplit, cap, pr.pack, prm, spec.n_acc,
-            ctr->as<unsigned long long>(), out->gkey->as<uint64_t>(), out->gfirst->as<uint32_t>(), out->gacc->as<uint64_t>(), gcap);
+            ctr->as<unsigned long long>(), gkey, out->gfirst->as<uint32_t>(), gacc, gcap, grow);
       }
     }
     if (!launched && !pf && nvu == 1 && spec.n_acc <= 2) {
diff --git a/sqlrs_amd/csrc/agg_partition.hpp b/sqlrs_amd/csrc/agg_partition.hpp
--- a/sqlrs_amd/csrc/agg_partition.hpp
+++ b/sqlrs_amd/csrc/agg_partition.hpp
@@ -36,11 +36,13 @@
   const uint32_t *join_mult = nullptr;
   RowFilter filter;
   bool exact_stats = false;
+  bool want_group_rows = false;
 };
 
 struct PartAggOutput {
   int64_t groups = 0, gcap = 0;
   BufP gkey, gfirst, gvalid, gvalid_bits, gacc;
+  BufP grow;
   BufP row_ids;
   uint64_t row_offset = 0;
   int64_t n_overflow = 0;
@@ -52,6 +54,7 @@
 };
 
 const uint64_t *part_row_ids(Ctx *ctx, PartAggOutput &po);
+void part_group_columns(Ctx *ctx, PartAggOutput &po, int n_acc);
 double estimate_distinct(Ctx *ctx, const uint64_t *keys, const uint64_t *validity, int64_t n,
                          uint64_t *omin = nullptr, uint64_t *omax = nullptr, bool *sampled = nullptr);
 bool partitioned_preaggregate(Ctx *ctx, const PartAggSpec &spec, const PartAggInput &in,
diff --git a/sqlrs_amd/csrc/common.hpp b/sqlrs_amd/csrc/common.hpp
--- a/sqlrs_amd/csrc/common.hpp
+++ b/sqlrs_amd/csrc/common.hpp
@@ -148,6 +148,7 @@
     AR_MERGE_GROUPS,
     AR_PENDING,
     AR_WIDE_PARTS,
+    AR_ORDER_PACKED,
     AR_COUNT_
   };
   int64_t agg_route[AR_COUNT_] = {};
diff --git a/sqlrs_amd/csrc/ctx.hip b/sqlrs_amd/csrc/ctx.hip
--- a/sqlrs_amd/csrc/ctx.hip
+++ b/sqlrs_amd/csrc/ctx.hip
@@ -1425,7 +1425,7 @@
       "agg_part_dense", "agg_part_slim_runs", "agg_part_slim_blk", "agg_part_probe_spec", "agg_part_probe_generic",
       "agg_part_interpreted", "agg_part_packed", "agg_part_unpacked", "agg_part_flags", "agg_part_rec",
       "agg_part_in_place", "agg_part_join", "agg_part_join_mult", "agg_part_split", "agg_part_overflow_rows",
-      "agg_merge_groups", "agg_pending_deferred", "agg_wide_parts"};
+      "agg_merge_groups", "agg_pending_deferred", "agg_wide_parts", "agg_order_packed"};
   for (int r = 0; r < Ctx::AR_COUNT_; r++) {
     if (!ctx->agg_route[r]) continue;
     if (n < cap) {
diff --git a/sqlrs_amd/csrc/hashagg_op.hip b/sqlrs_amd/csrc/hashagg_op.hip
--- a/sqlrs_amd/csrc/hashagg_op.hip
+++ b/sqlrs_amd/csrc/hashagg_op.hip
@@ -46,6 +46,7 @@
   bool active = false;
   PartAggOutput po;
   std::vector<DCol> keyvals;
+  int n_acc = 0;
   std::vector<int> cnt_of_col, acc_of_agg, col_of_agg;
   std::vector<uint8_t> col_nullable;
   std::vector<int32_t> col_dtype;
@@ -302,11 +303,66 @@
   }
 }
 
+static DCol group_key_column(const PartAggOutput &po, int32_t dtype) {
+  DCol kv;
+  kv.dtype = dtype;
+  kv.length = po.groups;
+  kv.values = po.gkey->p;
+  kv.own_values = po.gkey;
+  if (po.gvalid_bits) {
+    kv.validity = po.gvalid_bits->as<uint64_t>();
+    kv.own_validity = po.gvalid_bits;
+    kv.null_count = -1;
+  }
+  return kv;
+}
+
+static void group_rows_to_columns(sqlrs_hash_agg *a, PendingGroups &pg) {
+  if (!pg.po.grow) return;
+  part_group_columns(a->ctx, pg.po, pg.n_acc);
+  pg.keyvals.push_back(group_key_column(pg.po, pg.key_dtype));
+}
+
 static void flush_pending(sqlrs_hash_agg *a) {
   if (!a->pending.active) return;
   PendingGroups pg = std::move(a->pending);
   a->pending = PendingGroups();
+  group_rows_to_columns(a, pg);
   merge_groups(a, pg);
+}
+
+static DBatch emit_pending_group_rows(sqlrs_hash_agg *a) {
+  Ctx *ctx = a->ctx;
+  PendingGroups &pg = a->pending;
+  PartAggOutput &po = pg.po;
+  const int64_t G = po.groups;
+  ProfScope ps(ctx, "agg_order_groups");
+  ctx->agg_route[Ctx::AR_ORDER_PACKED]++;
+  DBatch o;
+  o.rows = G;
+  auto column = [&](int32_t dtype) {
+    DCol c;
+    c.dtype = dtype;
+    c.length = G;
+    c.own_values = ctx->alloc(8 * (size_t)G);
+    c.values = c.own_values->p;
+    return c;
+  };
+  SortedRowsOut ro;
+  ro.rows = po.grow->as<uint64_t>();
+  o.cols.push_back(column(pg.key_dtype));
+  ro.key = (uint64_t *)o.cols.back().values;
+  for (size_t i = 0; i < a->aggs.size(); i++) {
+    const AggSpec &s = a->aggs[i];
+    const bool count = s.func == SQLRS_AGG_COUNT;
+    o.cols.push_back(column(count ? SQLRS_INT64 : s.return_dtype));
+    ro.agg[i] = (uint64_t *)o.cols.back().values;
+    ro.cell[i] = count ? pg.cnt_of_col[(size_t)pg.col_of_agg[i]] : pg.acc_of_agg[i];
+  }
+  int bits = 1;
+  while (bits < 32 && (1ull << bits) <= (uint64_t)std::max<int64_t>(a->rows_seen, 1)) bits++;
+  radix_sort_gather_rows_u32(ctx, po.gfirst->as<uint32_t>(), G, bits, ro);
+  return o;
 }
 
 static DBatch emit_pending(sqlrs_hash_agg *a) {
@@ -314,6 +370,8 @@
   PendingGroups &pg = a->pending;
   PartAggOutput &po = pg.po;
   int64_t G = po.groups;
+  if (po.grow && G > 0) return emit_pending_group_rows(a);
+  group_rows_to_columns(a, pg);
   DBatch o;
   o.rows = G;
   for (const DCol &k : pg.keyvals) o.cols.push_back(k);
@@ -546,6 +604,14 @@
           pin.join_mult = js->mult;
         }
         if (rf) pin.filter = *rf;
+        const char *rows_e = hook("SQLRS_AGG_ORDER_PACKED");
+        const bool key_is_value = nk.exact && kcols.size() == 1 && (kcols[0].dtype == SQLRS_INT64 || kcols[0].dtype == SQLRS_FLOAT64) &&
+                                  kcols[0].dtype == nk.dtype;
+        bool rows_ok = !(rows_e && rows_e[0] == '0') && !a->any_order && a->st.ngroups == 0 && !a->pending.active && key_is_value && !nk.validity &&
+                       !a->aggs.empty() && a->aggs.size() <= 2 && spec.n_acc <= 2;
+        for (const AggSpec &s : a->aggs) rows_ok &= s.func == SQLRS_AGG_COUNT || s.func == SQLRS_AGG_SUM;
+        for (size_t k = 0; k < pcols.size(); k++) rows_ok &= pin.val_validity[k] == nullptr;
+        pin.want_group_rows = rows_ok;
         PartAggOutput po;
         flush_pending(a);
         bool part_ok = partitioned_preaggregate(ctx, spec, pin, (uint64_t)a->rows_seen, &po);
@@ -559,6 +625,7 @@
           pg.active = true;
           pg.exact = nk.exact;
           pg.key_dtype = nk.dtype;
+          pg.n_acc = spec.n_acc;
           pg.cnt_of_col = cnt_of_col;
           pg.acc_of_agg = acc_of_agg;
           for (const AggSpec &s : a->aggs) pg.col_of_agg.push_back(pidx[(size_t)s.argcol]);
@@ -566,25 +633,17 @@
             pg.col_nullable.push_back(pin.val_validity[k] != nullptr);
             pg.col_dtype.push_back(pcols[k].dtype);
           }
-          if (nk.exact && kcols.size() == 1 && (kcols[0].dtype == SQLRS_INT64 || kcols[0].dtype == SQLRS_FLOAT64) &&
-              kcols[0].dtype == nk.dtype) {
-            DCol kv;
-            kv.dtype = kcols[0].dtype;
-            kv.length = po.groups;
-            kv.values = po.gkey->p;
-            kv.own_values = po.gkey;
-            if (po.gvalid_bits) {
-              kv.validity = po.gvalid_bits->as<uint64_t>();
-              kv.own_validity = po.gvalid_bits;
-              kv.null_count = -1;
-            }
-            pg.keyvals.push_back(kv);
+          const bool defer = a->st.ngroups == 0 && po.n_overflow == 0 && !po.may_dup;
+          if (!defer) part_group_columns(ctx, po, spec.n_acc);
+          if (po.grow) {
+          } else if (key_is_value) {
+            pg.keyvals.push_back(group_key_column(po, kcols[0].dtype));
           } else {
             for (const DCol &kc : kcols)
               pg.keyvals.push_back(gather_column(ctx, kc, po.gfirst->p, false, nullptr, po.groups));
           }
           pg.po = po;
-          if (a->st.ngroups == 0 && po.n_overflow == 0 && !po.may_dup) {
+          if (defer) {
             a->pending = std::move(pg);
             ctx->agg_route[Ctx::AR_PENDING]++;
           } else
diff --git a/sqlrs_amd/csrc/prims.hpp b/sqlrs_amd/csrc/prims.hpp
--- a/sqlrs_amd/csrc/prims.hpp
+++ b/sqlrs_amd/csrc/prims.hpp
@@ -59,6 +59,13 @@
 void radix_sort_pairs(Ctx *ctx, uint64_t *keys, uint32_t *vals, int64_t n, int begin_bit,
                       int end_bit, bool keys_below_end_bit = false);
 void radix_sort_index_u32(Ctx *ctx, const uint32_t *keys, int64_t n, int bits, uint32_t *perm);
+struct SortedRowsOut {
+  const uint64_t *rows = nullptr;
+  uint64_t *key = nullptr;
+  uint64_t *agg[2] = {nullptr, nullptr};
+  int cell[2] = {0, 0};
+};
+void radix_sort_gather_rows_u32(Ctx *ctx, const uint32_t *keys, int64_t n, int bits, const SortedRowsOut &ro);
 void iota_u32(Ctx *ctx, uint32_t *out, int64_t n);
 bool order_fast(Ctx *ctx, const DCol &key, int desc, const DCol *carry, int64_t n, DCol *key_out, DCol *carry_out,
                 BufP *perm, bool want_perm, bool *in_order = nullptr);
diff --git a/sqlrs_amd/csrc/sort.hip b/sqlrs_amd/csrc/sort.hip
--- a/sqlrs_amd/csrc/sort.hip
+++ b/sqlrs_amd/csrc/sort.hip
@@ -29,12 +29,15 @@
   if (threadIdx.x < 256) hist[(int64_t)threadIdx.x * nblocks + blockIdx.x] = h[threadIdx.x];
 }
 
-enum { RS_PAIR = 0, RS_PACKED = 1 };
+enum { RS_PAIR = 0, RS_PACKED = 1, RS_ROWS = 2 };
+struct alignas(16) RsRowHalf {
+  uint64_t a, b;
+};
 template <int IN, int OUT, bool KEY32 = false>
 __global__ __launch_bounds__(RS_WG) void rs_scatter_kernel(
     const uint64_t *__restrict__ keys, const uint32_t *__restrict__ vals, int64_t n, int shift,
     int64_t nblocks, const uint32_t *__restrict__ offsets, uint64_t *__restrict__ keys_out,
-    uint32_t *__restrict__ vals_out, int key_lo, uint64_t key_const) {
+    uint32_t *__restrict__ vals_out, int key_lo, uint64_t key_const, SortedRowsOut ro = SortedRowsOut()) {
   __shared__ uint64_t skey[RS_TILE];
   __shared__ uint32_t sval[(IN == RS_PAIR && OUT == RS_PAIR) ? RS_TILE : 1];
   __shared__ uint32_t wcnt[RS_WAVES][256];
@@ -119,7 +122,13 @@
       const uint64_t kk = skey[p];
       const int sh = (IN == RS_PAIR && OUT == RS_PACKED) ? shift - key_lo + 32 : shift;
       const int64_t g = gbase[(uint32_t)(kk >> sh) & 255u] + p;
-      if (OUT == RS_PACKED) {
+      if (OUT == RS_ROWS) {
+        const RsRowHalf *row = (const RsRowHalf *)(ro.rows + 4 * (size_t)(uint32_t)kk);
+        const RsRowHalf lo = row[0], hi = row[1];
+        ro.key[g] = lo.a;
+        ro.agg[0][g] = ro.cell[0] ? hi.a : lo.b;
+        if (ro.agg[1]) ro.agg[1][g] = ro.cell[1] ? hi.a : lo.b;
+      } else if (OUT == RS_PACKED) {
         keys_out[g] = kk;
       } else if (IN == RS_PACKED) {
         if (keys_out) keys_out[g] = ((kk >> 32) << key_lo) | key_const;
@@ -223,11 +232,11 @@
   }
 }
 
-void radix_sort_index_u32(Ctx *ctx, const uint32_t *keys, int64_t n, int bits, uint32_t *perm) {
+static void sort_index_u32(Ctx *ctx, const uint32_t *keys, int64_t n, int bits, uint32_t *perm, const SortedRowsOut *ro) {
   if (n <= 0) return;
   if (n > 0xffffffffll) fail(SQLRS_ERR_INTERNAL, "radix sort: more than 2^32 rows");
   ProfScope ps(ctx, "radix_sort");
-  const int passes = std::max(1, (std::min(bits, 32) + 7) / 8);
+  const int passes = std::max(ro ? 2 : 1, (std::min(bits, 32) + 7) / 8);
   const int64_t nblocks = ceil_div(n, RS_TILE);
   BufP w0 = ctx->alloc(8 * (size_t)n), w1 = passes > 2 ? ctx->alloc(8 * (size_t)n) : nullptr;
   BufP hist = ctx->alloc(4 * (size_t)(256 * nblocks)), offs = ctx->alloc(4 * (size_t)(256 * nblocks));
@@ -242,7 +251,9 @@
     else rs_hist_kernel<false><<<g, b, 0, ctx->stream>>>(in, n, shift, nblocks, hist->as<uint32_t>());
     SQ_HIP(hipGetLastError());
     exclusive_scan_u32(ctx, hist->as<uint32_t>(), 256 * nblocks, nullptr, offs->as<uint32_t>(), total->as<uint64_t>());
-    if (first && last)
+    if (last && ro)
+      rs_scatter_kernel<RS_PACKED, RS_ROWS><<<g, b, 0, ctx->stream>>>(in, nullptr, n, shift, nblocks, offs->as<uint32_t>(), nullptr, nullptr, 0, 0, *ro);
+    else if (first && last)
       rs_scatter_kernel<RS_PAIR, RS_PAIR, true><<<g, b, 0, ctx->stream>>>(in, nullptr, n, shift, nblocks, offs->as<uint32_t>(), nullptr, perm, 0, 0);
     else if (first)
       rs_scatter_kernel<RS_PAIR, RS_PACKED, true><<<g, b, 0, ctx->stream>>>(in, nullptr, n, shift, nblocks, offs->as<uint32_t>(), out, nullptr, 0, 0);
@@ -256,4 +267,12 @@
   }
 }
 
-}
+void radix_sort_index_u32(Ctx *ctx, const uint32_t *keys, int64_t n, int bits, uint32_t *perm) {
+  sort_index_u32(ctx, keys, n, bits, perm, nullptr);
+}
+
+void radix_sort_gather_rows_u32(Ctx *ctx, const uint32_t *keys, int64_t n, int bits, const SortedRowsOut &ro) {
+  sort_index_u32(ctx, keys, n, bits, nullptr, &ro);
+}
+
+}
```

New measurement: 93790 Mrows/s, median of 6. +1.1%, better.
